# UDC-GAC/pRIblast

Hardware: AMD Instinct MI355X
Metric: query RNAs/sec in `ris` step (higher is better)
Workload: dtype f64

## Files before the change

### priblast_amd/csrc/capi_core.hip

```cpp
#include <dlfcn.h>

#include <algorithm>
#include <cstdio>
#include <cstdlib>
#include <cstring>
#include <numeric>

#include "../../include/priblast_hip.h"
#include "context.hpp"
#include "raccess_kernels.hpp"

namespace prb {

static thread_local std::string g_error;
void set_error(const std::string &msg) { g_error = msg; }
int hip_fail(hipError_t e, const char *what) {
  g_error = std::string("HIP error '") + hipGetErrorString(e) + "' in " + what;
  return PRB_ERR_HIP;
}

int DevBuf::ensure(size_t bytes) {
  if (bytes <= cap) return PRB_OK;
  if (p) {
    hipError_t e = hipFree(p);
    p = nullptr;
    cap = 0;
    if (e != hipSuccess) return hip_fail(e, "hipFree");
  }
  size_t want = bytes > ((size_t)8 << 30) ? bytes : bytes + bytes / 8;
  hipError_t e = hipMalloc(&p, want);
  if (e != hipSuccess) {
    (void)hipGetLastError();
    e = hipMalloc(&p, bytes);
    want = bytes;
  }
  if (e != hipSuccess) {
    (void)hipGetLastError();
    p = nullptr;
    size_t free_b = 0, total_b = 0;
    (void)hipMemGetInfo(&free_b, &total_b);
    set_error("out of device memory allocating " + std::to_string(bytes) + " bytes (" + std::to_string(free_b >> 20) + " MiB of " +
              std::to_string(total_b >> 20) + " free)");
    return PRB_ERR_NOMEM;
  }
  cap = want;
  return PRB_OK;
}
void DevBuf::release() {
  if (p) (void)hipFree(p);
  p = nullptr;
  cap = 0;
}

static std::string default_param_file() {
  Dl_info info;
  if (dladdr((void *)&default_param_file, &info) && info.dli_fname) {
    std::string so = info.dli_fname;
    size_t k = so.rfind('/');
    std::string dir = k == std::string::npos ? "." : so.substr(0, k);
    return dir + "/../params/rna_andronescu2007.par";
  }
  return "priblast_amd/params/rna_andronescu2007.par";
}

}

int prb_ctx::time_begin() {
  PRB_HIP(hipEventRecord(ev0, stream));
  return PRB_OK;
}
int prb_ctx::time_end(const char *stage, int64_t launches) { return time_end(timers[stage], launches); }
int prb_ctx::time_end(prb::StageTimer &t, int64_t launches) {
  PRB_HIP(hipEventRecord(ev1, stream));
  PRB_HIP(hipEventSynchronize(ev1));
  float ms = 0;
  PRB_HIP(hipEventElapsedTime(&ms, ev0, ev1));
  t.ms += ms;
  t.launches += launches;
  return PRB_OK;
}

using namespace prb;

extern "C" {

const char *prb_last_error(void) { return g_error.c_str(); }
const char *prb_version(void) { return "priblast-hip 0.1 (gfx950)"; }

void prb_ris_opts_default(prb_ris_opts *o) {
  o->max_seed_length = 20;
  o->hybrid_threshold = -6.0;
  o->interaction_threshold = -4.0;
  o->final_threshold = -8.0;
  o->drop_out_wo_gap = 5;
  o->drop_out_w_gap = 16;
  o->min_helix_length = 3;
  o->output_style = 0;
  o->distinct_sites = 0;
  o->chain_sites = 0;
  o->allowed_pairs = nullptr;
}

int prb_search_const_upload(prb_ctx *ctx);
void prb_search_const_free(prb_ctx *ctx);

}

static int ctx_init(prb_ctx *ctx, int device, const char *param_file) {
  PRB_HIP(hipSetDevice(device));
  ctx->device = device;
  std::string pf = param_file ? param_file : default_param_file();
  std::string err = load_energy_params(pf, ctx->params);
  if (!err.empty()) {
    set_error(err);
    return PRB_ERR_IO;
  }
  build_raccess_tables(ctx->params, ctx->ra_tables);
  build_fmath_tables(ctx->fm_tables);
  PRB_HIP(hipStreamCreateWithFlags(&ctx->stream, hipStreamNonBlocking));
  PRB_HIP(hipEventCreate(&ctx->ev0));
  PRB_HIP(hipEventCreate(&ctx->ev1));
  auto up = [&](DevBuf &b, const void *src, size_t bytes) -> int {
    int rc = b.ensure(bytes);
    if (rc) return rc;
    PRB_HIP(hipMemcpy(b.p, src, bytes, hipMemcpyHostToDevice));
    return PRB_OK;
  };
  int rc;
  if ((rc = up(ctx->d_expd, ctx->fm_tables.expd_tbl.data(), 2048 * sizeof(uint64_t)))) return rc;
  if ((rc = up(ctx->d_log, ctx->fm_tables.log_tbl.data(), 4096 * sizeof(float)))) return rc;
  if ((rc = up(ctx->d_small, ctx->ra_tables.small.data(), ctx->ra_tables.small.size() * sizeof(double)))) return rc;
  if ((rc = up(ctx->d_big, ctx->ra_tables.big.data(), ctx->ra_tables.big.size() * sizeof(double)))) return rc;
  RaConst &c = ctx->ra_const;
  c.expd_tbl = ctx->d_expd.as<uint64_t>();
  c.log_tbl = ctx->d_log.as<float>();
  c.small = ctx->d_small.as<double>();
  c.big = ctx->d_big.as<double>();
  c.expd_a = ctx->fm_tables.expd_a;
  c.expd_ra = ctx->fm_tables.expd_ra;
  c.c_log2 = ctx->fm_tables.c_log2;
  for (int a = 0; a < 5; a++)
    for (int b = 0; b < 5; b++) c.bp_pair[a * 5 + b] = (unsigned char)ctx->params.bp_pair[a][b];
  if ((rc = prb_search_const_upload(ctx))) return rc;
  size_t free_b = 0, total_b = 0;
  PRB_HIP(hipMemGetInfo(&free_b, &total_b));
  const char *env = getenv("PRB_RACCESS_WORKSPACE_GB");
  double gb = env ? atof(env) : 48.0;
  ctx->ra_budget_bytes = (size_t)std::min(gb * (double)(1ull << 30), 0.5 * (double)free_b);
  return PRB_OK;
}

extern "C" {

int prb_ctx_create(int device, const char *param_file, prb_ctx **out) {
  if (!out) return PRB_ERR_ARG;
  *out = nullptr;
  int ndev = 0;
  hipError_t e = hipGetDeviceCount(&ndev);
  if (e != hipSuccess || ndev == 0) {
    set_error("no HIP device available (this library has no CPU path)");
    return PRB_ERR_HIP;
  }
  if (device < 0 || device >= ndev) {
    set_error("device index out of range");
    return PRB_ERR_ARG;
  }
  prb_ctx *ctx = nullptr;
  int rc;
  try {
    ctx = new prb_ctx();
    rc = ctx_init(ctx, device, param_file);
  } catch (const std::exception &ex) {
    set_error(std::string("prb_ctx_create: ") + ex.what());
    rc = PRB_ERR_NOMEM;
  }
  if (rc != PRB_OK) {
    const std::string keep = prb_last_error();
    if (ctx) prb_ctx_destroy(ctx);
    set_error(keep);
    return rc;
  }
  *out = ctx;
  return PRB_OK;
}


void prb_ctx_destroy(prb_ctx *ctx) {
  if (!ctx) return;
  (void)hipSetDevice(ctx->device);
  if (ctx->stream) (void)hipStreamSynchronize(ctx->stream);
  prb_search_const_free(ctx);
  for (DevBuf *b : {&ctx->d_expd, &ctx->d_log, &ctx->d_small, &ctx->d_big, &ctx->ra_band, &ctx->ra_vec,
                    &ctx->ra_codes, &ctx->ra_desc, &ctx->ra_watchdog, &ctx->ra_acc, &ctx->ra_cond})
    b->release();
  if (ctx->ev0) (void)hipEventDestroy(ctx->ev0);
  if (ctx->ev1) (void)hipEventDestroy(ctx->ev1);
  if (ctx->stream) (void)hipStreamDestroy(ctx->stream);
  delete ctx;
}

int prb_ctx_synchronize(prb_ctx *ctx) {
  if (!ctx) return PRB_ERR_ARG;
  PRB_HIP(hipStreamSynchronize(ctx->stream));
  return PRB_OK;
}

int prb_ctx_stage_ms(prb_ctx *ctx, const char *stage, double *ms, int64_t *launches) {
  if (!ctx || !stage) return PRB_ERR_ARG;
  if (std::strcmp(stage, "slow_hits") == 0) {
    if (ms) *ms = 0;
    if (launches) *launches = ctx->slow_hits;
    return PRB_OK;
  }
  const prb::StageTimer *t = nullptr;
  for (int i = 0; i < (int)prb::ModeTimer::kCount && !t; i++)
    if (std::strcmp(stage, prb::kModeTimerName[i]) == 0) t = &ctx->mode_timers[i];
  if (!t) {
    auto it = ctx->timers.find(stage);
    if (it != ctx->timers.end()) t = &it->second;
  }
  if (ms) *ms = t ? t->ms : 0.0;
  if (launches) *launches = t ? t->launches : 0;
  return PRB_OK;
}
void prb_ctx_reset_timers(prb_ctx *ctx) {
  if (ctx) {
    ctx->timers.clear();
    for (prb::StageTimer &t : ctx->mode_timers) t = prb::StageTimer{};
    ctx->slow_hits = 0;
  }
}

}

namespace prb {

static inline unsigned char ra_code(char ch) {
  switch (ch) {
  case 'A': case 'a': return 1;
  case 'C': case 'c': return 2;
  case 'G': case 'g': return 3;
  case 'T': case 't': case 'U': case 'u': return 4;
  default: return 0;
  }
}

int run_accessibility(prb_ctx *ctx, int32_t nseq, const char *seqs, const int64_t *in_off, const int32_t *lens,
                      const int64_t *out_off, int W, int delta, float *d_acc, float *d_cond) {
  static_assert(kRaMaxSpan + 2 < RaSmallLayout::kHairpinN, "hairpin table covers every span");
  if (W < 1 || delta < 2 || W > kRaMaxSpan) {
    set_error("unsupported (maximal span -w, min accessible length -d): this build needs 1 <= w <= 255 and d >= 2");
    return PRB_ERR_ARG;
  }
  PRB_HIP(hipSetDevice(ctx->device));
  std::vector<int32_t> order(nseq);
  std::iota(order.begin(), order.end(), 0);
  auto len = [&](int i) { return (int64_t)lens[i]; };
  std::stable_sort(order.begin(), order.end(), [&](int a, int b) { return len(a) > len(b); });
  int32_t pos = 0;
  std::vector<RaSeqDesc> desc;
  std::vector<unsigned char> codes;
  while (pos < nseq) {
    desc.clear();
    codes.clear();
    int64_t band = 0, vec = 0;
    int32_t end = pos;
    while (end < nseq) {
      const int64_t L = len(order[end]);
      const size_t need = (size_t)(band + ra_band_elems((int)L, W) + vec + ra_vec_elems((int)L)) * sizeof(double);
      if (end > pos && (need > ctx->ra_budget_bytes || end - pos >= kRaMaxChunk)) break;
      RaSeqDesc d;
      d.band_off = band;
      d.vec_off = vec;
      d.code_off = (int64_t)codes.size();
      d.out_off = out_off[order[end]];
      d.L = (int32_t)L;
      d.pad = 0;
      desc.push_back(d);
      band += ra_band_elems((int)L, W);
      vec += ra_vec_elems((int)L);
      codes.push_back(0);
      const char *sp = seqs + in_off[order[end]];
      for (int64_t k = 0; k < L; k++) codes.push_back(ra_code(sp[k]));
      codes.push_back(0);
      end++;
    }
    const int32_t n = end - pos;
    int rc;
    if ((rc = ctx->ra_band.ensure((size_t)band * sizeof(double)))) return rc;
    if ((rc = ctx->ra_vec.ensure((size_t)vec * sizeof(double)))) return rc;
    if ((rc = ctx->ra_codes.ensure(codes.size()))) return rc;
    if ((rc = ctx->ra_desc.ensure(desc.size() * sizeof(RaSeqDesc)))) return rc;
    if ((rc = ctx->ra_watchdog.ensure(sizeof(int)))) return rc;
    PRB_HIP(hipMemcpyAsync(ctx->ra_codes.p, codes.data(), codes.size(), hipMemcpyHostToDevice, ctx->stream));
    PRB_HIP(hipMemcpyAsync(ctx->ra_desc.p, desc.data(), desc.size() * sizeof(RaSeqDesc), hipMemcpyHostToDevice,
                           ctx->stream));
    RaBatch b;
    b.desc = ctx->ra_desc.as<RaSeqDesc>();
    b.nseq = n;
    b.lmax = (int32_t)len(order[pos]);
    b.W = W;
    b.delta = delta;
    b.band = ctx->ra_band.as<double>();
    b.vec = ctx->ra_vec.as<double>();
    b.codes = ctx->ra_codes.as<unsigned char>();
    b.acc = d_acc;
    b.cond = d_cond;
    b.watchdog = ctx->ra_watchdog.as<int>();
    {
      const char *e = std::getenv("PRB_RACCESS_LOGSUM_WINDOWS");
      const int64_t lmax = len(order[pos]);
      b.logsum_windows = (e && std::atoi(e) == 0) ? 0 : (int32_t)((lmax + 63) / 64);
      const char *h = std::getenv("PRB_RACCESS_HELPERS");
      b.helpers = h ? std::max(0, std::min(3, std::atoi(h))) : (n <= 512 ? 3 : 0);
      const char *wa = std::getenv("PRB_RACCESS_WINDOWS_ALL");
      b.windows_all = wa ? (std::atoi(wa) != 0) : (n <= 512);
    }
    if (b.helpers == 3) PRB_HIP(hipMemsetAsync(b.watchdog, 0, sizeof(int), ctx->stream));
    if ((rc = ctx->time_begin())) return rc;
    PRB_HIP(ra_launch(b, ctx->ra_const, band, vec, ctx->stream));
    if ((rc = ctx->time_end("raccess", 1))) return rc;
    if (b.helpers == 3) {
      int tripped = 0;
      PRB_HIP(hipMemcpy(&tripped, b.watchdog, sizeof(int), hipMemcpyDeviceToHost));
      if (tripped) {
        set_error("Raccess: a wavefront gave up waiting for its workgroup (PRB_RACCESS_HELPERS=2 avoids that form of the passes)");
        return PRB_ERR_STATE;
      }
    }
    pos = end;
  }
  return PRB_OK;
}

}

extern "C" int prb_accessibility(prb_ctx *ctx, int32_t nseq, const char *seqs, const int64_t *offsets,
                                 int32_t maximal_span, int32_t min_accessible_length, float *acc, float *cond) {
  if (!ctx || nseq < 0 || (nseq > 0 && (!seqs || !offsets)) || !acc || !cond) {
    set_error("prb_accessibility: bad argument");
    return PRB_ERR_ARG;
  }
  if (nseq == 0) return PRB_OK;
  const int64_t total = offsets[nseq] - offsets[0];
  const size_t bytes = (size_t)std::max<int64_t>(total, 1) * sizeof(float);
  int rc;
  PRB_HIP(hipSetDevice(ctx->device));
  if ((rc = ctx->ra_acc.ensure(bytes))) return rc;
  if ((rc = ctx->ra_cond.ensure(bytes))) return rc;
  PRB_HIP(hipMemsetAsync(ctx->ra_acc.p, 0, bytes, ctx->stream));
  PRB_HIP(hipMemsetAsync(ctx->ra_cond.p, 0, bytes, ctx->stream));
  std::vector<int32_t> lens(nseq);
  std::vector<int64_t> out_off(nseq);
  for (int32_t i = 0; i < nseq; i++) {
    if (offsets[i + 1] < offsets[i] || offsets[i + 1] - offsets[i] > INT32_MAX - 4) {
      set_error("prb_accessibility: bad offsets");
      return PRB_ERR_ARG;
    }
    lens[i] = (int32_t)(offsets[i + 1] - offsets[i]);
    out_off[i] = offsets[i] - offsets[0];
  }
  if ((rc = run_accessibility(ctx, nseq, seqs, offsets, lens.data(), out_off.data(), maximal_span,
                              min_accessible_length, ctx->ra_acc.as<float>(), ctx->ra_cond.as<float>())))
    return rc;
  PRB_HIP(hipMemcpyAsync(acc, ctx->ra_acc.p, (size_t)total * sizeof(float), hipMemcpyDeviceToHost, ctx->stream));
  PRB_HIP(hipMemcpyAsync(cond, ctx->ra_cond.p, (size_t)total * sizeof(float), hipMemcpyDeviceToHost, ctx->stream));
  PRB_HIP(hipStreamSynchronize(ctx->stream));
  return PRB_OK;
}

extern "C" int prb_accessibility_tables(prb_ctx *ctx, const char *seq, int32_t len, int32_t maximal_span,
                                        int32_t min_accessible_length, float *acc, float *cond,
                                        double *alpha_outer, double *beta_outer, double *const tables[12]) {
  if (!ctx || !seq || len < 0 || !acc || !cond) return PRB_ERR_ARG;
  const int64_t offsets[2] = {0, len};
  int rc = prb_accessibility(ctx, 1, seq, offsets, maximal_span, min_accessible_length, acc, cond);
  if (rc) return rc;
  const int W = maximal_span, S = W + 2;
  const int64_t rows = (int64_t)len + 2;
  std::vector<double> band((size_t)kRaBands * rows * S), vec((size_t)kRaVecs * rows);
  PRB_HIP(hipMemcpy(band.data(), ctx->ra_band.p, band.size() * sizeof(double), hipMemcpyDeviceToHost));
  PRB_HIP(hipMemcpy(vec.data(), ctx->ra_vec.p, vec.size() * sizeof(double), hipMemcpyDeviceToHost));
  if (alpha_outer) std::memcpy(alpha_outer, vec.data(), (size_t)(len + 1) * sizeof(double));
  if (beta_outer) std::memcpy(beta_outer, vec.data() + rows, (size_t)(len + 1) * sizeof(double));
  static const int ids[12] = {0, 1, 2, 3, 4, 5, 7, 8, 9, 10, 11, 12};
  for (int t = 0; tables && t < 12; t++) {
    if (!tables[t]) continue;
    const double *src = band.data() + (size_t)ids[t] * rows * S;
    for (int64_t i = 0; i <= len; i++)
      for (int d = 0; d < S; d++) {
        const int64_t end = i + d;
        tables[t][i * S + d] = end <= len + 1 ? src[end * S + d] : kNegInf;
      }
  }
  return PRB_OK;
}
```

### priblast_amd/csrc/capi_gapped.hip

```cpp
#include <algorithm>
#include <cstdio>

#include "search_stages.hpp"

namespace prb {

static const char *const kTierTimer[5] = {"gapped", "gapped_t1", "gapped_t2", "gapped_t3", "gapped_slow"};

struct WorkList {
  const uint32_t *cur = nullptr;
  int64_t m = 0;
  uint32_t *bufs[2];
  int nb = 0;
  uint32_t *spare() const { return bufs[nb]; }
};
struct Cascade {
  WorkList l;
  GapResume rs[kLdsTiers - 1];
  int skip_mask = 0;
};

static GapArgs view_args(const SubSearch &s, int mode) {
  SearchWs &w = s.w;
  GapArgs a;
  a.in = s.U;
  a.out = s.G;
  a.qb = s.qb->view;
  a.pg = s.pd;
  a.sc = s.sc;
  a.o = s.eo;
  a.first_flag = s.first;
  a.bp_out = w.bpOut.as<int32_t>();
  a.next_work = w.count.as<unsigned long long>() + 1;
  if (mode == 0) {
    a.overflow = w.overflow.as<uint8_t>();
    a.tier_out = w.tierOf.as<uint8_t>();
    a.bp_count = w.ntrace.as<int32_t>();
    a.trace = w.trace.as<uint16_t>();
  }
  return a;
}

static int scratch_for(SubSearch &s, int64_t n, int cap_diag, int cap_rec, GapScratch &gs) {
  gs.cap_diag = cap_diag;
  gs.cap_rec = cap_rec;
  gs.bytes_per_wave = gapped_wave_scratch_bytes(cap_diag, cap_rec);
  if (gs.bytes_per_wave <= kGapWaveLdsBytes && !s.k.wave_hbm) {
    gs.base = nullptr;
    gs.nwaves = (int32_t)std::min<int64_t>(n, 4096);
    return PRB_OK;
  }
  int64_t nw = std::min<int64_t>(n, 4096);
  while (nw > 64 && (size_t)nw * gs.bytes_per_wave > ((size_t)4 << 30)) nw /= 2;
  gs.nwaves = (int32_t)nw;
  int r = s.w.gapScratch.ensure((size_t)nw * gs.bytes_per_wave);
  gs.base = s.w.gapScratch.as<uint8_t>();
  return r;
}

static int select_overflow(SubSearch &s, const uint32_t *cur, int64_t m, uint32_t *next, int64_t *mout) {
  return select_flagged(s.ctx, s.w, cur, s.w.overflow.as<uint8_t>(), next, (size_t)m, mout);
}
static int advance(SubSearch &s, WorkList &l, int64_t *rest) {
  if (int rc = select_overflow(s, l.cur, l.m, l.spare(), rest)) return rc;
  l.cur = l.spare();
  l.nb ^= 1;
  return PRB_OK;
}

static int run_wave(SubSearch &s, int mode, const uint32_t *cur, int64_t m, uint32_t *spare, const int64_t *off_dev, int handover = 0) {
  prb_ctx *ctx = s.ctx;
  SearchWs &w = s.w;
  int rc;
  const bool long_traces = mode == 0 && !s.chunked && m <= 65536 && !s.k.trace_no_long;
  if (long_traces && cur == nullptr) {
    if ((rc = w.slowList.ensure((size_t)m * 4))) return rc;
    PRB_HIP(launch_iota_u32(w.slowList.as<uint32_t>(), m, ctx->stream));
    cur = w.slowList.as<uint32_t>();
  }
  if (long_traces) {
    const int32_t cap = s.k.trace_long_cap;
    if (s.lt_used == 0) {
      if ((rc = w.slowSlot.ensure((size_t)s.nmax * 4))) return rc;
      PRB_HIP(hipMemsetAsync(w.slowSlot.p, 0xFF, (size_t)s.nmax * 4, ctx->stream));
    }
    const size_t have = (size_t)s.lt_used, need = have + (size_t)m;
    if ((rc = grow_keep(ctx, w.slowCnt, have * 8, need * 8)) || (rc = grow_keep(ctx, w.slowTrace, have * 8 * cap, need * 8 * cap))) return rc;
    PRB_HIP(hipMemsetAsync(w.slowCnt.as<int32_t>() + have * 2, 0xFF, (size_t)m * 8, ctx->stream));
    PRB_HIP(launch_assign_slots(cur, m, s.lt_used, w.slowSlot.as<int32_t>(), ctx->stream));
    s.lt_used += (int32_t)m;
    s.lt = LongTrace{w.slowTrace.as<uint32_t>(), w.slowCnt.as<int32_t>(), w.slowSlot.as<int32_t>(), cap};
  }
  int cap_diag = 512, cap_rec = 2048;
  if (mode != 0) {
    cap_diag = std::max(512, ctx->max_gap_caps);
    cap_rec = cap_diag * 4;
  }
  GapArgs a = view_args(s, mode);
  a.bp_off = off_dev;
  a.handover = handover;
  a.lt = s.lt;
  uint32_t *other = spare;
  while (m > 0) {
    GapScratch gs;
    if ((rc = scratch_for(s, m, cap_diag, cap_rec, gs))) return rc;
    a.n = m;
    a.subset = cur;
    PRB_HIP(launch_gapped_wave(a, gs, mode, ctx->stream));
    if (mode != 0) break;
    int64_t again = 0;
    if ((rc = select_overflow(s, cur, m, other, &again))) return rc;
    uint32_t *done_list = const_cast<uint32_t *>(cur);
    cur = other;
    other = done_list ? done_list : (other == w.listA.as<uint32_t>() ? w.listB.as<uint32_t>() : w.listA.as<uint32_t>());
    m = again;
    if (m == 0) break;
    cap_diag *= 4;
    cap_rec *= 4;
    if (cap_diag > 32768) {
      set_error("gapped extension exceeds the supported extension length (32768)");
      return PRB_ERR_STATE;
    }
    ctx->max_gap_caps = std::max(ctx->max_gap_caps, cap_diag);
  }
  return PRB_OK;
}
static int run_slow(SubSearch &s, WorkList &l, int handover) {
  int rc;
  if (!handover) call_front_free(s);
  if ((rc = s.ctx->time_begin())) return rc;
  s.hs->slow_hits += l.m;
  s.ctx->slow_hits += l.m;
  if ((rc = run_wave(s, 0, l.cur, l.m, l.spare(), nullptr, handover))) return rc;
  l.m = 0;
  return s.ctx->time_end(kTierTimer[kWaveTier], 1);
}

static int run_front(SubSearch &s, Cascade &c, bool second_only = false) {
  prb_ctx *ctx = s.ctx;
  SearchWs &w = s.w;
  WorkList &l = c.l;
  int rc;
  if ((rc = w.frontScratch.ensure(gapped_front_scratch_bytes()))) return rc;
  if ((rc = ctx->time_begin())) return rc;
  GapArgs a = view_args(s, 0);
  a.n = l.m;
  a.subset = l.cur;
  a.tier_id = 0;
  PRB_HIP(launch_gapped_front(a, w.frontScratch.p, second_only && !s.k.front_paired, ctx->stream));
  int64_t rest = 0;
  if ((rc = advance(s, l, &rest))) return rc;
  if (s.k.debug_rows) fprintf(stderr, "[front] hits %lld, go on %lld\n", (long long)l.m, (long long)rest);
  ctx->timers["gapped_front_hits"].launches += l.m - rest;
  l.m = rest;
  return ctx->time_end("gapped_front", 1);
}

static int run_cascade(SubSearch &s, Cascade &c, int handover, bool hold_wave) {
  prb_ctx *ctx = s.ctx;
  WorkList &l = c.l;
  int rc;
  for (int tier = s.k.first_tier; tier <= kWaveTier && l.m > 0; tier++) {
    if (tier < kLdsTiers - 1 && ((c.skip_mask >> tier) & 1)) continue;
    if (tier == kWaveTier) {
      if (hold_wave) break;
      if ((rc = run_slow(s, l, handover))) return rc;
      continue;
    }
    if ((rc = ctx->time_begin())) return rc;
    if (tier == 0) ctx->timers["gapped_tier0_hits"].launches += l.m;
    GapArgs a = view_args(s, 0);
    a.n = l.m;
    a.subset = l.cur;
    if (tier >= 1) a.rin = c.rs[tier - 1];
    if (tier < kLdsTiers - 1) a.rout = c.rs[tier];
    a.handover = handover;
    a.acc_scratch = s.w.accScratch.as<double>();
    PRB_HIP(launch_gapped_lds(a, 0, tier, s.k.tiers, ctx->stream));
    int64_t rest = 0;
    if ((rc = advance(s, l, &rest))) return rc;
    if (s.k.debug_rows)
      fprintf(stderr, "[tier %d%s] hits %lld, go on %lld\n", tier, handover ? ", first direction" : "", (long long)l.m, (long long)rest);
    l.m = rest;
    if ((rc = ctx->time_end(kTierTimer[tier], 1))) return rc;
  }
  return PRB_OK;
}

static const struct {
  int one_in;
  int32_t at_most;
} kResumeRoom[kLdsTiers - 1] = {{4, 4 << 20}, {8, 2 << 20}, {32, 1 << 20}};
static_assert(kLdsTiers == 4, "one capacity rule per LDS tier but the last");
static int prepare_resume(SubSearch &s, Cascade &c) {
  SearchWs &w = s.w;
  int rc;
  if ((rc = w.resumeSlot.ensure((size_t)s.nch * 4 * (kLdsTiers - 1))) || (rc = w.resumeCount.ensure(16))) return rc;
  for (int t = 0; t < kLdsTiers - 1; t++) {
    const auto &room = kResumeRoom[t];
    c.rs[t].cap = s.k.resume_cap > 0 ? s.k.resume_cap : (int32_t)std::min<int64_t>(s.nch / room.one_in + 1024, room.at_most);
    if ((rc = w.resumePool[t].ensure((size_t)c.rs[t].cap * gapped_resume_bytes(t)))) return rc;
    c.rs[t].slot = w.resumeSlot.as<int32_t>() + (size_t)t * s.nch;
    c.rs[t].pool = w.resumePool[t].as<uint8_t>();
    c.rs[t].count = w.resumeCount.as<uint32_t>() + t;
  }
  return PRB_OK;
}
static int clear_resume(SubSearch &s) {
  PRB_HIP(hipMemsetAsync(s.w.resumeCount.p, 0, 16, s.ctx->stream));
  PRB_HIP(hipMemsetAsync(s.w.resumeSlot.p, 0xFF, (size_t)s.nch * 4 * (kLdsTiers - 1), s.ctx->stream));
  return PRB_OK;
}

static int run_handover(SubSearch &s, Cascade &c) {
  prb_ctx *ctx = s.ctx;
  SearchWs &w = s.w;
  WorkList &l = c.l;
  int rc;
  const int64_t m_first = l.m;
  if ((rc = w.listC.ensure((size_t)m_first * 4))) return rc;
  PRB_HIP(hipMemcpyAsync(w.listC.p, l.cur, (size_t)m_first * 4, hipMemcpyDeviceToDevice, ctx->stream));
  if ((rc = run_cascade(s, c, 1, true))) return rc;
  const int64_t n_slow = l.m;
  if (n_slow > 0) {
    if ((rc = w.slowList.ensure((size_t)n_slow * 4))) return rc;
    PRB_HIP(hipMemcpyAsync(w.slowList.p, l.cur, (size_t)n_slow * 4, hipMemcpyDeviceToDevice, ctx->stream));
  }
  PRB_HIP(launch_flag_marked(w.tierOf.as<uint8_t>(), w.listC.as<uint32_t>(), m_first, kHandoverMark, w.overflow.as<uint8_t>(), ctx->stream));
  l.cur = w.listC.as<uint32_t>();
  l.m = m_first;
  int64_t mh = 0;
  if ((rc = advance(s, l, &mh))) return rc;
  l.m = mh;
  if (l.m > 0) {
    if (c.rs[0].slot && (rc = clear_resume(s))) return rc;
    if ((rc = run_front(s, c, true))) return rc;
    if ((rc = run_cascade(s, c, 0, true))) return rc;
  }
  if (n_slow + l.m == 0) return PRB_OK;
  if (l.m > 0) {
    if ((rc = grow_keep(ctx, w.slowList, (size_t)n_slow * 4, (size_t)(n_slow + l.m) * 4))) return rc;
    PRB_HIP(hipMemcpyAsync(w.slowList.as<uint32_t>() + n_slow, l.cur, (size_t)l.m * 4, hipMemcpyDeviceToDevice, ctx->stream));
  }
  l.cur = w.slowList.as<uint32_t>();
  l.m += n_slow;
  return run_slow(s, l, 0);
}

static int extend_chunk(SubSearch &s) {
  SearchWs &w = s.w;
  int rc;
  Cascade c;
  if ((rc = w.accScratch.ensure(std::max<size_t>(gapped_acc_scratch_bytes(), 8)))) return rc;
  PRB_HIP(hipMemsetAsync(w.tierOf.p, 0, (size_t)s.nch, s.ctx->stream));
  if (!s.k.no_resume) {
    if ((rc = prepare_resume(s, c)) || (rc = clear_resume(s))) return rc;
  }
  c.l.m = s.nch;
  c.l.bufs[0] = w.listA.as<uint32_t>();
  c.l.bufs[1] = w.listB.as<uint32_t>();
  const bool front_on = s.k.first_tier == 0 && s.k.front && gapped_front_supported(s.sc, s.eo);
  if (front_on) {
    if ((rc = run_front(s, c))) return rc;
    c.skip_mask = s.k.skip_tiers;
  }
  if (!(front_on && s.k.handover)) return run_cascade(s, c, 0, false);
  return c.l.m > 0 ? run_handover(s, c) : PRB_OK;
}

static int keep_chunk(SubSearch &s, int64_t c0) {
  prb_ctx *ctx = s.ctx;
  SearchWs &w = s.w;
  const size_t trace_row = 2 * kTraceCap * sizeof(uint16_t);
  int rc;
  int64_t mc = 0;
  if ((rc = ctx->time_begin())) return rc;
  if ((rc = compact_below(ctx, w, s.G, s.nch, s.opts.final_threshold, w.cidx, w.hitsB, &mc, s.ngap))) return rc;
  if (mc > 0) {
    const size_t have = (size_t)s.ngap, need = have + (size_t)mc;
    if ((rc = grow_keep(ctx, w.keptU, have * sizeof(HitRec), need * sizeof(HitRec))) || (rc = grow_keep(ctx, w.keptFirst, have, need)) ||
        (rc = grow_keep(ctx, w.keptTier, have, need)) || (rc = grow_keep(ctx, w.keptNtrace, have * 4, need * 4)) ||
        (rc = grow_keep(ctx, w.keptTrace, have * trace_row, need * trace_row)))
      return rc;
    const uint32_t *idx = w.cidx.as<uint32_t>();
    PRB_HIP(launch_gather_hits_to_recs(s.U, idx, w.keptU.as<HitRec>() + have, mc, ctx->stream));
    PRB_HIP(launch_gather_u8(s.first, idx, w.keptFirst.as<uint8_t>() + have, mc, ctx->stream));
    PRB_HIP(launch_gather_u8(w.tierOf.as<uint8_t>(), idx, w.keptTier.as<uint8_t>() + have, mc, ctx->stream));
    PRB_HIP(launch_gather_u32(w.ntrace.as<uint32_t>(), idx, w.keptNtrace.as<uint32_t>() + have, mc, ctx->stream));
    PRB_HIP(launch_gather_rows(w.trace.p, idx, static_cast<uint8_t *>(w.keptTrace.p) + have * trace_row, mc, (int)trace_row, ctx->stream));
  }
  if ((rc = ctx->time_end("filter", 2))) return rc;
  if (s.k.debug_rows)
    fprintf(stderr, "[gapped chunk] hits %lld at %lld of %lld, kept %lld\n", (long long)s.nch, (long long)c0, (long long)s.nung, (long long)mc);
  s.ngap += mc;
  if (s.ngap > (int64_t)UINT32_MAX - 16) {
    set_error("more than 4e9 hits under the -g threshold in one sub-batch: build the database in smaller pages (db -c)");
    return PRB_ERR_NOMEM;
  }
  return PRB_OK;
}

int gapped_stage(SubSearch &s) {
  prb_ctx *ctx = s.ctx;
  SearchWs &w = s.w;
  int rc;
  s.chunked = s.nung > s.k.gapped_chunk_hits;
  s.nmax = s.chunked ? s.k.gapped_chunk_hits : s.nung;
  const size_t NM = (size_t)s.nmax;
  if ((rc = w.hitsC.ensure(hits_bytes(s.nmax)))) return rc;
  if ((rc = w.overflow.ensure(NM)) || (rc = w.subset.ensure(NM * 4)) || (rc = w.ntrace.ensure(NM * 4)) || (rc = w.tierOf.ensure(NM)) ||
      (rc = w.listA.ensure(NM * 4)) || (rc = w.listB.ensure(NM * 4)) || (rc = w.count.ensure(16)) ||
      (rc = w.trace.ensure(NM * 2 * kTraceCap * sizeof(uint16_t))))
    return rc;
  s.G = carve_hits(w.hitsC, s.nmax);
  s.nch = s.nmax;
  if (!s.chunked) {
    if ((rc = extend_chunk(s))) return rc;
    s.tier_all = w.tierOf.as<uint8_t>();
    s.ntrace_all = w.ntrace.as<int32_t>();
    s.trace_all = w.trace.as<uint16_t>();
    return PRB_OK;
  }
  const HitSoA Uall = s.U;
  for (int64_t c0 = 0; c0 < s.nung; c0 += s.k.gapped_chunk_hits) {
    s.nch = std::min<int64_t>(s.k.gapped_chunk_hits, s.nung - c0);
    s.U = offset_hits(Uall, c0);
    s.G = carve_hits(w.hitsC, s.nch);
    s.first = w.first.as<uint8_t>() + c0;
    if ((rc = extend_chunk(s)) || (rc = keep_chunk(s, c0))) return rc;
  }
  if (s.ngap > 0) {
    if ((rc = w.hitsA.ensure(hits_bytes(s.ngap))) || (rc = w.cidx.ensure((size_t)s.ngap * 4))) return rc;
    s.U = carve_hits(w.hitsA, s.ngap);
    PRB_HIP(launch_iota_u32(w.cidx.as<uint32_t>(), s.ngap, ctx->stream));
    PRB_HIP(launch_gather_recs_to_hits(w.keptU.as<HitRec>(), w.cidx.as<uint32_t>(), s.U, s.ngap, ctx->stream));
  }
  s.first = w.keptFirst.as<uint8_t>();
  s.tier_all = w.keptTier.as<uint8_t>();
  s.ntrace_all = w.keptNtrace.as<int32_t>();
  s.trace_all = w.keptTrace.as<uint16_t>();
  return PRB_OK;
}

int retrace_tier(SubSearch &s, int tier, const uint32_t *subset2, const int64_t *bpOff2, int64_t m) {
  if (tier == kWaveTier) return run_wave(s, 2, subset2, m, nullptr, bpOff2);
  GapArgs a = view_args(s, 2);
  a.n = m;
  a.subset = subset2;
  a.bp_off = bpOff2;
  a.acc_scratch = s.w.accScratch.as<double>();
  PRB_HIP(launch_gapped_lds(a, 2, tier, s.k.tiers, s.ctx->stream));
  return PRB_OK;
}

}
```

### priblast_amd/csrc/capi_search.hip

```cpp
#include <omp.h>

#include <algorithm>
#include <cmath>
#include <cstdlib>
#include <cstring>

#include "search_stages.hpp"

using namespace prb;

namespace prb {

static bool env_off(const char *e) { return e && atoi(e) == 0; }
static SearchKnobs read_search_knobs() {
  SearchKnobs k;
  const char *e;
  e = getenv("PRB_SEARCH_PAIRS");
  k.budget = e ? atof(e) : 4.0e8;
  k.chunk_pairs = k.budget;
  if ((e = getenv("PRB_SEARCH_CHUNK_PAIRS"))) k.chunk_pairs = atof(e);
  e = getenv("PRB_SEED_ROW_SHIFT");
  k.row_shift = e ? std::min(atoi(e), 30) : 7;
  e = getenv("PRB_SEED_SORT_BITS");
  k.sort_bits = e ? std::max(atoi(e), 1) : 16;
  k.local_order = !env_off(getenv("PRB_SEED_LOCAL_ORDER"));
  e = getenv("PRB_SEED_PAIR_WIDE");
  k.pair_wide = e && atoi(e) != 0;
  k.fused = !env_off(getenv("PRB_SEED_FUSED"));
  k.front_ahead = !getenv("PRB_NO_FRONT_AHEAD");
  k.sort_four_keys = getenv("PRB_SORT_FOUR_KEYS") != nullptr;
  k.sort_two_lengths = getenv("PRB_SORT_TWO_LENGTHS") != nullptr;
  e = getenv("PRB_BIG_LIST_BYTES");
  k.big_list_bytes = e ? (size_t)atof(e) : (size_t)20 << 30;
  e = getenv("PRB_GAPPED_CHUNK_HITS");
  k.gapped_chunk_hits = e ? std::max<int64_t>(1, (int64_t)atof(e)) : 120000000;
  e = getenv("PRB_GAPPED_FIRST_TIER");
  k.first_tier = e ? std::min(std::max(atoi(e), 0), kWaveTier) : 0;
  k.wave_hbm = getenv("PRB_GAPPED_WAVE_HBM") != nullptr;
  k.no_resume = getenv("PRB_GAPPED_NO_RESUME") != nullptr;
  e = getenv("PRB_GAPPED_RESUME_CAP");
  k.resume_cap = e ? std::max(1, atoi(e)) : 0;
  k.front_paired = getenv("PRB_GAPPED_FRONT_PAIRED") != nullptr;
  e = getenv("PRB_GAPPED_SKIP_TIERS");
  k.skip_tiers = e ? atoi(e) : 0;
  k.front = !env_off(getenv("PRB_GAPPED_FRONT"));
  k.handover = !env_off(getenv("PRB_GAPPED_HANDOVER"));
  k.tiers.pair = !env_off(getenv("PRB_GAPPED_PAIR"));
  k.tiers.pool = !env_off(getenv("PRB_GAPPED_POOL"));
  GapTierKnobs &t = k.tiers;
  if ((e = getenv("PRB_GAPPED_LDS_PAD"))) sscanf(e, "%d,%d,%d", &t.pad[1], &t.pad[2], &t.pad[3]);
  t.pad_set = e != nullptr;
  if ((e = getenv("PRB_GAPPED_PERIOD"))) sscanf(e, "%d,%d,%d,%d", &t.period[0], &t.period[1], &t.period[2], &t.period[3]);
  t.period_set = e != nullptr;
  if ((e = getenv("PRB_GAPPED_EARLY"))) sscanf(e, "%d,%d,%d,%d", &t.early[0], &t.early[1], &t.early[2], &t.early[3]);
  t.early_set = e != nullptr;
  k.filter_tiles = !env_off(getenv("PRB_FILTER_TILES"));
  k.trace_no_long = getenv("PRB_TRACE_NO_LONG") != nullptr;
  e = getenv("PRB_TRACE_LONG_CAP");
  k.trace_long_cap = e ? std::max(1, atoi(e)) : 1024;
  k.trace_no_slots = getenv("PRB_TRACE_NO_SLOTS") != nullptr;
  e = getenv("PRB_TRACE_SLOT_CAP");
  k.trace_slot_cap = e ? std::min(kTraceCap, atoi(e)) : kTraceCap;
  e = getenv("PRB_DISTINCT_LDS_HITS");
  k.distinct_lds_hits = e ? atoi(e) : kSiteLdsHits;
  e = getenv("PRB_CHAIN_LDS_HITS");
  k.chain_lds_hits = e ? atoi(e) : kChainLdsHits;
  k.debug_rows = getenv("PRB_DEBUG_ROWS") != nullptr;
  k.debug_mem = getenv("PRB_DEBUG_MEM") != nullptr;
  return k;
}

HitSoA carve_hits(uint8_t *p, int64_t n) {
  HitSoA h;
  const size_t n8 = ((size_t)n + 1) & ~(size_t)1;
  h.e_acc = reinterpret_cast<double *>(p);
  h.e_hyb = h.e_acc + n8;
  h.e_tot = h.e_hyb + n8;
  int32_t *ip = reinterpret_cast<int32_t *>(h.e_tot + n8);
  h.q_sp = ip;
  h.db_sp = ip + n8;
  h.q_len = ip + 2 * n8;
  h.db_len = ip + 3 * n8;
  h.db_id = ip + 4 * n8;
  h.db_id_start = ip + 5 * n8;
  h.query = ip + 6 * n8;
  return h;
}

int sort_target_keys(hipStream_t s, DevBuf &tmp, const uint32_t *kin, uint32_t *kout, const uint32_t *vin, uint32_t *vout, size_t n, unsigned bits) {
  return sort_pairs(s, tmp, kin, kout, vin, vout, n, bits);
}
hipError_t sort_span_keys(void *tmp, size_t &bytes, uint64_t *kin, uint64_t *kout, uint32_t *vin, uint32_t *vout, size_t n, int bits, hipStream_t s) {
  return rocprim::radix_sort_pairs(tmp, bytes, kin, kout, vin, vout, n, 0, bits, s);
}

static int sort_hits(prb_ctx *ctx, SearchWs &w, const SearchKnobs &k, const HitRec *recs, HitSoA out, int64_t n, const SortBounds &sb,
                     uint32_t **perm_out, int32_t *form = nullptr) {
  int rc;
  int32_t why = PRB_SORT_GENERAL_FORCED;
  const size_t N = (size_t)n;
  {
    PackedKeyInfo f;
    f.qmin = sb.qmin;
    f.one_len = sb.eq_len_max > 0;
    f.lmax = f.one_len ? sb.eq_len_max : std::max(sb.max_qlen, sb.max_dblen);
    f.bl = bits_for(f.lmax);
    f.bq = bits_for(sb.max_qlen);
    f.bd = bits_for(sb.nchars);
    const int total = (f.one_len ? 1 : 2) * f.bl + f.bq + f.bd + bits_for(sb.qspan - 1);
    if (!k.sort_four_keys) why = PRB_SORT_GENERAL_WIDTH;
    if (total <= 64 && f.lmax <= 65535 && !k.sort_four_keys) {
      if ((rc = w.kP.ensure(N * 8)) || (rc = w.kTmp2.ensure(N * 8)) || (rc = w.kE.ensure(N * 8)) || (rc = w.kTmp.ensure(N * 8)) ||
          (rc = w.idxA.ensure(N * 4)) || (rc = w.idxB.ensure(N * 4)) || (rc = w.pending.ensure(16)))
        return rc;
      PRB_HIP(launch_make_packed_keys_recs(recs, n, f, w.kP.as<uint64_t>(), w.kE.as<uint64_t>(), w.idxA.as<uint32_t>(), ctx->stream));
      if ((rc = sort_pairs(ctx->stream, w.sortTmp, w.kP.as<uint64_t>(), w.kTmp2.as<uint64_t>(), w.idxA.as<uint32_t>(),
                           w.idxB.as<uint32_t>(), N, (unsigned)total)))
        return rc;
      PRB_HIP(launch_gather_u64(w.kE.as<uint64_t>(), w.idxB.as<uint32_t>(), w.kTmp.as<uint64_t>(), n, ctx->stream));
      PRB_HIP(hipMemsetAsync(w.pending.p, 0, 4, ctx->stream));
      PRB_HIP(launch_fix_ties(w.kTmp2.as<uint64_t>(), w.kTmp.as<uint64_t>(), w.idxB.as<uint32_t>(), n, recs, w.idxA.as<uint32_t>(),
                              w.pending.as<int32_t>(), ctx->stream));
      int32_t too_long = 0;
      PRB_HIP(hipMemcpyAsync(&too_long, w.pending.p, 4, hipMemcpyDeviceToHost, ctx->stream));
      PRB_HIP(hipStreamSynchronize(ctx->stream));
      if (!too_long) {
        PRB_HIP(launch_gather_recs_to_hits(recs, w.idxA.as<uint32_t>(), out, n, ctx->stream));
        *perm_out = w.idxA.as<uint32_t>();
        if (form) *form = f.one_len ? PRB_SORT_PACKED_ONE_LENGTH : PRB_SORT_PACKED_TWO_LENGTHS;
        return PRB_OK;
      }
      why = PRB_SORT_GENERAL_TIE_RUN;
    }
  }
  if (form) *form = why;
  if (k.debug_mem) fprintf(stderr, "[mem] sort: the general form (%lld hits)\n", (long long)n);
  if ((rc = w.hitsTmp.ensure(hits_bytes(n)))) return rc;
  const HitSoA in = carve_hits(w.hitsTmp, n);
  PRB_HIP(launch_gather_recs_to_hits(recs, nullptr, in, n, ctx->stream));
  if ((rc = w.kE.ensure(N * 8)) || (rc = w.kL.ensure(N * 4)) || (rc = w.kQ.ensure(N * 4)) || (rc = w.kP.ensure(N * 8)) ||
      (rc = w.kTmp.ensure(N * 8)) || (rc = w.kTmp2.ensure(N * 8)) || (rc = w.idxA.ensure(N * 4)) ||
      (rc = w.idxB.ensure(N * 4)))
    return rc;
  PRB_HIP(launch_make_keys(in, n, w.kE.as<uint64_t>(), w.kL.as<uint32_t>(), w.kQ.as<uint32_t>(), w.kP.as<uint64_t>(),
                           w.idxA.as<uint32_t>(), ctx->stream));
  uint32_t *ia = w.idxA.as<uint32_t>(), *ib = w.idxB.as<uint32_t>();
  auto sort_step = [&](auto *keys, unsigned bits) -> int {
    using K = std::remove_pointer_t<decltype(keys)>;
    if (int r = sort_pairs(ctx->stream, w.sortTmp, keys, w.kTmp2.as<K>(), ia, ib, N, bits)) return r;
    std::swap(ia, ib);
    return PRB_OK;
  };
  PRB_HIP(launch_order_keys(in.e_acc, n, w.kTmp.as<uint64_t>(), ctx->stream));
  if ((rc = sort_step(w.kTmp.as<uint64_t>(), 64))) return rc;
  PRB_HIP(launch_order_keys(in.e_hyb, n, w.kTmp2.as<uint64_t>(), ctx->stream));
  PRB_HIP(launch_gather_u64(w.kTmp2.as<uint64_t>(), ia, w.kTmp.as<uint64_t>(), n, ctx->stream));
  if ((rc = sort_step(w.kTmp.as<uint64_t>(), 64))) return rc;
  PRB_HIP(launch_gather_u64(w.kE.as<uint64_t>(), ia, w.kTmp.as<uint64_t>(), n, ctx->stream));
  if ((rc = sort_step(w.kTmp.as<uint64_t>(), 64))) return rc;
  PRB_HIP(launch_gather_u32(w.kL.as<uint32_t>(), ia, w.kTmp.as<uint32_t>(), n, ctx->stream));
  if ((rc = sort_step(w.kTmp.as<uint32_t>(), 32))) return rc;
  PRB_HIP(launch_gather_u32(w.kQ.as<uint32_t>(), ia, w.kTmp.as<uint32_t>(), n, ctx->stream));
  if ((rc = sort_step(w.kTmp.as<uint32_t>(), 32))) return rc;
  PRB_HIP(launch_gather_u64(w.kP.as<uint64_t>(), ia, w.kTmp.as<uint64_t>(), n, ctx->stream));
  unsigned qbits = 1;
  while ((int64_t(1) << qbits) < (int64_t)sb.qmin + sb.qspan && qbits < 31) qbits++;
  if ((rc = sort_step(w.kTmp.as<uint64_t>(), 32 + qbits))) return rc;
  PRB_HIP(launch_gather_hits(in, ia, out, n, ctx->stream));
  *perm_out = ia;
  return PRB_OK;
}

struct MaxOp {
  __host__ __device__ int64_t operator()(const int64_t &a, const int64_t &b) const { return a > b ? a : b; }
};

static int filter_hits(prb_ctx *ctx, SearchWs &w, const HitSoA &h, int64_t n, double thr, bool tiles, int64_t *nsurv) {
  int rc;
  const size_t N = (size_t)n;
  *nsurv = 0;
  if (n == 0) return PRB_OK;
  if ((rc = w.endKey.ensure(N * 8)) || (rc = w.pmax.ensure(N * 8)) || (rc = w.state.ensure(N)) || (rc = w.keep.ensure(N)) ||
      (rc = w.pending.ensure(16)) || (rc = w.surv.ensure(N * 4)) || (rc = w.count.ensure(16)))
    return rc;
  PRB_HIP(launch_filter_init(h, n, thr, w.endKey.as<int64_t>(), w.state.as<uint8_t>(), ctx->stream));
  if ((rc = with_temp(w.scanTmp, "rocprim::inclusive_scan", [&](void *t, size_t &b) {
         return rocprim::inclusive_scan(t, b, w.endKey.as<int64_t>(), w.pmax.as<int64_t>(), N, MaxOp(), ctx->stream);
       })))
    return rc;
  for (int round = 0;; round++) {
    PRB_HIP(hipMemsetAsync(w.pending.p, 0, 4, ctx->stream));
    PRB_HIP(launch_filter_round(h, n, w.pmax.as<int64_t>(), w.state.as<uint8_t>(), w.pending.as<int32_t>(), tiles, ctx->stream));
    int32_t pend = 0;
    PRB_HIP(hipMemcpyAsync(&pend, w.pending.p, 4, hipMemcpyDeviceToHost, ctx->stream));
    PRB_HIP(hipStreamSynchronize(ctx->stream));
    if (!pend) break;
    if (round > 100000) {
      set_error("redundancy filter did not converge");
      return PRB_ERR_STATE;
    }
  }
  PRB_HIP(launch_filter_final(h, n, w.pmax.as<int64_t>(), w.state.as<uint8_t>(), w.keep.as<uint8_t>(), tiles, ctx->stream));
  return select_flagged(ctx, w, nullptr, w.keep.as<uint8_t>(), w.surv.as<uint32_t>(), N, nsurv);
}

static void mem_note(const char *where, const SearchWs &w) {
  static const bool on = getenv("PRB_DEBUG_MEM") != nullptr;
  if (!on) return;
  size_t free_b = 0, total_b = 0;
  (void)hipMemGetInfo(&free_b, &total_b);
  fprintf(stderr, "[mem] %-18s free %7zu MiB | hitsA %6zu hitsB %6zu hitsC %6zu hitsTmp %6zu MiB\n", where, free_b >> 20, w.hitsA.cap >> 20,
          w.hitsB.cap >> 20, w.hitsC.cap >> 20, w.hitsTmp.cap >> 20);
}

int grow_keep(prb_ctx *ctx, DevBuf &buf, size_t have, size_t need, size_t spare_limit) {
  int rc;
  if (have > 0 && need > buf.cap) {
    DevBuf bigger;
    if ((rc = need > spare_limit ? PRB_ERR_NOMEM : bigger.ensure(need + need / 2)) && (rc = bigger.ensure(need + need / 6)) &&
        (rc = bigger.ensure(need)))
      return rc;
    PRB_HIP(hipMemcpyAsync(bigger.p, buf.p, have, hipMemcpyDeviceToDevice, ctx->stream));
    PRB_HIP(hipStreamSynchronize(ctx->stream));
    buf.release();
    buf = bigger;
    return PRB_OK;
  }
  return buf.ensure(need);
}
static int reserve_recs(prb_ctx *ctx, DevBuf &recbuf, int64_t have, int64_t more) {
  return grow_keep(ctx, recbuf, (size_t)have * sizeof(HitRec), ((size_t)have + (size_t)more) * sizeof(HitRec), (size_t)16 << 30);
}

int compact_below(prb_ctx *ctx, SearchWs &w, const HitSoA &in, int64_t n, double thr, DevBuf &idxbuf, DevBuf &recbuf, int64_t *m,
                  int64_t have) {
  int rc;
  *m = 0;
  if (n == 0) return PRB_OK;
  const size_t N = (size_t)n;
  if ((rc = w.keep.ensure(N)) || (rc = idxbuf.ensure(N * 4)) || (rc = w.count.ensure(16))) return rc;
  PRB_HIP(launch_flag_not_above(in.e_tot, n, thr, w.keep.as<uint8_t>(), ctx->stream));
  if ((rc = select_flagged(ctx, w, nullptr, w.keep.as<uint8_t>(), idxbuf.as<uint32_t>(), N, m))) return rc;
  if ((rc = reserve_recs(ctx, recbuf, have, std::max<int64_t>(*m, 1)))) return rc;
  PRB_HIP(launch_gather_hits_to_recs(in, idxbuf.as<uint32_t>(), recbuf.as<HitRec>() + have, *m, ctx->stream));
  return PRB_OK;
}

static int download_hits(prb_ctx *ctx, SearchWs &w, const HitSoA &h, int64_t n, std::vector<prb_hit> &out) {
  HostTimer ht(ctx, "host_download");
  const size_t base = out.size();
  if (n == 0) return PRB_OK;
  int rc;
  const size_t bytes = (size_t)n * sizeof(prb_hit);
  if ((rc = w.packed.ensure(bytes)) || (rc = w.pinned.ensure(bytes))) return rc;
  PRB_HIP(launch_pack_hits(h, n, nullptr, nullptr, -1, w.packed.p, ctx->stream));
  PRB_HIP(hipMemcpyAsync(w.pinned.p, w.packed.p, bytes, hipMemcpyDeviceToHost, ctx->stream));
  if (out.capacity() < base + (size_t)n) out.reserve(std::max(2 * out.capacity(), base + (size_t)n));
  PRB_HIP(hipStreamSynchronize(ctx->stream));
  const prb_hit *src = static_cast<const prb_hit *>(w.pinned.p);
  out.insert(out.end(), src, src + n);
  return PRB_OK;
}

static int32_t chunk_end(const CandDev *cd, int32_t ncand, int32_t c0, double chunk_pairs, double *pairs_out) {
  int32_t c1 = c0;
  double acc = 0;
  while (c1 < ncand) {
    const double pairs = (double)(cd[c1].ep_q - cd[c1].sp_q + 1) * (double)(cd[c1].ep_db - cd[c1].sp_db + 1);
    if (c1 > c0 && (acc + pairs > chunk_pairs || c1 - c0 >= kMaxFusedCands)) break;
    acc += pairs;
    c1++;
  }
  *pairs_out = acc;
  return c1;
}

struct RowKeyBits {
  int dbits, kbits;
  int begin = 0;
  bool wide() const { return kbits > 32; }
};
static RowKeyBits row_key_bits(const PageDev &pd, int row_shift, const CandDev *cd, int32_t nc) {
  const int dbits = bits_for(std::max<int64_t>(1, ((int64_t)pd.nchars - 1) >> row_shift));
  return RowKeyBits{dbits, dbits + bits_for(std::max<int64_t>(1, (int64_t)cd[nc - 1].query - cd[0].query))};
}
template <class V>
static int sort_by_row_key(hipStream_t s, DevBuf &tmp, const RowKeyBits &kb, DevBuf &kin, DevBuf &kout, const V *vin, V *vout, size_t n) {
  return kb.wide() ? sort_pairs(s, tmp, kin.as<uint64_t>(), kout.as<uint64_t>(), vin, vout, n, (unsigned)kb.begin, (unsigned)kb.kbits)
                   : sort_pairs(s, tmp, kin.as<uint32_t>(), kout.as<uint32_t>(), vin, vout, n, (unsigned)kb.begin, (unsigned)kb.kbits);
}
static int sort_chunk_pairs(hipStream_t s, DevBuf &tmp, const PairLayout &lay, DevBuf &kin, DevBuf &kout, DevBuf &vin, DevBuf &vout, size_t n) {
  const RowKeyBits kb{lay.pbits, lay.kbits, lay.begin};
  return lay.narrow ? sort_by_row_key(s, tmp, kb, kin, kout, vin.as<uint32_t>(), vout.as<uint32_t>(), n)
                    : sort_by_row_key(s, tmp, kb, kin, kout, vin.as<uint64_t>(), vout.as<uint64_t>(), n);
}

static int scan_row_counts(prb_ctx *ctx, SearchWs &w, int64_t n) {
  auto in = rocprim::make_transform_iterator(w.row_count.as<int32_t>(), ToI64());
  return with_temp(w.scanTmp, "rocprim::exclusive_scan", [&](void *t, size_t &b) {
    return rocprim::exclusive_scan(t, b, in, w.row_off.as<int64_t>(), (int64_t)0, (size_t)n + 1, rocprim::plus<int64_t>(), ctx->stream);
  });
}

static int issue_front(SearchWs &w, const prb_qbatch *qb, const PageDev &pd, int delta, const SearchKnobs &k, const CandDev *cd, int32_t nc,
                       int64_t cents, hipStream_t s, int64_t *np_out, const AllowDev *allow, prb_ctx *timed) {
  SearchWs::FrontStage &F = w.front;
  int rc;
  *np_out = -1;
  if ((rc = F.pair0_pin.ensure(((size_t)nc + 1) * 8))) return rc;
  int64_t *pair0 = static_cast<int64_t *>(F.pair0_pin.p);
  int64_t np = 0;
  for (int32_t c = 0; c < nc; c++) {
    const int64_t qw = cd[c].ep_q - cd[c].sp_q + 1;
    if (qw > kMaxFusedEntries) return PRB_OK;
    pair0[c] = np;
    np += qw * (int64_t)(cd[c].ep_db - cd[c].sp_db + 1);
  }
  pair0[nc] = np;
  const size_t NP = (size_t)np;
  const PairLayout lay = pair_layout(pd.nchars, (int64_t)cd[nc - 1].query - cd[0].query, k.row_shift, k.sort_bits, k.local_order, k.pair_wide);
  if ((rc = F.cands.ensure((size_t)nc * sizeof(CandDev))) || (rc = F.seed_qacc.ensure((size_t)std::max<int64_t>(cents, 1) * 8)) ||
      (rc = F.pair0.ensure(((size_t)nc + 1) * 8)) || (rc = F.keyA.ensure(NP * lay.key_bytes())) || (rc = F.keyB.ensure(NP * lay.key_bytes())) ||
      (rc = F.valA.ensure(NP * lay.val_bytes())) || (rc = F.valB.ensure(NP * lay.val_bytes())))
    return rc;
  PRB_HIP(hipMemcpyAsync(F.cands.p, cd, (size_t)nc * sizeof(CandDev), hipMemcpyHostToDevice, s));
  PRB_HIP(hipMemcpyAsync(F.pair0.p, pair0, ((size_t)nc + 1) * 8, hipMemcpyHostToDevice, s));
  PRB_HIP(launch_seed_qacc(F.cands.as<CandDev>(), nc, cents, qb->view, delta, F.seed_qacc.as<double>(), s));
  PRB_HIP(launch_pair_keys(F.cands.as<CandDev>(), F.pair0.as<int64_t>(), nc, np, pd, cd[0].query, lay, F.keyA.p, F.valA.p, s));
  F.unsorted = false;
  F.np_all = np;
  F.lay = lay;
  F.keys = F.keyB.p;
  F.vals = F.valB.p;
  if (allow) {
    const int64_t nw = allow_words(np);
    if ((rc = F.ballot.ensure((size_t)nw * 8)) || (rc = F.wcount.ensure((size_t)(nw + 1) * 4)) || (rc = F.woff.ensure((size_t)(nw + 1) * 8)) ||
        (rc = F.kept_pin.ensure(8)))
      return rc;
    if (timed && ((rc = timed->time_end("seed", 1)) || (rc = timed->time_begin()))) return rc;
    PRB_HIP(hipMemsetAsync(F.wcount.as<int32_t>() + nw, 0, 4, s));
    PRB_HIP(launch_allow_test(F.cands.as<CandDev>(), F.pair0.as<int64_t>(), F.valA.p, lay, np, pd, *allow, F.ballot.as<uint64_t>(),
                              F.wcount.as<int32_t>(), s));
    auto counts = rocprim::make_transform_iterator(F.wcount.as<int32_t>(), ToI64());
    if ((rc = with_temp(F.scanTmp, "rocprim::exclusive_scan", [&](void *t, size_t &b) {
           return rocprim::exclusive_scan(t, b, counts, F.woff.as<int64_t>(), (int64_t)0, (size_t)nw + 1, rocprim::plus<int64_t>(), s);
         })))
      return rc;
    PRB_HIP(launch_allow_scatter(F.keyA.p, F.valA.p, np, lay, F.ballot.as<uint64_t>(), F.woff.as<int64_t>(), F.keyB.p, F.valB.p, s));
    PRB_HIP(hipMemcpyAsync(F.kept_pin.p, F.woff.as<int64_t>() + nw, 8, hipMemcpyDeviceToHost, s));
    if (timed && ((rc = timed->time_end(ModeTimer::kAllow, 3)) || (rc = timed->time_begin()))) return rc;
    F.unsorted = true;
    *np_out = np;
    return PRB_OK;
  }
  if ((rc = sort_chunk_pairs(s, F.sortTmp, lay, F.keyA, F.keyB, F.valA, F.valB, NP))) return rc;
  *np_out = np;
  return PRB_OK;
}

static int finish_front(prb_ctx *ctx, SearchWs &w, const SearchKnobs &k, int32_t nc, int64_t *np) {
  SearchWs::FrontStage &F = w.front;
  int rc;
  PRB_HIP(hipStreamSynchronize(ctx->stream));
  F.unsorted = false;
  const int64_t kept = *static_cast<const int64_t *>(F.kept_pin.p);
  if (kept < 0 || kept > F.np_all) {
    set_error("pair mask: " + std::to_string(kept) + " of " + std::to_string(F.np_all) + " pairs kept");
    return PRB_ERR_STATE;
  }
  if (k.debug_rows) fprintf(stderr, "[allow] cands %d pairs %lld allowed %lld\n", nc, (long long)F.np_all, (long long)kept);
  *np = kept;
  if (kept == 0) return PRB_OK;
  if ((rc = sort_chunk_pairs(ctx->stream, F.sortTmp, F.lay, F.keyB, F.keyA, F.valB, F.valA, (size_t)kept))) return rc;
  F.keys = F.keyA.p;
  F.vals = F.valA.p;
  return PRB_OK;
}

struct SeedChunk {
  int32_t c0, c1, nc;
  int64_t crows, cents;
  double pairs;
};

static int count_hits_under_f(SubSearch &s, int64_t more) {
  s.nf += more;
  if (s.nf > (int64_t)UINT32_MAX - 16) {
    set_error("more than 4e9 hits under the -f threshold in one sub-batch: build the database in smaller pages (db -c)");
    return PRB_ERR_NOMEM;
  }
  return PRB_OK;
}

static int seed_chunk_one_pass(SubSearch &s, const SeedChunk &c, int64_t np) {
  prb_ctx *ctx = s.ctx;
  SearchWs &w = s.w;
  SearchWs::FrontStage &F = w.front;
  int rc;
  if ((rc = w.count.ensure(16))) return rc;
  if ((rc = ctx->time_end("seed", s.allow ? 1 : 2))) return rc;
  if ((rc = ctx->time_begin())) return rc;
  const int64_t nsl = fused_slices(np);
  if ((rc = w.hitsA.ensure((size_t)nsl * kFusePairs * kSliceRecBytes)) || (rc = w.row_count.ensure((size_t)(nsl + 1) * 4)) ||
      (rc = w.row_off.ensure((size_t)(nsl + 1) * 8)))
    return rc;
  PRB_HIP(hipMemsetAsync(w.count.p, 0, 16, ctx->stream));
  PRB_HIP(hipMemsetAsync(w.row_count.as<int32_t>() + nsl, 0, 4, ctx->stream));
  PRB_HIP(launch_seed_extend(F.cands.as<CandDev>(), F.keys, F.vals, F.lay, np, s.qb->view, s.pd, s.sc, s.eo, F.seed_qacc.as<double>(),
                             s.opts.interaction_threshold, s.max_qlen, w.hitsA.p, w.row_count.as<int32_t>(), w.count.as<uint64_t>(),
                             ctx->stream));
  if ((rc = scan_row_counts(ctx, w, nsl))) return rc;
  uint64_t kept = 0, seeds_maxlen[2] = {0, 0};
  PRB_HIP(hipMemcpyAsync(seeds_maxlen, w.count.p, 16, hipMemcpyDeviceToHost, ctx->stream));
  PRB_HIP(hipMemcpyAsync(&kept, w.row_off.as<int64_t>() + nsl, 8, hipMemcpyDeviceToHost, ctx->stream));
  PRB_HIP(hipStreamSynchronize(ctx->stream));
  s.one_pass_maxlen = std::max<int64_t>(s.one_pass_maxlen, (int64_t)seeds_maxlen[1]);
  if (kept > 0) {
    if ((rc = reserve_recs(ctx, w.hitsB, s.nf, (int64_t)kept))) return rc;
    PRB_HIP(launch_collect_slices(w.hitsA.p, w.row_count.as<int32_t>(), w.row_off.as<int64_t>(), nsl, w.hitsB.as<HitRec>() + s.nf,
                                  ctx->stream));
  }
  if ((rc = ctx->time_end("ungapped", 1))) return rc;
  s.hs->counts[0] += (int64_t)seeds_maxlen[0];
  if (s.k.debug_rows)
    fprintf(stderr, "[pairs] cands %d pairs %lld seeds %lld kept %lld\n", c.nc, (long long)np, (long long)seeds_maxlen[0], (long long)kept);
  return count_hits_under_f(s, (int64_t)kept);
}

static int seed_chunk_lists(SubSearch &s, const SeedChunk &c) {
  prb_ctx *ctx = s.ctx;
  SearchWs &w = s.w;
  const CandDev *cd = s.b.cd + c.c0;
  const int32_t nc = c.nc;
  const int64_t crows = c.crows, cents = c.cents;
  const int delta = s.eo.delta;
  int rc;
  s.all_one_pass = false;
  if ((rc = w.cands.ensure((size_t)nc * sizeof(CandDev))) || (rc = w.row_count.ensure((size_t)(crows + 1) * 4)) ||
      (rc = w.row_off.ensure((size_t)(crows + 1) * 8)) || (rc = w.row_cand.ensure((size_t)(crows + 1) * 4)) ||
      (rc = w.seed_qacc.ensure((size_t)std::max<int64_t>(cents, 1) * 8)))
    return rc;
  PRB_HIP(hipMemcpyAsync(w.cands.p, cd, (size_t)nc * sizeof(CandDev), hipMemcpyHostToDevice, ctx->stream));
  if ((rc = ctx->time_begin())) return rc;
  PRB_HIP(hipMemsetAsync(w.row_count.as<int32_t>() + crows, 0, 4, ctx->stream));
  PRB_HIP(launch_seed_qacc(w.cands.as<CandDev>(), nc, cents, s.qb->view, delta, w.seed_qacc.as<double>(), ctx->stream));
  const uint32_t *row_perm = nullptr;
  if (s.last_stage != 1 && crows > 1 && crows < (int64_t)UINT32_MAX && s.k.row_shift >= 0) {
    const size_t NR = (size_t)crows;
    const RowKeyBits kb = row_key_bits(s.pd, s.k.row_shift, cd, nc);
    if ((rc = w.kP.ensure(NR * 8)) || (rc = w.kTmp2.ensure(NR * 8)) || (rc = w.idxA.ensure(NR * 4)) || (rc = w.idxB.ensure(NR * 4)))
      return rc;
    PRB_HIP(launch_row_keys(w.cands.as<CandDev>(), nc, crows, s.pd, cd[0].query, s.k.row_shift, kb.dbits, kb.wide(), w.row_cand.as<int32_t>(),
                            w.kP.p, w.idxA.as<uint32_t>(), ctx->stream));
    if ((rc = sort_by_row_key(ctx->stream, w.sortTmp, kb, w.kP, w.kTmp2, w.idxA.as<uint32_t>(), w.idxB.as<uint32_t>(), NR))) return rc;
    row_perm = w.idxB.as<uint32_t>();
  }
  if (s.allow)
    PRB_HIP(launch_seed_count_allowed(w.cands.as<CandDev>(), nc, crows, s.qb->view, s.pd, delta, w.seed_qacc.as<double>(),
                                      w.row_count.as<int32_t>(), w.row_cand.as<int32_t>(), row_perm, *s.allow, ctx->stream));
  else
    PRB_HIP(launch_seed_count(w.cands.as<CandDev>(), nc, crows, s.qb->view, s.pd, delta, w.seed_qacc.as<double>(),
                              w.row_count.as<int32_t>(), w.row_cand.as<int32_t>(), row_perm, ctx->stream));
  if ((rc = scan_row_counts(ctx, w, crows))) return rc;
  int64_t nseed = 0;
  PRB_HIP(hipMemcpyAsync(&nseed, w.row_off.as<int64_t>() + crows, 8, hipMemcpyDeviceToHost, ctx->stream));
  PRB_HIP(hipStreamSynchronize(ctx->stream));
  s.hs->counts[0] += nseed;
  if (s.k.debug_rows)
    fprintf(stderr, "[rows] cands %d rows %lld qents %lld pairs %.0f seeds %lld\n", nc, (long long)crows, (long long)cents, c.pairs, (long long)nseed);
  if (nseed == 0) return ctx->time_end("seed", 2);
  if (nseed > (int64_t)UINT32_MAX - 16) {
    set_error("too many seed hits in one chunk of candidates (a single candidate with more than 4e9 seed hits?): lower "
              "PRB_SEARCH_CHUNK_PAIRS");
    return PRB_ERR_NOMEM;
  }
  if ((rc = w.hitsA.ensure(hits_bytes(nseed)))) return rc;
  HitSoA A = carve_hits(w.hitsA, nseed);
  if (s.allow)
    PRB_HIP(launch_seed_emit_allowed(w.cands.as<CandDev>(), nc, crows, s.qb->view, s.pd, delta, w.seed_qacc.as<double>(),
                                     w.row_cand.as<int32_t>(), w.row_off.as<int64_t>(), A, row_perm, *s.allow, ctx->stream));
  else
    PRB_HIP(launch_seed_emit(w.cands.as<CandDev>(), nc, crows, s.qb->view, s.pd, delta, w.seed_qacc.as<double>(),
                             w.row_cand.as<int32_t>(), w.row_off.as<int64_t>(), A, row_perm, ctx->stream));
  if ((rc = ctx->time_end("seed", 2))) return rc;
  if (s.last_stage == 1) return download_hits(ctx, w, A, nseed, s.hs->hits);
  if ((rc = ctx->time_begin())) return rc;
  PRB_HIP(launch_ungapped(A, nseed, s.qb->view, s.pd, s.sc, s.eo, s.max_qlen, ctx->stream));
  if ((rc = ctx->time_end("ungapped", 1))) return rc;
  int64_t mc = 0;
  if ((rc = ctx->time_begin())) return rc;
  if ((rc = compact_below(ctx, w, A, nseed, s.opts.interaction_threshold, w.cidx, w.hitsB, &mc, s.nf))) return rc;
  if ((rc = ctx->time_end("filter", 2))) return rc;
  return count_hits_under_f(s, mc);
// ... 854 lines not shown
```

### priblast_amd/csrc/context.hpp

```cpp
#pragma once
#include <hip/hip_runtime.h>

#include <cstdint>
#include <map>
#include <string>
#include <vector>

#include "energy.hpp"
#include "raccess_device.hpp"

namespace prb {

void set_error(const std::string &msg);
int hip_fail(hipError_t e, const char *what);

#define PRB_HIP(call)                                   \
  do {                                                  \
    hipError_t e_ = (call);                             \
    if (e_ != hipSuccess) return prb::hip_fail(e_, #call); \
  } while (0)

struct DevBuf {
  void *p = nullptr;
  size_t cap = 0;
  int ensure(size_t bytes);
  void release();
  template <class T> T *as() const { return static_cast<T *>(p); }
};

struct StageTimer {
  double ms = 0;
  int64_t launches = 0;
};

enum class ModeTimer { kSummary, kTop, kProfile, kTopHits, kTargets, kDistinct, kChain, kAllow, kCoverage, kNull, kGroup, kGnull, kEval, kGroupRank, kFeature, kFnull, kCount };
inline constexpr const char *kModeTimerName[(int)ModeTimer::kCount] = {"summary", "top",   "profile",  "tophits", "targets", "distinct",
                                                                       "chain",   "allow", "coverage", "null",    "group",   "gnull",
                                                                       "eval",    "grouprank", "feature", "fnull"};

}

struct prb_ctx {
  int device = 0;
  hipStream_t stream = nullptr;
  hipEvent_t ev0 = nullptr, ev1 = nullptr;
  prb::EnergyParams params;
  prb::RaccessTables ra_tables;
  prb::FmathTables fm_tables;
  prb::RaConst ra_const{};
  void *search_const = nullptr;
  void *search_ws = nullptr;
  int64_t slow_hits = 0;
  int max_gap_caps = 128;
  bool keep_device_records = false;
  size_t keep_hint_hits = 0, keep_hint_bp = 0;
  size_t host_hint_hits = 0, host_hint_bp = 0;
  prb::DevBuf d_expd, d_log, d_small, d_big;
  prb::DevBuf ra_band, ra_vec, ra_codes, ra_desc, ra_acc, ra_cond;
  prb::DevBuf ra_watchdog;
  size_t ra_budget_bytes = 0;
  std::map<std::string, prb::StageTimer> timers;
  prb::StageTimer mode_timers[(int)prb::ModeTimer::kCount];

  int time_begin();
  int time_end(const char *stage, int64_t launches);
  int time_end(prb::ModeTimer t, int64_t launches) { return time_end(mode_timers[(int)t], launches); }
  int time_end(prb::StageTimer &t, int64_t launches);
};
```

### priblast_amd/csrc/gapped_args.hpp

```cpp
#pragma once
#include <hip/hip_runtime.h>

#include <cstdint>

#include "search_device.hpp"
#include "search_kernels.hpp"

namespace prb {

struct Rec32 {
  using word = uint32_t;
  static constexpr bool kBases = true;
  static __device__ __forceinline__ word pack(int i, int j, int pred, int type, int qa, int da) {
    return (word)i | ((word)j << 7) | ((word)pred << 14) | ((word)type << 21) | ((word)qa << 24) | ((word)da << 27);
  }
  static __device__ __forceinline__ int i(word v) { return v & 0x7F; }
  static __device__ __forceinline__ int j(word v) { return (v >> 7) & 0x7F; }
  static __device__ __forceinline__ int pred(word v) { return (v >> 14) & 0x7F; }
  static __device__ __forceinline__ int type(word v) { return (v >> 21) & 7; }
  static __device__ __forceinline__ int qa(word v) { return (v >> 24) & 7; }
  static __device__ __forceinline__ int da(word v) { return (v >> 27) & 7; }
};



struct DirOrigin {
  int q_start, id_start, id_end;
  int64_t db_start;
};
__device__ __forceinline__ DirOrigin dir_origin(const HitState &h, int flag) {
  DirOrigin o;
  if (flag == 0) {
    o.q_start = h.q_sp;
    o.db_start = h.db_sp;
  } else {
    o.q_start = h.q_sp + h.q_len - 1;
    o.db_start = (int64_t)h.db_sp + h.db_len - 1;
  }
  o.id_start = h.id_start;
  o.id_end = h.id_start + h.db_len - 1;
  return o;
}

}
```

### priblast_amd/csrc/gapped_front.hip

```cpp
#include <algorithm>
#include <cstdlib>

#include "gapped_args.hpp"
#include "search_device.hpp"
#include "search_kernels.hpp"

namespace prb {

#ifdef PRB_GAP_PROFILE
__device__ unsigned long long g_front_prof[32];
#define FP_DECL unsigned long long fp_t0_ = __builtin_amdgcn_s_memtime(), fp_acc_[32] = {}
#define FP_MARK(k)                                              \
  do {                                                          \
    const unsigned long long t_ = __builtin_amdgcn_s_memtime(); \
    fp_acc_[k] += t_ - fp_t0_;                                  \
    fp_t0_ = t_;                                                \
  } while (0)
#define FP_COUNT(k, v) fp_acc_[k] += (unsigned long long)(v)
#define FP_FLUSH()                                                        \
  do {                                                                    \
    if (lane == 0)                                                        \
      for (int i_ = 0; i_ < 32; i_++) atomicAdd(&g_front_prof[i_], fp_acc_[i_]); \
  } while (0)
#else
#define FP_DECL
#define FP_MARK(k)
#define FP_COUNT(k, v)
#define FP_FLUSH()
#endif

namespace {

constexpr int kFD = kFrontMaxDrop;
#ifndef PRB_FRONT_RING
#define PRB_FRONT_RING 24
#endif
constexpr int kFR = PRB_FRONT_RING;
constexpr int kFWaves = 1;
constexpr int kFDirs = 64;
constexpr int kFCells = 192;
#ifndef PRB_FRONT_PAIRS
#define PRB_FRONT_PAIRS 256
#endif
constexpr int kFPairs = PRB_FRONT_PAIRS;
constexpr int kFScan = 8;

struct FrontTab {
  static constexpr int kBulge = SearchTab::kInt11;
  static constexpr int kTau = kBulge + 31;
  static constexpr int kZero = kTau + 8;
  static constexpr int kCount = kZero + 1;
};
static_assert(SearchTab::kStack == 0 && SearchTab::kInt11 == 255, "stack, internal and mismatch tables lead SearchTab");

struct FrontAcc {
  double eq[kFD][kFDirs], ed[kFD][kFDirs];
};

#ifndef PRB_FRONT_POOL
#define PRB_FRONT_POOL 832
#endif
constexpr int kFPool = PRB_FRONT_POOL;
static_assert(kFPool >= 2 * kFDirs && kFPool <= 1024, "FRec::pool");
static_assert(kFrontMaxDrop <= 16, "FrontLds::wfp: 16 cells per anti-diagonal");
struct FRec {
  static __device__ __forceinline__ uint32_t pack(int i, int j, int pool, int type, int qa, int da) {
    return (uint32_t)i | ((uint32_t)j << 5) | ((uint32_t)pool << 10) | ((uint32_t)type << 20) | ((uint32_t)qa << 23) | ((uint32_t)da << 26);
  }
  static __device__ __forceinline__ int i(uint32_t v) { return v & 31; }
  static __device__ __forceinline__ int j(uint32_t v) { return (v >> 5) & 31; }
  static __device__ __forceinline__ int pool(uint32_t v) { return (v >> 10) & 1023; }
  static __device__ __forceinline__ int type(uint32_t v) { return (v >> 20) & 7; }
  static __device__ __forceinline__ int qa(uint32_t v) { return (v >> 23) & 7; }
  static __device__ __forceinline__ int da(uint32_t v) { return (v >> 26) & 7; }
};

struct FrontLds {
  double hyb[kFPool];
  double te[kFPairs];
  int32_t tab[FrontTab::kCount];
  uint32_t info[kFR][kFDirs];
  uint32_t cells[kFCells];
  uint32_t wfp[2][kFDirs];
  uint8_t improved[kFDirs];
  uint32_t pairs[kFPairs];
};

struct Planes {
  uint32_t lo, hi, valid;
};
__device__ __forceinline__ int plane_base(uint32_t lo, uint32_t hi, uint32_t valid, int t) {
  const uint32_t l = (lo >> t) & 1, h = (hi >> t) & 1, v = (valid >> t) & 1;
  return v ? (int)(((h * 2 + l + 2) & 3) + 1) : 0;
}

__device__ __forceinline__ Planes load_planes(const uint8_t *s, int64_t n, int64_t start, int dir) {
  Planes p{0, 0, 0};
  const int64_t first = dir > 0 ? start : start - 31;
  const uintptr_t addr = reinterpret_cast<uintptr_t>(s) + (uintptr_t)first;
  const int sh = (int)(addr & 3);
  const uint32_t *sw = reinterpret_cast<const uint32_t *>(addr - (uintptr_t)sh);
  uint32_t w[9];
#pragma unroll
  for (int k = 0; k < 9; k++) {
    const int64_t pos_lo = first - sh + 4 * k;
    w[k] = (pos_lo + 3 >= 0 && pos_lo < n) ? sw[k] : 0u;
  }
  uint32_t x[8];
#pragma unroll
  for (int k = 0; k < 8; k++) x[k] = __builtin_amdgcn_alignbyte(w[k + 1], w[k], (uint32_t)sh);
#pragma unroll
  for (int k = 0; k < 8; k++) {
    const uint32_t c = x[k];
    const uint32_t any = (c | (c >> 1) | (c >> 2)) >> 1;
    const uint32_t lo4 = ((c & 0x01010101u) * 0x10204080u) >> 28;
    const uint32_t hi4 = (((c >> 1) & 0x01010101u) * 0x10204080u) >> 28;
    const uint32_t ok4 = ((any & 0x01010101u) * 0x10204080u) >> 28;
    p.lo |= lo4 << (4 * k);
    p.hi |= hi4 << (4 * k);
    p.valid |= ok4 << (4 * k);
  }
  {
    const int64_t lo_t = first < 0 ? -first : 0;
    const int64_t hi_t = first + 31 >= n ? n - 1 - first : 31;
    uint32_t inside = 0;
    if (hi_t >= lo_t) inside = (hi_t >= 31 ? ~0u : ((1u << (hi_t + 1)) - 1u)) & ~((1u << lo_t) - 1u);
    p.valid &= inside;
  }
  if (dir < 0) {
    p.lo = __builtin_bitreverse32(p.lo);
    p.hi = __builtin_bitreverse32(p.hi);
    p.valid = __builtin_bitreverse32(p.valid);
  }
  p.lo &= p.valid;
  p.hi &= p.valid;
  return p;
}

__device__ __forceinline__ void diag_masks(const Planes &q, const Planes &dr, int len, uint32_t &pairs, uint32_t &wob) {
  const int s = 31 - len;
  const uint32_t dl = dr.lo >> s, dh = dr.hi >> s, dv = dr.valid >> s;
  const uint32_t both = q.valid & dv, ldiff = q.lo ^ dl;
  const uint32_t gu = ~(q.hi | dh);
  wob = both & ldiff & gu;
  pairs = both & ldiff & ((q.hi ^ dh) | gu);
}

__device__ __forceinline__ int wave_excl_scan(int v, int lane, int &total) {
  int x = v;
  x += __builtin_amdgcn_update_dpp(0, x, 0x111, 0xF, 0xF, true);
  x += __builtin_amdgcn_update_dpp(0, x, 0x112, 0xF, 0xF, true);
  x += __builtin_amdgcn_update_dpp(0, x, 0x114, 0xF, 0xF, true);
  x += __builtin_amdgcn_update_dpp(0, x, 0x118, 0xF, 0xF, true);
  x += __builtin_amdgcn_update_dpp(0, x, 0x142, 0xA, 0xF, false);
  x += __builtin_amdgcn_update_dpp(0, x, 0x143, 0xC, 0xF, false);
  (void)lane;
  total = __builtin_amdgcn_readlane(x, 63);
  return x - v;
}

__device__ __forceinline__ void wave_lds_sync() {
  __builtin_amdgcn_fence(__ATOMIC_RELEASE, "wavefront");
  __builtin_amdgcn_wave_barrier();
  __builtin_amdgcn_fence(__ATOMIC_ACQUIRE, "wavefront");
}
__device__ __forceinline__ void wave_mem_sync() {
  __builtin_amdgcn_fence(__ATOMIC_RELEASE, "workgroup");
  __builtin_amdgcn_wave_barrier();
  __builtin_amdgcn_fence(__ATOMIC_ACQUIRE, "workgroup");
}

__device__ __forceinline__ double loop_energy_front(const SearchConst &sc, const int32_t *lt, int type, int type2, int u1, int u2, int a,
                                                    int b, int c, int d) {
  using T = SearchTab;
  using F = FrontTab;
  const int tt = type * 8 + type2;
  const int st = T::kStack + type * 7 + type2;
  const bool z1 = u1 == 0, z2 = u2 == 0;
  const int u = z1 ? u2 : u1;
  const bool c11 = u1 == 1 && u2 == 1, c12 = u1 == 1 && u2 == 2, c21 = u1 == 2 && u2 == 1, c22 = u1 == 2 && u2 == 2;
  const bool special = c11 || c12 || c21 || c22;
  int i1 = T::kInternal + u1 + u2;
  int i2 = special ? F::kZero : T::kMismatchI + (type * 5 + a) * 5 + b;
  int i3 = special ? F::kZero : T::kMismatchI + (type2 * 5 + d) * 5 + c;
  if (z1 || z2) {
    const bool stack = z1 && z2;
    i1 = stack ? st : F::kBulge + u;
    i2 = stack ? F::kZero : (u == 1 ? st : F::kTau + type);
    i3 = (stack || u == 1) ? F::kZero : F::kTau + type2;
  }
  int z1v = lt[special ? F::kZero : i1];
  if (special) {
    const int i11 = T::kInt11 + (tt * 5 + a) * 5 + b;
    const int i21a = T::kInt21 + ((tt * 5 + a) * 5 + d) * 5 + b;
    const int i21b = T::kInt21 + (((type2 * 8 + type) * 5 + d) * 5 + a) * 5 + c;
    const int i22 = T::kInt22 + (((tt * 5 + a) * 5 + c) * 5 + d) * 5 + b;
    z1v = sc.tab[c11 ? i11 : c12 ? i21a : c21 ? i21b : i22];
  }
  return div100(sc, z1v + lt[i2] + lt[i3]);
}

template <bool kOneDir>
__global__ __launch_bounds__(64 * kFWaves) void k_gapped_front(GapArgs a, FrontAcc *acc_blocks) {
  __shared__ FrontLds lds[kFWaves];
  const int lane = threadIdx.x & 63;
  FrontLds &S = lds[threadIdx.x >> 6];
  FrontAcc &A = acc_blocks[(int64_t)blockIdx.x * kFWaves + (threadIdx.x >> 6)];
  const SearchConst &sc = a.sc;
  for (int t = lane; t < FrontTab::kCount; t += 64)
    S.tab[t] = t < SearchTab::kInt11    ? sc.tab[t]
               : t < FrontTab::kTau     ? sc.tab[SearchTab::kBulge + (t - FrontTab::kBulge)]
               : t < FrontTab::kZero    ? sc.tab[SearchTab::kTau + (t - FrontTab::kTau)]
                                        : 0;
  const int flag = kOneDir ? 1 : lane & 1;
  const bool f0 = flag == 0;
  const int drop = a.o.drop_w_gap, min_helix = a.o.min_helix, delta = a.o.delta;
  const int64_t nwaves = (int64_t)gridDim.x * kFWaves;
  constexpr int kTileHits = kOneDir ? kFDirs : kFDirs / 2;
  const int64_t ntiles = (a.n + kTileHits - 1) / kTileHits;
  const bool isdir = lane < kFDirs;
  const int me = isdir ? lane : 0;
  int64_t tile = (int64_t)blockIdx.x * kFWaves + (threadIdx.x >> 6);
  FP_DECL;
  while (tile < ntiles) {
    FP_MARK(0);
    FP_COUNT(16, 1);
    unsigned long long nt = 0;
    const int64_t w = tile * kTileHits + (kOneDir ? lane : lane >> 1);
    const bool live = isdir && w < a.n;
    int64_t x = 0, qo = 0, dbase = 0;
    int query = 0, id = 0, qn = 1, q_sp = 0, db_sp = 0, q_len = 0, db_len = 0, id_start = 0;
    double e_tot = 0, e_acc = 0;
    bool resumed = false;
    int tier0 = 0, nleft0 = 0;
    if (live) {
      x = a.subset ? (int64_t)a.subset[w] : w;
      query = a.in.query[x];
      qo = a.qb.off[query];
      qn = a.qb.len[query] + 1;
      id = a.in.db_id[x];
      dbase = (int64_t)a.pg.start_pos[id] - id;
      q_sp = a.in.q_sp[x];
      db_sp = a.in.db_sp[x];
      q_len = a.in.q_len[x];
      db_len = a.in.db_len[x];
      id_start = a.in.db_id_start[x];
      e_tot = a.in.e_tot[x];
      e_acc = a.in.e_acc[x];
      const uint8_t mark = a.tier_out[x];
      if (is_resumed(mark)) {
        resumed = true;
        tier0 = mark & kMarkTier;
        nleft0 = a.bp_count[x] & 0xFFFF;
        q_sp = a.out.q_sp[x];
        db_sp = a.out.db_sp[x];
        q_len = a.out.q_len[x];
        db_len = a.out.db_len[x];
        id_start = a.out.db_id_start[x];
        e_tot = a.out.e_tot[x];
        e_acc = a.out.e_acc[x];
      }
    }
    const uint8_t *qs = a.qb.enc + qo;
    const int q_start = f0 ? q_sp : q_sp + US(q_len) - 1;
    const int64_t db_start = f0 ? (int64_t)db_sp : (int64_t)db_sp + US(db_len) - 1;
    const int id_end = id_start + US(db_len) - 1;
    bool dead = !live || (resumed && f0);
    if (kOneDir && !resumed) dead = true;
    FP_MARK(1);

    Planes q{0, 0, 0}, dr{0, 0, 0};
    int tq0 = 1, td0 = 1;
    int type0 = 0, q1 = 0, d1 = 0;
    if (live) {
      q = load_planes(qs, qn, q_start, f0 ? -1 : 1);
      const Planes dd = load_planes(a.pg.seqs, a.pg.nchars, db_start, f0 ? -1 : 1);
      tq0 = (q.valid >> 1) == 0x7FFFFFFFu ? 32 : __builtin_ctz(~(q.valid >> 1)) + 1;
      td0 = (dd.valid >> 1) == 0x7FFFFFFFu ? 32 : __builtin_ctz(~(dd.valid >> 1)) + 1;
      const int q0 = plane_base(q.lo, q.hi, q.valid, 0), d0 = plane_base(dd.lo, dd.hi, dd.valid, 0);
      q1 = plane_base(q.lo, q.hi, q.valid, 1);
      d1 = plane_base(dd.lo, dd.hi, dd.valid, 1);
      type0 = bp_type(sc, q0, d0);
      if (f0) type0 = rtype_of(type0);
      dr.lo = __builtin_bitreverse32(dd.lo);
      dr.hi = __builtin_bitreverse32(dd.hi);
      dr.valid = __builtin_bitreverse32(dd.valid);
    }
    FP_MARK(2);
    const int open_until = tq0 > td0 ? tq0 : td0;
    const int lend = drop < open_until ? drop : open_until;

    {
      const float *a3 = f0 ? a.qb.acc + qo : a.pg.acc + dbase, *c3 = f0 ? a.qb.cond + qo : a.pg.cond + dbase;
      const float *c1 = f0 ? a.pg.cond + dbase + id_end : a.qb.cond + qo + q_start;
      const int p0 = f0 ? q_start : id_start;
      const int t3 = f0 ? tq0 : td0, t1 = f0 ? td0 : tq0;
      double s3 = 0, s1 = 0;
      const float *const nowhere = a.qb.acc;
      float ta[kFD + 1], tz[kFD], tw[kFD];
      const bool v0 = live && 1 < t3 && 1 <= lend;
      ta[0] = *(v0 ? a3 + p0 : nowhere);
#pragma unroll
      for (int len = 1; len <= kFD; len++) {
        const bool v3 = live && len < t3 && len <= lend, v1 = live && len < t1 && len <= lend;
        ta[len] = *(v3 ? a3 + (p0 - len) : nowhere);
        tz[len - 1] = *(v3 ? c3 + (p0 - len + delta) : nowhere);
        tw[len - 1] = *(v1 ? c1 + len : nowhere);
      }
      if (lane == 0) nt = atomicAdd(a.next_work, 1ull);
      if (!v0) ta[0] = 0.0f;
#pragma unroll
      for (int len = 1; len <= kFD; len++) {
        const bool v3 = live && len < t3 && len <= lend, v1 = live && len < t1 && len <= lend;
        if (!v3) ta[len] = tz[len - 1] = 0.0f;
        if (!v1) tw[len - 1] = 0.0f;
      }
#pragma unroll
      for (int len = 1; len <= kFD; len++) {
        const float xx = ta[len], yy = ta[len - 1], zz = tz[len - 1], ww = tw[len - 1];
        s3 = len == 1 ? (double)(xx - yy + zz) : s3 + xx - yy + zz;
        s1 = len == 1 ? (double)ww : s1 + ww;
        if (isdir) {
          A.eq[len - 1][lane] = f0 ? s3 : s1;
          A.ed[len - 1][lane] = f0 ? s1 : s3;
        }
      }
    }
    if (isdir) {
      S.hyb[lane] = e_tot;
      S.info[0][lane] = FRec::pack(0, 0, lane, type0, q1, d1);
      S.improved[lane] = 0;
    }
    int nrec = 1;
    int pool_used = kFDirs;
    uint32_t F2 = type0 != 0 ? 1u : 0u, W2 = wobble(type0) ? 1u : 0u, F1 = 0, W1 = 0;
    wave_mem_sync();
    FP_MARK(3);

    for (int LA = 2; LA <= kFD; LA += 2) {
      if (__ballot(!dead && LA <= lend) == 0) break;
      FP_COUNT(17, 1);
      uint32_t fA = 0, fB = 0;
#pragma unroll
      for (int h = 0; h < 2; h++) {
        const int L = LA + h;
        uint32_t p0, wb0, ahead = ~0u;
        diag_masks(q, dr, L, p0, wb0);
        for (int xx = 1; xx <= min_helix - 1; xx++) {
          uint32_t px, wbx;
          Planes qx{q.lo >> xx, q.hi >> xx, q.valid >> xx};
          diag_masks(qx, dr, L + xx, px, wbx);
          ahead &= px;
          if (xx == 1) ahead &= ~(wb0 & wbx);
        }
        const uint32_t Fp = h == 0 ? F2 : F1, Wp = h == 0 ? W2 : W1;
        const uint32_t need = ~(Fp << 1) | (wb0 & (Wp << 1));
        const int i_first = L - td0 + 1 > 1 ? L - td0 + 1 : 1;
        const int i_hi = (L < tq0 ? L : tq0) - 1;
        const uint32_t range = i_hi >= i_first ? (((i_hi >= 31 ? ~0u : ((1u << (i_hi + 1)) - 1))) & ~((1u << i_first) - 1)) : 0u;
        const uint32_t f = (!dead && L <= lend) ? (p0 & (ahead | ~need) & range) : 0u;
        if (h == 0) fA = f;
        else fB = f;
      }
      int cnt = __popc(fA) + __popc(fB);
      FP_MARK(4);
      if (nrec + cnt > kFR) {
        FP_COUNT(21, __popcll(__ballot(nrec + cnt > kFR)));
        dead = true;
        fA = fB = 0;
        cnt = 0;
      }
      int total;
      int base = wave_excl_scan(cnt, lane, total);
      FP_COUNT(31, total > kFCells || pool_used + total > kFPool);
      if (total > kFCells || pool_used + total > kFPool) {
        if (base + cnt > kFCells || pool_used + base + cnt > kFPool) {
          dead = true;
          fA = fB = 0;
          cnt = 0;
        }
        base = wave_excl_scan(cnt, lane, total);
      }
      {
        int r = 0;
        for (uint32_t m = fA; m; m &= m - 1, r++) S.cells[base + r] = (uint32_t)lane | ((uint32_t)__builtin_ctz(m) << 8) | ((uint32_t)(nrec + r) << 16);
        for (uint32_t m = fB; m; m &= m - 1, r++)
          S.cells[base + r] = (uint32_t)lane | ((uint32_t)__builtin_ctz(m) << 8) | (1u << 13) | ((uint32_t)(nrec + r) << 16);
      }
      if (isdir) {
        S.wfp[0][lane] = 0;
        S.wfp[1][lane] = 0;
      }
      wave_lds_sync();
      FP_MARK(5);
      FP_COUNT(19, total);

      for (int c0 = 0; c0 < total;) {
        FP_COUNT(18, 1);
        const bool has = c0 + lane < total;
        const uint32_t cell = has ? S.cells[c0 + lane] : 0u;
        const int dl = cell & 63, ci = (cell >> 8) & 31, isB = (cell >> 13) & 1, rec = (int)(cell >> 16);
        const int cj = LA + isB - ci;
        const bool cf0 = !kOneDir && (dl & 1) == 0;
        const uint32_t cq_lo = __shfl(q.lo, dl), cq_hi = __shfl(q.hi, dl), cq_v = __shfl(q.valid, dl);
        const uint32_t cd_lo = __shfl(dr.lo, dl), cd_hi = __shfl(dr.hi, dl), cd_v = __shfl(dr.valid, dl);
        const int nrecb = __shfl(nrec, dl);
        const int qc = plane_base(cq_lo, cq_hi, cq_v, ci), nq = plane_base(cq_lo, cq_hi, cq_v, ci > 0 ? ci - 1 : 0),
                  fq = plane_base(cq_lo, cq_hi, cq_v, ci + 1);
        const int sh = 31 - cj - 1;
        const uint32_t dlo = cd_lo >> (sh & 31), dhi = cd_hi >> (sh & 31), dvv = cd_v >> (sh & 31);
        const int fd = plane_base(dlo, dhi, dvv, 0), dc = plane_base(dlo, dhi, dvv, 1), nd = plane_base(dlo, dhi, dvv, 2);
        int ctype = bp_type(sc, qc, dc);
        if (!cf0) ctype = rtype_of(ctype);
        uint32_t qmask = 0;
        double eqc = 0, edc = 0;
        if (has) {
          eqc = A.eq[ci - 1][dl];
          edc = A.ed[cj - 1][dl];
        }
        const int nscan = has ? nrecb : 0;
        FP_COUNT(27, __popcll(__ballot(nscan > kFScan)));
        FP_COUNT(28, __popcll(__ballot(nscan > 2 * kFScan)));
        FP_COUNT(29, __popcll(__ballot(nscan == kFR - 1)));
        for (int k = 0; __ballot(k < nscan) != 0; k += kFScan) {
          uint32_t v[kFScan];
#pragma unroll
          for (int u = 0; u < kFScan; u++) v[u] = S.info[k + u < kFR ? k + u : kFR - 1][dl];
#pragma unroll
          for (int u = 0; u < kFScan; u++)
            if (k + u < nscan && FRec::i(v[u]) < ci && FRec::j(v[u]) < cj) qmask |= 1u << (k + u);
        }
        const uint32_t cdw = (uint32_t)ci | ((uint32_t)cj << 5) | ((uint32_t)ctype << 10) | ((uint32_t)nq << 13) | ((uint32_t)nd << 16) |
                             ((uint32_t)dl << 19);
        const int pool = pool_used + c0 + lane;
        if (has) S.info[rec][dl] = FRec::pack(ci, cj, pool, rtype_of(ctype), fq, fd);
        FP_MARK(6);
        int npc = __popc(qmask), ptotal;
        int poff = wave_excl_scan(npc, lane, ptotal);
        const unsigned long long fits = __ballot(has && poff + npc <= kFPairs);
        const int ncr = fits == ~0ull ? 64 : __builtin_ctzll(~fits);
        const bool mine = lane < ncr;
        if (ncr < 64) ptotal = __shfl(poff, ncr);
        if (mine) {
          int r = 0;
          for (uint32_t m = qmask; m; m &= m - 1, r++) S.pairs[poff + r] = cdw | ((uint32_t)__builtin_ctz(m) << 25);
        }
        wave_lds_sync();
        FP_MARK(7);
        FP_COUNT(20, ptotal);
        for (int p0 = 0; p0 < ptotal; p0 += 64) {
          const int p = p0 + lane;
          if (p < ptotal) {
            const uint32_t cdv = S.pairs[p];
            const int k = cdv >> 25;
            const int pci = cdv & 31, pcj = (cdv >> 5) & 31, pct = (cdv >> 10) & 7, pnq = (cdv >> 13) & 7, pnd = (cdv >> 16) & 7,
                      pdl = (cdv >> 19) & 63;
            const bool pf0 = !kOneDir && (pdl & 1) == 0;
            const uint32_t v = S.info[k][pdl];
            const double hk = S.hyb[FRec::pool(v)];
            const int ri = FRec::i(v), rj = FRec::j(v), rq = FRec::qa(v), rd = FRec::da(v), rt = FRec::type(v);
            double te = loop_energy_front(sc, S.tab, pf0 ? pct : rt, pf0 ? rt : pct, pci - ri - 1, pcj - rj - 1, pf0 ? pnq : rq,
                                          pf0 ? pnd : rd, pf0 ? rq : pnq, pf0 ? rd : pnd);
            te += hk;
            S.te[p] = te;
          }
        }
        wave_lds_sync();
        FP_MARK(8);
        if (mine) {
          double bte = 1000000.0;
          int bk = 0;
          int r = 0;
          for (uint32_t m = qmask; m; m &= m - 1, r++) {
            const double te = S.te[poff + r];
            if (te < bte) {
              bte = te;
              bk = __builtin_ctz(m);
            }
          }
          const int ptype = FRec::type(S.info[bk][dl]);
          S.hyb[pool] = bte;
          FP_COUNT(30, __popcll(__ballot(wobble(ptype))));
          if (ptype != 0) atomicOr(&S.wfp[isB][dl], (wobble(ptype) ? 0x10001u : 1u) << (ci - 1));
          const double ie = eqc + edc + bte;
          const double min_e = S.hyb[dl];
          if (ie < min_e) S.improved[dl] = 1;
        }
        wave_lds_sync();
        FP_MARK(9);
        c0 += ncr;
      }
      nrec += cnt;
      pool_used += total;
      {
        const uint32_t m0 = S.wfp[0][me], m1 = S.wfp[1][me];
        F2 = (m0 & 0xFFFFu) << 1;
        W2 = (m0 >> 16) << 1;
        F1 = (m1 & 0xFFFFu) << 1;
        W1 = (m1 >> 16) << 1;
      }
      FP_COUNT(22, __popcll(__ballot(!dead && S.improved[me] != 0)));
      if (S.improved[me]) dead = true;
      FP_MARK(10);
    }

    FP_COUNT(23, pool_used > 640);
    FP_COUNT(24, pool_used > 704);
    FP_COUNT(25, pool_used > 768);
    FP_COUNT(26, pool_used);
    FP_MARK(11);
    bool ok = live && (!dead || (resumed && f0));
    bool ok_other;
    double dng = 0, dng_other = 0;
    if constexpr (kOneDir) {
      ok_other = ok;
      ok = live && resumed;
      if (live) {
        dng = dangle_energy_gapped(sc, q_sp, (int64_t)db_sp, 0, qs, qn, a.pg.seqs, a.pg.nchars);
        dng_other = dangle_energy_gapped(sc, q_sp + US(q_len) - 1, (int64_t)db_sp + US(db_len) - 1, 1, qs, qn, a.pg.seqs, a.pg.nchars);
      }
    } else {
      ok_other = __shfl_xor(ok ? 1 : 0, 1) != 0;
      if (live) {
        const int qp = f0 ? q_sp : q_sp + US(q_len) - 1;
        const int64_t dp = f0 ? (int64_t)db_sp : (int64_t)db_sp + US(db_len) - 1;
        dng = dangle_energy_gapped(sc, qp, dp, flag, qs, qn, a.pg.seqs, a.pg.nchars);
      }
      dng_other = __shfl_xor(dng, 1);
    }
    if (live && (kOneDir || f0)) {
      if (ok && ok_other) {
        const double d0 = dng, d1 = dng_other;
        double e = e_tot, hy = e_tot - e_acc;
        e += d0;
        e += d1;
        hy += d0;
        hy += d1;
        a.overflow[w] = 0;
        a.tier_out[x] = (uint8_t)(resumed ? tier0 : a.tier_id);
        a.bp_count[x] = nleft0;
        a.out.q_sp[x] = q_sp;
        a.out.db_sp[x] = db_sp;
        a.out.q_len[x] = q_len;
        a.out.db_len[x] = db_len;
        a.out.db_id[x] = id;
        a.out.db_id_start[x] = id_start;
        a.out.query[x] = query;
        a.out.e_acc[x] = e_acc;
        a.out.e_hyb[x] = hy;
        a.out.e_tot[x] = e;
      } else {
        a.overflow[w] = 1;
        if (resumed) {
          a.tier_out[x] = (uint8_t)(kResumeMark | tier0);
        } else if (ok) {
          a.out.q_sp[x] = q_sp;
          a.out.db_sp[x] = db_sp;
          a.out.q_len[x] = q_len;
          a.out.db_len[x] = db_len;
          a.out.db_id_start[x] = id_start;
          a.out.e_acc[x] = e_acc;
          a.out.e_hyb[x] = e_tot - e_acc;
          a.out.e_tot[x] = e_tot;
          a.bp_count[x] = 0;
          a.tier_out[x] = kResumeMark;
        }
      }
    }
    wave_mem_sync();
    tile = nwaves + (int64_t)__shfl(nt, 0);
    FP_MARK(12);
  }
  FP_FLUSH();
}

}

#ifdef PRB_GAP_PROFILE
extern "C" int prb_debug_front_profile(unsigned long long *out, int reset) {
  if (hipDeviceSynchronize() != hipSuccess) return -1;
  if (hipMemcpyFromSymbol(out, HIP_SYMBOL(g_front_prof), sizeof(unsigned long long) * 32) != hipSuccess) return -1;
  if (reset) {
    unsigned long long z[32] = {};
    if (hipMemcpyToSymbol(HIP_SYMBOL(g_front_prof), z, sizeof(z)) != hipSuccess) return -1;
  }
  return 0;
}
#endif

bool gapped_front_supported(const SearchConst &sc, const ExtOpts &o) {
  uint32_t pm = 0, wm = 0;
  auto set = [&](uint32_t &m, int q, int d) { m |= 1u << (q * 5 + d); };
  set(pm, 1, 4), set(pm, 4, 1), set(pm, 2, 3), set(pm, 3, 2), set(pm, 3, 4), set(pm, 4, 3);
  set(wm, 3, 4), set(wm, 4, 3);
  return sc.pair_mask == pm && sc.wobble_mask == wm && o.min_helix >= 1 && o.min_helix <= 7 && o.drop_w_gap >= 1 &&
         o.drop_w_gap <= kFD;
}

static int front_blocks_per_cu() {
  const size_t granule = 2048, lds = (sizeof(FrontLds) * kFWaves + granule - 1) / granule * granule;
  return std::max<int>(1, std::min<int>(12, (int)((160 * 1024) / lds)));
}
size_t gapped_front_scratch_bytes() { return (size_t)256 * front_blocks_per_cu() * kFWaves * sizeof(FrontAcc); }

hipError_t launch_gapped_front(const GapArgs &args, void *scratch, bool second_only, hipStream_t s) {
  const int64_t n = args.n;
  if (n <= 0) return hipSuccess;
  GapArgs a = args;
  a.first_flag = nullptr;
  a.trace = nullptr;
  a.bp_off = nullptr;
  a.bp_out = nullptr;
  a.rin = a.rout = GapResume{};
  if (hipError_t e = hipMemsetAsync(a.next_work, 0, sizeof(unsigned long long), s); e != hipSuccess) return e;
  const int per_tile = second_only ? kFDirs : kFDirs / 2;
  const int64_t tiles = (n + per_tile - 1) / per_tile, want_blocks = (tiles + kFWaves - 1) / kFWaves;
  const dim3 grid((unsigned)std::min<int64_t>(want_blocks, 256 * front_blocks_per_cu())), blk(64 * kFWaves);
  if (second_only) hipLaunchKernelGGL(k_gapped_front<true>, grid, blk, 0, s, a, static_cast<FrontAcc *>(scratch));
  else hipLaunchKernelGGL(k_gapped_front<false>, grid, blk, 0, s, a, static_cast<FrontAcc *>(scratch));
  return hipGetLastError();
}

}
```

### priblast_amd/csrc/gapped_lds.hip

```cpp
#include <algorithm>
#include <type_traits>

#include "gapped_args.hpp"
#include "search_device.hpp"
#include "search_kernels.hpp"

namespace prb {

#ifdef PRB_GAP_PROFILE
constexpr int kProfSlots = 31;
__device__ unsigned long long g_gap_prof[10 * kProfSlots];
struct GapProf {
  unsigned long long last, acc[kProfSlots];
  int cells_now = 0, cells_prev = 0;
  __device__ __forceinline__ void start() {
    for (int i = 0; i < kProfSlots; i++) acc[i] = 0;
    last = __builtin_amdgcn_s_memtime();
  }
  __device__ __forceinline__ void mark(int r) {
    const unsigned long long t = __builtin_amdgcn_s_memtime();
    if (t >= last) acc[r] += t - last;
    else acc[29] += 1;
    last = t;
  }
// ... 1006 lines not shown
    S.info(rec) = R::pack(ci, cj, bk, rtype_of(ctype), S.qb(ci + 1), S.db(cj + 1));
    S.ptab(cur, ci) = (uint8_t)ptype;
  }
  GP_MARK(6);
}

template <class Store>
__device__ __forceinline__ void pair_fill_group(const SearchConst &sc, const Store &S, int flag, const PairStep &p, int gl, GapProf &prof) {
  unsigned long long cells = (unsigned long long)p.cellsA | ((unsigned long long)p.cellsB << 32);
  int rec = p.nrec;
  while (cells) {
    const unsigned long long rest = cells & (cells - 1);
    const bool two = rest != 0, hi = two && gl >= 4;
    const int b = hi ? __builtin_ctzll(rest) : __builtin_ctzll(cells);
    pair_cell(sc, S, flag, p, b, rec + (hi ? 1 : 0), two ? (gl & 3) : gl, two ? 4 : 8, two, true, prof);
    cells = two ? rest & (rest - 1) : rest;
    rec += two ? 2 : 1;
  }
  GP_MARK(26);
  group_sync<true>();
}

template <class T, class Rec>
__device__ __forceinline__ void pair_fill_pool(const SearchConst &sc, LdsLive<T, Rec> *wave_lds, int flag, const PairStep &p, int lane,
                                               GapProf &prof) {
  static_assert(T::kG == 8 && !T::kAccGlobal && T::kCapD < 255 && T::kCapR < 256, "eight groups per wavefront, state in LDS, 8-bit fields");
  const int n = __popc(p.cellsA) + __popc(p.cellsB);
  int incl[8];
  int total = 0;
#pragma unroll
  for (int g = 0; g < 8; g++) {
    total += __builtin_amdgcn_readlane(n, 8 * g);
    incl[g] = total;
  }
  group_sync<true>();
  const uint32_t pk0 = (uint32_t)p.LA | ((uint32_t)p.loA << 8) | ((uint32_t)p.loB << 16) | ((uint32_t)p.dstartA << 24);
  const uint32_t pk1 = (uint32_t)p.i_loA | ((uint32_t)p.curA << 8) | ((uint32_t)p.typeA0 << 10) | ((uint32_t)flag << 13) | ((uint32_t)p.nrec << 16);
  const int slot = lane >> 2, sub = lane & 3;
  for (int t0 = 0; t0 < total; t0 += 16) {
    GP_COUNT(30);
    const int t = t0 + slot;
    int o = 0, ex = 0;
#pragma unroll
    for (int g = 0; g < 7; g++) {
      if (t >= incl[g]) {
        o = g + 1;
        ex = incl[g];
      }
    }
    const int ob = 8 * o;
    const uint32_t q0 = __shfl(pk0, ob), q1 = __shfl(pk1, ob), cA = __shfl(p.cellsA, ob), cB = __shfl(p.cellsB, ob);
    PairStep po;
    po.cellsA = cA;
    po.cellsB = cB;
    po.LA = q0 & 0xFF;
    po.loA = (q0 >> 8) & 0xFF;
    po.loB = (q0 >> 16) & 0xFF;
    po.dstartA = q0 >> 24;
    po.i_loA = q1 & 0xFF;
    po.curA = (q1 >> 8) & 3;
    po.typeA0 = (q1 >> 10) & 7;
    po.nrec = q1 >> 16;
    po.paired = false;
    const int oflag = (q1 >> 13) & 1;
    const int rank = t - ex, nA = __popc(cA);
    const int b = rank < nA ? nth_bit(cA, rank) : 32 + nth_bit(cB, rank - nA);
    GP_MARK(28);
    const LdsStore<T, Rec> So{wave_lds[o], nullptr};
    pair_cell(sc, So, oflag, po, b, po.nrec + rank, sub, 4, true, t < total, prof);
  }
  group_sync<true>();
}

template <class Store>
__device__ __forceinline__ bool pair_close(const ExtOpts &o, const Store &S, int gl, DirState &d, const PairStep &p, GapProf &prof) {
  using R = typename Store::R;
  const int drop = o.drop_w_gap;
  const int n = __popc(p.cellsA) + __popc(p.cellsB);
  if (n != 0) {
    double m = __builtin_inf();
    int key = 0x7fffffff;
    for (int r = gl; r < n; r += 8) {
      const auto v = S.info(p.nrec + r);
      const double ie = S.eq(R::i(v) - 1) + S.ed(R::j(v) - 1) + S.hyb(p.nrec + r);
      if (ie < m) {
        m = ie;
        key = r;
      }
    }
    group_min<8>(m, key);
    if (m < d.min_e) {
      const auto v = S.info(p.nrec + key);
      d.min_e = m;
      d.best = p.nrec + key;
      d.min_ci = R::i(v);
      d.min_cj = R::j(v);
    }
    d.nrec = p.nrec + n;
  }
  GP_MARK(6);
  if (d.overflow) return true;
  if (p.paired) {
    d.length = p.LA + 1;
    d.lo = p.loB;
    if (p.LA + 1 - (d.min_ci + d.min_cj) >= drop) return true;
    return !(p.LA + 1 < d.tq0 || p.LA + 1 < d.td0);
  }
  if (p.LA - (d.min_ci + d.min_cj) >= drop) return true;
  return !(p.LA < d.tq0 || p.LA < d.td0);
}

template <class Store> __device__ __forceinline__ DirResult dir_finish(const DirState &d, HitState &h, int flag, const Store &S) {
  DirResult r;
  r.overflow = d.overflow;
  r.best = d.min_ci != 0 ? d.best : 0;
  if (d.min_ci != 0) {
    h.e_acc = h.e_acc + S.eq(d.min_ci - 1) + S.ed(d.min_cj - 1);
    if (flag == 0) {
      h.q_sp -= d.min_ci;
      h.db_sp -= d.min_cj;
    } else {
      h.id_start -= d.min_cj;
    }
    h.q_len += d.min_ci;
    h.db_len += d.min_cj;
  }
  h.e_tot = d.min_e;
  return r;
}

struct ResumeHeader {
  DirState d;
  double acc_prev1;
  HitState h;
  int32_t flag, nleft;
};
template <class T, class Rec> constexpr size_t resume_bytes() {
  return (sizeof(ResumeHeader) + sizeof(LdsState<T, Rec>) + 63) & ~(size_t)63;
}

template <int G, class T, class Rec>
__device__ __forceinline__ void resume_dump(const GapResume &ro, const HitCtx &c, const DirState &d, int flag,
                                            const LdsStore<T, Rec> &S, int gl, int gbase) {
  int slot = -1;
  if (gl == 0) {
    slot = (int)atomicAdd(ro.count, 1u);
    if (slot >= ro.cap) slot = -1;
  }
  slot = __shfl(slot, gbase);
  if (slot < 0) return;
  uint8_t *dst = ro.pool + (size_t)slot * resume_bytes<T, Rec>();
  ResumeHeader *H = reinterpret_cast<ResumeHeader *>(dst);
  if (gl == 0) {
    H->d = d;
    H->h = c.h;
    H->flag = flag;
    H->nleft = c.nleft;
    ro.slot[c.x] = slot;
  } else if (gl == 1) {
    H->acc_prev1 = d.acc_prev;
  }
  if constexpr (!T::kAccGlobal) {
    uint32_t *w = reinterpret_cast<uint32_t *>(dst + sizeof(ResumeHeader));
    const uint32_t *src = reinterpret_cast<const uint32_t *>(&S.s);
#pragma unroll 2
    for (int t = gl; t < (int)(sizeof(LdsState<T, Rec>) / 4); t += G) w[t] = src[t];
  } else {
    LdsState<T, Rec> *o = reinterpret_cast<LdsState<T, Rec> *>(dst + sizeof(ResumeHeader));
    for (int t = gl; t < T::kCapD; t += G) {
      o->eq[t] = S.eq(t);
      o->ed[t] = S.ed(t);
    }
    for (int t = gl; t < d.nrec; t += G) {
      o->hyb[t] = S.hyb(t);
      o->info[t] = S.info(t);
    }
    uint32_t *pw = reinterpret_cast<uint32_t *>(&o->ptab[0][0]);
    const uint32_t *ps = reinterpret_cast<const uint32_t *>(&S.s.ptab[0][0]);
    for (int t = gl; t < 3 * LdsState<T, Rec>::kPtabLen / 4; t += G) pw[t] = ps[t];
  }
}

template <int G, class TS, class RecS, class Store>
__device__ __forceinline__ void resume_load(const GapResume &ri, int slot, const GapArgs &a, HitCtx &c, DirState &d, int &flag,
                                            const Store &S, int gl) {
  using R = typename Store::R;
  const uint8_t *src = ri.pool + (size_t)slot * resume_bytes<TS, RecS>();
  const ResumeHeader *H = reinterpret_cast<const ResumeHeader *>(src);
  d = H->d;
  if (G > 1 && gl == 1) d.acc_prev = H->acc_prev1;
  d.overflow = false;
  c.h = H->h;
  c.nleft = H->nleft;
  flag = H->flag;
  const LdsState<TS, RecS> *s0 = reinterpret_cast<const LdsState<TS, RecS> *>(src + sizeof(ResumeHeader));
  stage_windows<G, true>(SeqBases{a.qb.enc, a.qb.acc, a.qb.cond, a.pg.acc, a.pg.cond}, c, flag, a.pg.seqs, a.pg.nchars, S, gl,
                         d);
  for (int t = gl; t < TS::kCapD; t += G) {
    S.eq(t) = s0->eq[t];
    S.ed(t) = s0->ed[t];
  }
  for (int t = gl; t < d.nrec; t += G) {
    S.hyb(t) = s0->hyb[t];
    const auto v = s0->info[t];
    S.info(t) = R::pack(RecS::i(v), RecS::j(v), RecS::pred(v), RecS::type(v), RecS::qa(v), RecS::da(v));
  }
  constexpr int kLenS = LdsState<TS, RecS>::kPtabLen;
  for (int t = gl; t < 3 * kLenS; t += G) {
    const int row = t / kLenS, i = t - row * kLenS;
    S.ptab(row, i) = s0->ptab[row][i];
  }
  group_sync<true>();
  acc_sync<Store>();
}

template <int kMode> __device__ __forceinline__ void hit_load(const GapArgs &a, int64_t w, HitCtx &c) {
  const SearchConst &sc = a.sc;
  const int64_t x = a.subset ? (int64_t)a.subset[w] : w;
  c.x = x;
  c.query = a.in.query[x];
  c.qo = a.qb.off[c.query];
  c.qn = a.qb.len[c.query] + 1;
  c.id = a.in.db_id[x];
  c.dbase = (int64_t)a.pg.start_pos[c.id] - c.id;
  HitState &h = c.h;
  h.q_sp = a.in.q_sp[x];
  h.db_sp = a.in.db_sp[x];
  h.q_len = a.in.q_len[x];
  h.db_len = a.in.db_len[x];
  h.id_start = a.in.db_id_start[x];
  h.e_tot = a.in.e_tot[x];
  h.e_acc = a.in.e_acc[x];
  c.diag_q = h.q_sp;
  c.diag_d = h.db_sp;
  c.diag_len = US(h.q_len);
  c.ndiag = 0;
  if (kMode != 0)
    for (int t = 0; t < c.diag_len; t++)
      c.ndiag += diag_pairs(sc, a.qb.enc[c.qo + c.diag_q + t], a.pg.seqs[c.diag_d + t]);
  c.unsorted = kMode != 0 && a.first_flag && a.first_flag[x];
  c.out0 = kMode == 2 ? a.bp_off[w] : 0;
  c.ovf = false;
  c.nleft = 0;
  c.nright = 0;
  c.resumed = false;
  c.tier0 = 0;
  if (kMode == 0 && is_resumed(a.tier_out[x])) {
    c.tier0 = a.tier_out[x] & kMarkTier;
    h.q_sp = a.out.q_sp[x];
    h.db_sp = a.out.db_sp[x];
    h.q_len = a.out.q_len[x];
    h.db_len = a.out.db_len[x];
    h.id_start = a.out.db_id_start[x];
    h.e_tot = a.out.e_tot[x];
    h.e_acc = a.out.e_acc[x];
    c.nleft = a.bp_count[x] & 0xFFFF;
    c.resumed = true;
  }
}

template <int kMode, bool kLds, class Store>
__device__ __forceinline__ void hit_dir_done(const GapArgs &a, HitCtx &c, int flag, const DirOrigin &og ,
                                             const DirResult &r, const Store &S, int gl) {
  using R = typename Store::R;
  c.ovf = r.overflow;
  if (c.ovf) return;
  int cnt = 0;
  int lslot = -1;
  if constexpr (kMode == 0 && !kLds) lslot = a.lt.slot ? a.lt.slot[c.x] : -1;
  for (int k = r.best; k != 0; k = R::pred(S.info(k)), cnt++) {
    if (kMode == 0 && kLds && gl == 0 && cnt < kTraceCap) {
      const auto v = S.info(k);
      a.trace[(c.x * 2 + flag) * kTraceCap + cnt] = (uint16_t)(R::i(v) | (R::j(v) << 8));
    }
    if (kMode == 0 && !kLds && gl == 0 && lslot >= 0 && cnt < a.lt.cap) {
      const auto v = S.info(k);
      a.lt.trace[((int64_t)lslot * 2 + flag) * a.lt.cap + cnt] = (uint32_t)R::i(v) | ((uint32_t)R::j(v) << 16);
    }
  }
  if (kMode == 0 && !kLds && gl == 0 && lslot >= 0) a.lt.count[lslot * 2 + flag] = cnt <= a.lt.cap ? cnt : -2;
  if (flag == 0) c.nleft = cnt;
  else c.nright = cnt;
  if (kMode == 2 && gl == 0) {
    int t = 0;
    for (int k = r.best; k != 0; k = R::pred(S.info(k)), t++) {
      const auto v = S.info(k);
      int64_t pos;
      int qv, dv;
      if (flag == 0) {
        qv = og.q_start - R::i(v);
        dv = (int)(og.db_start - R::j(v));
        pos = c.unsorted ? c.out0 + c.ndiag + t : c.out0 + t;
      } else {
        qv = og.q_start + R::i(v);
        dv = (int)(og.db_start + R::j(v));
        pos = c.unsorted ? c.out0 + c.ndiag + c.nleft + t : c.out0 + c.nleft + c.ndiag + (cnt - 1 - t);
      }
      a.bp_out[2 * pos] = qv;
      a.bp_out[2 * pos + 1] = dv;
    }
  }
}

template <int kMode>
__device__ __forceinline__ void hit_store(const GapArgs &a, int64_t w, const HitCtx &c, int flag , int gl) {
  if (gl != 0) return;
  const SearchConst &sc = a.sc;
  const HitState &h = c.h;
  const uint8_t *ds = a.pg.seqs, *qs = a.qb.enc + c.qo;
  if (kMode == 0) {
    a.overflow[w] = c.ovf ? 1 : 0;
    if (c.ovf && flag == 1) {
      const int64_t x = c.x;
      a.out.q_sp[x] = h.q_sp;
      a.out.db_sp[x] = h.db_sp;
      a.out.q_len[x] = h.q_len;
      a.out.db_len[x] = h.db_len;
      a.out.db_id_start[x] = h.id_start;
      a.out.e_acc[x] = h.e_acc;
      a.out.e_hyb[x] = h.e_tot - h.e_acc;
      a.out.e_tot[x] = h.e_tot;
      a.bp_count[x] = c.nleft;
      a.tier_out[x] = (uint8_t)(kResumeMark | ((c.resumed ? c.tier0 : a.tier_id) & kMarkTier));
    }
    if (!c.ovf) {
      const int64_t x = c.x;
      int tcode = a.tier_id > c.tier0 ? a.tier_id : c.tier0;
      if (a.tier_id == kWaveTier && a.lt.slot) {
        const int ls = a.lt.slot[x];
        if (ls >= 0) {
          const int c0 = a.lt.count[ls * 2], c1 = a.lt.count[ls * 2 + 1];
          if ((c0 >= 0 || (c0 == -1 && c.nleft <= kTraceCap)) && c1 >= 0) tcode = kLongTraceTier;
        }
      }
      a.tier_out[x] = (uint8_t)tcode;
      a.bp_count[x] = c.nleft | (c.nright << 16);
      const double d0 = dangle_energy_gapped(sc, h.q_sp, h.db_sp, 0, qs, c.qn, ds, a.pg.nchars);
      const double d1 = dangle_energy_gapped(sc, h.q_sp + US(h.q_len) - 1, (int64_t)h.db_sp + US(h.db_len) - 1, 1, qs, c.qn,
                                             ds, a.pg.nchars);
      double e = h.e_tot, hy = h.e_tot - h.e_acc;
      e += d0;
      e += d1;
      hy += d0;
      hy += d1;
      a.out.q_sp[x] = h.q_sp;
      a.out.db_sp[x] = h.db_sp;
      a.out.q_len[x] = h.q_len;
      a.out.db_len[x] = h.db_len;
      a.out.db_id[x] = c.id;
      a.out.db_id_start[x] = h.id_start;
      a.out.query[x] = c.query;
      a.out.e_acc[x] = h.e_acc;
      a.out.e_hyb[x] = hy;
      a.out.e_tot[x] = e;
    }
  } else if (!c.ovf) {
    int t = 0;
    const int64_t d0 = c.unsorted ? c.out0 : c.out0 + c.nleft;
    for (int u = 0; u < c.diag_len; u++)
      if (diag_pairs(sc, qs[c.diag_q + u], ds[c.diag_d + u])) {
        a.bp_out[2 * (d0 + t)] = c.diag_q + u;
        a.bp_out[2 * (d0 + t) + 1] = c.diag_d + u;
        t++;
      }
  }
}

__device__ __forceinline__ void hit_handover(const GapArgs &a, int64_t w, const HitCtx &c, int gl) {
  if (gl != 0) return;
  const int64_t x = c.x;
  const HitState &h = c.h;
  a.overflow[w] = 0;
  a.out.q_sp[x] = h.q_sp;
  a.out.db_sp[x] = h.db_sp;
  a.out.q_len[x] = h.q_len;
  a.out.db_len[x] = h.db_len;
  a.out.db_id_start[x] = h.id_start;
  a.out.e_acc[x] = h.e_acc;
  a.out.e_hyb[x] = h.e_tot - h.e_acc;
  a.out.e_tot[x] = h.e_tot;
  a.bp_count[x] = c.nleft;
  a.tier_out[x] = (uint8_t)(kHandoverMark | (a.tier_id & kMarkTier));
}

template <int kMode, class T, class Rec, bool kPair>
#ifdef PRB_TIERS_VGPR128
__global__ __launch_bounds__(T::kG *T::kGroups) __attribute__((amdgpu_num_vgpr(128))) void k_gapped_lds(GapArgs a) {
#else
__global__ __launch_bounds__(T::kG *T::kGroups, T::kWavesPerSimd) void k_gapped_lds(GapArgs a) {
#endif
  static_assert(!kPair || (T::kPairSteps && T::kG == 8), "pair steps");
  __shared__ LdsLive<T, Rec> lds[T::kGroups];
  constexpr int G = T::kG;
  const int gl = threadIdx.x & (G - 1);
  const int gbase = (threadIdx.x & 63) & ~(G - 1);
  const int gid = threadIdx.x / G;
  const LdsStore<T, Rec> S{lds[gid], T::kAccGlobal ? a.acc_scratch + ((size_t)blockIdx.x * T::kGroups + gid) * 2 * T::kCapD : nullptr};
  const int64_t ngroups = (int64_t)gridDim.x * T::kGroups;
  GapProf prof;
  prof.start();
  int64_t w = (int64_t)blockIdx.x * T::kGroups + gid;
  enum { kLoad, kInit, kRun, kFinished, kDone };
  int phase = w < a.n ? kLoad : kDone, flag = 0;
  const int period = a.period > 0 ? a.period : kPair ? (a.o.drop_w_gap > 1 ? (a.o.drop_w_gap + 1) / 2 : 1) : (a.o.drop_w_gap > 1 ? a.o.drop_w_gap : 1);
  int tick = 0;
  HitCtx c;
  DirState d;
  const SeqBases sb{a.qb.enc, a.qb.acc, a.qb.cond, a.pg.acc, a.pg.cond};
  while (__ballot(phase != kDone) != 0) {
    GP_MARK(14);
    if (a.early > 0 && tick != 0 && __popcll(__ballot(phase == kFinished)) >= a.early * G) tick = 0;
    if (tick == 0) {
      if (phase == kFinished) {
        DirResult r{true, 0};
        const DirOrigin og = dir_origin(c.h, flag);
        if (!d.overflow) {
          r = dir_finish(d, c.h, flag, S);
        } else {
          if constexpr (kMode == 0 && T::kResumable)
            if (a.rout.slot) resume_dump<G, T, Rec>(a.rout, c, d, flag, S, gl, gbase);
        }
        hit_dir_done<kMode, true>(a, c, flag, og, r, S, gl);
        group_sync<true>();
        GP_MARK(7);
        const bool hand = kMode == 0 && a.handover && !c.ovf && flag == 0 && !c.resumed;
        if (c.ovf || flag == 1 || hand) {
          if (hand) hit_handover(a, w, c, gl);
          else hit_store<kMode>(a, w, c, flag, gl);
          unsigned long long nw = 0;
          if (gl == 0) nw = (unsigned long long)ngroups + atomicAdd(a.next_work, 1ull);
          w = (int64_t)__shfl(nw, gbase);
          phase = w < a.n ? kLoad : kDone;
          GP_MARK(9);
        } else {
          flag = 1;
          phase = kInit;
        }
      }
      if (phase == kLoad) {
        hit_load<kMode>(a, w, c);
        flag = c.resumed ? 1 : 0;
        phase = kInit;
        if constexpr (kMode == 0 && T::kResumes) {
          const int slot = a.rin.slot ? a.rin.slot[c.x] : -1;
          if (slot >= 0) {
            resume_load<G, typename T::From, typename T::FromRec>(a.rin, slot, a, c, d, flag, S, gl);
            phase = kRun;
          }
        }
        GP_MARK(8);
      }
      if (phase == kInit) {
        dir_init<G, true>(a.sc, sb, c, flag, a.pg.seqs, a.pg.nchars, S, gl, a.o.delta, d);
        phase = kRun;
        GP_MARK(0);
      }
    }
    GP_MARK(15);
#ifdef PRB_GAP_PROFILE
    prof.cells_now = 0;
#endif
    if constexpr (kPair) {
      const bool run = phase == kRun;
      PairStep ps{0u, 0u, 0, 0, 0, 0, 0, 0, 0, 0, false};
      bool fin = false;
      if (run) fin = pair_prep(a.sc, sb, a.o, c, flag, S, gl, gbase, d, ps, prof);
      GP_MARK(run ? 3 : 27);
      if (a.pool) pair_fill_pool<T, Rec>(a.sc, &lds[gid & ~7], flag, ps, threadIdx.x & 63, prof);
      else if (run) pair_fill_group(a.sc, S, flag, ps, gl, prof);
      GP_MARK(run ? 26 : 27);
      if (run && (fin || pair_close(a.o, S, gl, d, ps, prof))) phase = kFinished;
      GP_MARK(run ? 6 : 27);
    } else {
      if (phase == kRun && dir_step<G, true>(a.sc, sb, a.o, c, flag, S, gl, gbase, d, prof)) phase = kFinished;
    }
#ifdef PRB_GAP_PROFILE
    if constexpr (G == 8) {
      auto wave_max = [](int v) {
        for (int m = 32; m >= 8; m >>= 1) {
          const int o = __shfl_xor(v, m);
          v = o > v ? o : v;
        }
        return v;
      };
      const int cn = prof.cells_now;
      prof.acc[16] += (unsigned long long)wave_max((cn + 1) / 2);
      prof.acc[17] += (unsigned long long)wave_max(cn);
      auto wave_sum = [](int v) {
        for (int m = 32; m >= 8; m >>= 1) v += __shfl_xor(v, m);
        return v;
      };
      prof.acc[18] += (unsigned long long)wave_sum(cn);
      if (tick & 1) {
        prof.acc[19] += (unsigned long long)wave_max((cn + prof.cells_prev + 1) / 2);
        prof.acc[20] += 1;
      } else {
        prof.cells_prev = cn;
      }
      prof.acc[21] += 1;
    }
#endif
    tick = tick + 1 == period ? 0 : tick + 1;
  }
  prof.flush(a.tier_id * 2 + (kMode != 0));
}

template <int kMode, bool kInLds> __global__ __launch_bounds__(64) void k_gapped_wave(GapArgs a, GapScratch scratch) {
  extern __shared__ __align__(16) uint8_t wave_smem[];
  const int gl = threadIdx.x;
  uint8_t *mine = kInLds ? wave_smem : scratch.base + (size_t)blockIdx.x * scratch.bytes_per_wave;
  HbmStore S;
  S.capd = scratch.cap_diag;
  S.capr = scratch.cap_rec;
  S.eq_ = reinterpret_cast<double *>(mine);
  S.ed_ = S.eq_ + S.capd;
  S.hyb_ = S.ed_ + S.capd;
  S.info_ = reinterpret_cast<uint64_t *>(S.hyb_ + S.capr);
  S.ptab_ = reinterpret_cast<uint8_t *>(S.info_ + S.capr);
  S.qb_ = S.ptab_ + 3 * ((size_t)S.capd + 4);
  S.db_ = S.qb_ + S.capd + 16;
  GapProf prof;
  prof.start();
  HitCtx c;
  DirState d;
  const SeqBases sb{a.qb.enc, a.qb.acc, a.qb.cond, a.pg.acc, a.pg.cond};
  for (int64_t w = blockIdx.x; w < a.n; w += gridDim.x) {
    hit_load<kMode>(a, w, c);
    int last = 0;
    bool hand = false;
    for (int flag = c.resumed ? 1 : 0; flag < 2 && !c.ovf && !hand; flag++) {
      GP_MARK(8);
      dir_init<64, false>(a.sc, sb, c, flag, a.pg.seqs, a.pg.nchars, S, gl, a.o.delta, d);
      GP_MARK(0);
      while (!dir_step<64, false>(a.sc, sb, a.o, c, flag, S, gl, 0, d, prof)) {
      }
      DirResult r{true, 0};
      const DirOrigin og = dir_origin(c.h, flag);
      if (!d.overflow) r = dir_finish(d, c.h, flag, S);
      hit_dir_done<kMode, false>(a, c, flag, og, r, S, gl);
      group_sync<false>();
      last = flag;
      hand = kMode == 0 && a.handover && !c.ovf && flag == 0 && !c.resumed;
      GP_MARK(7);
    }
    if (hand) hit_handover(a, w, c, gl);
    else hit_store<kMode>(a, w, c, last, gl);
    GP_MARK(9);
  }
  prof.flush(kWaveTier * 2 + (kMode != 0));
}

}

#ifdef PRB_GAP_PROFILE
extern "C" int prb_debug_gap_profile(unsigned long long *out, int reset) {
  if (hipDeviceSynchronize() != hipSuccess) return -1;
  if (hipMemcpyFromSymbol(out, HIP_SYMBOL(g_gap_prof), sizeof(unsigned long long) * 10 * kProfSlots) != hipSuccess) return -1;
  if (reset) {
    unsigned long long z[10 * kProfSlots] = {};
    if (hipMemcpyToSymbol(HIP_SYMBOL(g_gap_prof), z, sizeof(z)) != hipSuccess) return -1;
  }
  return 0;
}
#endif

size_t gapped_resume_bytes(int tier) {
  return tier == 0 ? resume_bytes<Tier0, Rec32>() : tier == 1 ? resume_bytes<Tier1, Rec32>() : resume_bytes<Tier2, Rec32>();
}

size_t gapped_acc_scratch_bytes() {
  if (!Tier1::kAccGlobal && !Tier0::kAccGlobal) return 0;
  const size_t t0 = (size_t)256 * Tier0::kWgPerCu * Tier0::kGroups * 2 * Tier0::kCapD * sizeof(double);
  const size_t t1 = (size_t)256 * Tier1::kWgPerCu * Tier1::kGroups * 2 * Tier1::kCapD * sizeof(double);
  const size_t t2 = (size_t)256 * Tier2::kWgPerCu * Tier2::kGroups * 2 * Tier2::kCapD * sizeof(double);
  return std::max(t0, std::max(t1, t2));
}

size_t gapped_wave_scratch_bytes(int cap_diag, int cap_rec) {
  size_t b = (size_t)cap_diag * 16 + (size_t)cap_rec * 16 + 3 * ((size_t)cap_diag + 4) + 2 * ((size_t)cap_diag + 16);
  return (b + 255) & ~(size_t)255;
}

namespace {
template <class T, class Rec> hipError_t launch_tier(GapArgs a, int mode, const GapTierKnobs &k, hipStream_t s) {
  const int64_t want = (a.n + T::kGroups - 1) / T::kGroups;
  const dim3 grid((unsigned)std::min<int64_t>(want, 256 * T::kWgPerCu)), blk(T::kG * T::kGroups);
  if (hipError_t e = hipMemsetAsync(a.next_work, 0, sizeof(unsigned long long), s); e != hipSuccess) return e;
  if constexpr (T::kPairSteps) {
    if (k.pair) {
      a.pool = k.pool;
      if (mode == 0) hipLaunchKernelGGL((k_gapped_lds<0, T, Rec, true>), grid, blk, 0, s, a);
      else hipLaunchKernelGGL((k_gapped_lds<2, T, Rec, true>), grid, blk, 0, s, a);
      return hipGetLastError();
    }
  }
  const size_t pad = k.pad_set ? (size_t)k.pad[a.tier_id < kLdsTiers ? a.tier_id : 0] : 0;
  if (mode == 0) hipLaunchKernelGGL((k_gapped_lds<0, T, Rec, false>), grid, blk, pad, s, a);
  else hipLaunchKernelGGL((k_gapped_lds<2, T, Rec, false>), grid, blk, 0, s, a);
  return hipGetLastError();
}
}

hipError_t launch_gapped_lds(const GapArgs &args, int mode, int tier, const GapTierKnobs &knobs, hipStream_t s) {
  if (args.n <= 0) return hipSuccess;
  GapArgs a = args;
  a.tier_id = tier;
  a.lt = LongTrace{};
  if (mode != 0) a.handover = 0;
  if (((tier == 1 || tier == 2) && Tier1::kAccGlobal || tier == 0 && Tier0::kAccGlobal) && !a.acc_scratch) return hipErrorInvalidValue;
  const bool lds_tier = tier >= 0 && tier < kLdsTiers;
  a.period = knobs.period_set && mode == 0 && lds_tier ? knobs.period[tier] : 0;
  a.pool = 1;
  a.early = tier == 2 ? 2 : 0;
  if (knobs.early_set) a.early = lds_tier ? knobs.early[tier] : 0;
  if (tier == 0) return launch_tier<Tier0, Rec32>(a, mode, knobs, s);
  if (tier == 1) return launch_tier<Tier1, Rec32>(a, mode, knobs, s);
  if (tier == 2) return launch_tier<Tier2, Rec32>(a, mode, knobs, s);
  return launch_tier<Tier3, Rec32W>(a, mode, knobs, s);
}

hipError_t launch_gapped_wave(const GapArgs &args, GapScratch scratch, int mode, hipStream_t s) {
  if (args.n <= 0) return hipSuccess;
  GapArgs a = args;
  a.tier_id = kWaveTier;
  a.trace = nullptr;
  a.next_work = nullptr;
  a.rin = a.rout = GapResume{};
  if (mode != 0) {
    a.lt = LongTrace{};
    a.handover = 0;
  }
  const int blocks = scratch.nwaves;
  if (scratch.base == nullptr) {
    const size_t lds = scratch.bytes_per_wave;
    if (mode == 0) hipLaunchKernelGGL((k_gapped_wave<0, true>), dim3(blocks), dim3(64), lds, s, a, scratch);
    else hipLaunchKernelGGL((k_gapped_wave<2, true>), dim3(blocks), dim3(64), lds, s, a, scratch);
  } else {
    if (mode == 0) hipLaunchKernelGGL((k_gapped_wave<0, false>), dim3(blocks), dim3(64), 0, s, a, scratch);
    else hipLaunchKernelGGL((k_gapped_wave<2, false>), dim3(blocks), dim3(64), 0, s, a, scratch);
  }
  return hipGetLastError();
}

}
```

### priblast_amd/csrc/search_host.hpp

```cpp
#pragma once
#include <atomic>
#include <chrono>
#include <condition_variable>
#include <cstring>
#include <deque>
#include <memory>
#include <mutex>
#include <thread>

#include <rocprim/rocprim.hpp>

#include "../../include/priblast_hip.h"
#include "context.hpp"
#include "db_format.hpp"
#include "hitset.hpp"
#include "output.hpp"
#include "search_kernels.hpp"
#include "seed_dfs.hpp"

namespace prb {

struct SearchConstMem {
  DevBuf ints, bulge;
  SearchConst view{};
};

struct PageMem {
  DevBuf seqs, sa, sa_seq, blk_seq, start_pos, seq_length, acc, cond;
  PageDev view{};
};

#define PRB_SEARCH_BUFFERS(X)                                                                                                   \
  X(cands, 1) X(row_count, 1) X(row_off, 1) X(row_cand, 1) X(seed_qacc, 1)                                           \
  X(hitsA, 1) X(hitsB, 1) X(hitsC, 1) X(hitsTmp, 1)                                                              \
  X(kE, 1) X(kL, 1) X(kQ, 1) X(kP, 1) X(kTmp, 1) X(kTmp2, 1) X(idxA, 1) X(idxB, 1) X(sortTmp, 1)                      \
  X(endKey, 1) X(pmax, 1) X(state, 1) X(keep, 1) X(pending, 0) X(surv, 1) X(count, 0) X(scanTmp, 1)         \
  X(first, 1) X(cidx, 1)                                                                                                        \
  X(gapScratch, 1) X(overflow, 1) X(tierOf, 1) X(listA, 1) X(listB, 1) X(listC, 1) X(ntrace, 1) X(trace, 1)         \
  X(frontScratch, 1) X(accScratch, 0)                                                                                           \
  X(resumeSlot, 0) X(resumeCount, 0)                                                                                            \
  X(slowList, 1) X(slowSlot, 1) X(slowCnt, 1) X(slowTrace, 1)                                                                   \
  X(keptU, 1) X(keptFirst, 1) X(keptTier, 1) X(keptNtrace, 1) X(keptTrace, 1)                               \
  X(subset, 1) X(subset2, 1) X(tierFin, 1) X(ntraceFin, 1)                                                       \
  X(bpCount, 1) X(bpOff, 1) X(bpOff2, 1) X(bpOut, 1) X(bpEnds, 1)                                                               \
  X(packed, 0) X(pairHead, 1) X(pairStart, 1)

struct SearchWs {
#define X(name, trimmable) DevBuf name;
  PRB_SEARCH_BUFFERS(X)
#undef X
  DevBuf resumePool[kLdsTiers - 1];
  struct FrontStage {
    DevBuf cands, seed_qacc, pair0, keyA, keyB, valA, valB, sortTmp;
    PinnedBuf pair0_pin;
    hipStream_t stream = nullptr;
    hipEvent_t done = nullptr;
    bool ahead = false;
    const CandDev *cd = nullptr;
    int32_t nc = 0;
    int64_t np = 0;
    PairLayout lay;
    const void *keys = nullptr, *vals = nullptr;
    DevBuf ballot, wcount, woff, scanTmp;
    PinnedBuf kept_pin;
    bool unsorted = false;
    int64_t np_all = 0;
    int init() {
      if (stream) return PRB_OK;
      int lo = 0, hi = 0;
      (void)hipDeviceGetStreamPriorityRange(&lo, &hi);
      if (hipStreamCreateWithPriority(&stream, hipStreamNonBlocking, lo) != hipSuccess ||
          hipEventCreateWithFlags(&done, hipEventDisableTiming) != hipSuccess) {
        set_error("hipStreamCreateWithPriority / hipEventCreate failed (seed front stage)");
        return PRB_ERR_HIP;
      }
      return PRB_OK;
    }
    void release() {
      if (stream) {
        (void)hipStreamSynchronize(stream);
        (void)hipStreamDestroy(stream);
        (void)hipEventDestroy(done);
        stream = nullptr;
      }
      for (DevBuf *b : {&cands, &seed_qacc, &pair0, &keyA, &keyB, &valA, &valB, &sortTmp, &ballot, &wcount, &woff, &scanTmp}) b->release();
      pair0_pin.release();
      kept_pin.release();
      ahead = false;
    }
  } front;
  hipStream_t copy_stream = nullptr;
  hipEvent_t packed_ready = nullptr, copy_done = nullptr;
  bool copy_pending = false;
  int copy_init() {
    if (copy_stream) return PRB_OK;
    if (hipStreamCreateWithFlags(&copy_stream, hipStreamNonBlocking) != hipSuccess ||
        hipEventCreateWithFlags(&packed_ready, hipEventDisableTiming) != hipSuccess ||
        hipEventCreateWithFlags(&copy_done, hipEventDisableTiming) != hipSuccess) {
      set_error("hipStreamCreate / hipEventCreate failed (result copies)");
      return PRB_ERR_HIP;
    }
    return PRB_OK;
  }
  PinnedBuf pinned, cand_pinned[2], tb_pinned, pin_hits[2], pin_bp[2];
  bool trim_next = false;
  void trim() {
#define X(name, trimmable) \
  if (trimmable && name.cap > ((size_t)256 << 20)) name.release();
    PRB_SEARCH_BUFFERS(X)
#undef X
    for (DevBuf &b : resumePool)
      if (b.cap > ((size_t)256 << 20)) b.release();
    trim_next = false;
  }
  void release() {
#define X(name, trimmable) name.release();
    PRB_SEARCH_BUFFERS(X)
#undef X
    for (DevBuf &b : resumePool) b.release();
    front.release();
    if (copy_stream) {
      (void)hipStreamSynchronize(copy_stream);
      (void)hipStreamDestroy(copy_stream);
      (void)hipEventDestroy(packed_ready);
      (void)hipEventDestroy(copy_done);
      copy_stream = nullptr;
    }
    for (PinnedBuf *b : {&pinned, &cand_pinned[0], &cand_pinned[1], &tb_pinned, &pin_hits[0], &pin_hits[1], &pin_bp[0], &pin_bp[1]})
      b->release();
  }
};

inline SearchWs &ws_of(prb_ctx *ctx) {
  if (!ctx->search_ws) ctx->search_ws = new SearchWs();
  return *static_cast<SearchWs *>(ctx->search_ws);
}

struct Drainer {
  struct Job {
    int slot;
    int64_t nhits, nbp_ints;
  };
  std::vector<prb_hit> *hits;
  std::vector<int32_t> *bp;
  std::vector<prb_pair_summary> *pairs = nullptr;
  PinnedBuf *pin_hits, *pin_bp;
  hipEvent_t ev[2] = {nullptr, nullptr};
  std::thread th;
  std::mutex m;
  std::condition_variable cv;
  std::deque<Job> jobs;
  bool busy[2] = {false, false}, stop = false, failed = false;
  std::atomic<size_t> hint_hits{0}, hint_bp{0};

  Drainer(std::vector<prb_hit> *h, std::vector<int32_t> *b, PinnedBuf *ph, PinnedBuf *pb)
      : hits(h), bp(b), pin_hits(ph), pin_bp(pb) {}
  int start() {
    for (int i = 0; i < 2; i++)
      if (hipEventCreateWithFlags(&ev[i], hipEventDisableTiming) != hipSuccess) return PRB_ERR_HIP;
    th = std::thread([this] { run(); });
    return PRB_OK;
  }
  void run() {
    for (;;) {
      Job j;
      {
        std::unique_lock<std::mutex> lk(m);
        cv.wait(lk, [this] { return stop || !jobs.empty(); });
        if (jobs.empty()) return;
        j = jobs.front();
        jobs.pop_front();
      }
      if (hipEventSynchronize(ev[j.slot]) != hipSuccess) failed = true;
      if (pairs) {
        const prb_pair_summary *ps = static_cast<const prb_pair_summary *>(pin_hits[j.slot].p);
        pairs->insert(pairs->end(), ps, ps + j.nhits);
      } else {
        const prb_hit *src = static_cast<const prb_hit *>(pin_hits[j.slot].p);
        if (hits->capacity() < hits->size() + (size_t)j.nhits)
          hits->reserve(std::max({2 * hits->capacity(), hits->size() + (size_t)j.nhits, hint_hits.load()}));
        hits->insert(hits->end(), src, src + j.nhits);
        const int32_t *bsrc = static_cast<const int32_t *>(pin_bp[j.slot].p);
        if (bp->capacity() < bp->size() + (size_t)j.nbp_ints)
          bp->reserve(std::max({2 * bp->capacity(), bp->size() + (size_t)j.nbp_ints, hint_bp.load()}));
        bp->insert(bp->end(), bsrc, bsrc + j.nbp_ints);
      }
      {
        std::lock_guard<std::mutex> lk(m);
        busy[j.slot] = false;
      }
      cv.notify_all();
    }
  }
  void acquire(int slot) {
    std::unique_lock<std::mutex> lk(m);
    cv.wait(lk, [&] { return !busy[slot]; });
    busy[slot] = true;
  }
  void submit(const Job &j) {
    {
      std::lock_guard<std::mutex> lk(m);
      jobs.push_back(j);
    }
    cv.notify_all();
  }
  int finish() {
    {
      std::lock_guard<std::mutex> lk(m);
      stop = true;
    }
    cv.notify_all();
    if (th.joinable()) th.join();
    for (int i = 0; i < 2; i++)
      if (ev[i]) (void)hipEventDestroy(ev[i]);
    return failed ? PRB_ERR_HIP : PRB_OK;
  }
};

struct HostTimer {
  prb_ctx *ctx;
  const char *name;
  std::chrono::steady_clock::time_point t0 = std::chrono::steady_clock::now();
  HostTimer(prb_ctx *c, const char *n) : ctx(c), name(n) {}
  ~HostTimer() {
    auto &t = ctx->timers[name];
    t.ms += std::chrono::duration<double, std::milli>(std::chrono::steady_clock::now() - t0).count();
    t.launches++;
  }
};

struct ToI64 {
  __host__ __device__ int64_t operator()(const int32_t &v) const { return (int64_t)v; }
};
inline int bits_for(int64_t max_value) {
  int b = 1;
  while (b < 40 && (int64_t(1) << b) <= max_value) b++;
  return b;
}

template <class Call> int with_temp(DevBuf &tmp, const char *what, Call &&call) {
  size_t bytes = 0;
  if (hipError_t e = call(nullptr, bytes); e != hipSuccess) return hip_fail(e, what);
  if (int rc = tmp.ensure(bytes)) return rc;
  if (hipError_t e = call(tmp.p, bytes); e != hipSuccess) return hip_fail(e, what);
  return PRB_OK;
}

template <class K, class V>
int sort_pairs(hipStream_t s, DevBuf &tmp, const K *kin, K *kout, const V *vin, V *vout, size_t n, unsigned begin, unsigned end) {
  return with_temp(tmp, "rocprim::radix_sort_pairs",
                   [&](void *t, size_t &b) { return rocprim::radix_sort_pairs(t, b, kin, kout, vin, vout, n, begin, end, s); });
}
template <class K, class V>
int sort_pairs(hipStream_t s, DevBuf &tmp, const K *kin, K *kout, const V *vin, V *vout, size_t n, unsigned bits) {
  return sort_pairs(s, tmp, kin, kout, vin, vout, n, 0u, bits);
}

inline PairLayout pair_layout(int64_t nchars, int64_t qspan, int row_shift, int sort_bits, bool local_order, bool force_wide) {
  PairLayout L;
  if (row_shift < 0) return L;
  const int qbits = bits_for(std::max<int64_t>(1, qspan)), pbits = bits_for(std::max<int64_t>(1, nchars - 1));
  if (!force_wide && pbits + qbits <= 32) {
    L.narrow = true;
    L.pbits = pbits;
    L.kbits = pbits + qbits;
    const int shift = std::min(row_shift, pbits);
    L.begin = shift;
    if (local_order) L.begin = std::min(std::max(shift, L.kbits - std::max(sort_bits, 1)), shift + kPairLocalBits);
    L.local_bits = L.begin - shift;
    return L;
  }
  L.shift = row_shift;
  L.pbits = bits_for(std::max<int64_t>(1, (nchars - 1) >> row_shift));
  L.kbits = L.pbits + qbits;
  return L;
}

inline int select_flagged(prb_ctx *ctx, SearchWs &w, const uint32_t *in, const uint8_t *flags, uint32_t *out, size_t n, int64_t *nsel) {
  int rc;
  if (in)
    rc = with_temp(w.scanTmp, "rocprim::select",
                   [&](void *t, size_t &b) { return rocprim::select(t, b, in, flags, out, w.count.as<size_t>(), n, ctx->stream); });
  else
    rc = with_temp(w.scanTmp, "rocprim::select", [&](void *t, size_t &b) {
      return rocprim::select(t, b, rocprim::counting_iterator<uint32_t>(0), flags, out, w.count.as<size_t>(), n, ctx->stream);
    });
  if (rc) return rc;
  size_t cnt = 0;
  PRB_HIP(hipMemcpyAsync(&cnt, w.count.p, sizeof(size_t), hipMemcpyDeviceToHost, ctx->stream));
  PRB_HIP(hipStreamSynchronize(ctx->stream));
  *nsel = (int64_t)cnt;
  return PRB_OK;
}

}

struct prb_db {
  prb_ctx *ctx = nullptr;
  prb::DbHeader hdr;
  std::vector<prb::DbPage> pages;
  std::vector<prb::PageMem> mem;
  std::vector<int> slot_of_page, page_in_slot;
  std::vector<uint64_t> slot_used;
  std::vector<hipEvent_t> slot_ready;
  uint64_t clock = 0;
  hipStream_t copy_stream = nullptr;
  bool pinned = false;
  int64_t uploads = 0;
  std::vector<prb::SeqTable> tabs;
};

namespace prb {
struct SeedPlan {
  const prb_db *db = nullptr;
  int32_t page = 0, nq = 0, max_seed_length = 0;
  double hybrid_threshold = 0;
  std::vector<std::vector<SeedCandidate>> per_q;
  std::vector<double> qpairs;
  std::vector<int64_t> qrows, qents;
  std::unique_ptr<std::atomic<int>[]> done;
  std::atomic<int32_t> next_query{0};
  std::thread producer;
  double dfs_ms = 0;
  ~SeedPlan() {
    if (producer.joinable()) producer.join();
  }
  void wait_for(int32_t q) const {
    while (!done[q].load(std::memory_order_acquire)) std::this_thread::sleep_for(std::chrono::microseconds(50));
  }
};
}

struct prb_qbatch {
  prb_ctx *ctx = nullptr;
  int32_t nq = 0, repeat_flag = 0;
  std::vector<int64_t> off;
  std::vector<int32_t> len, len_unmasked;
  std::vector<char> seqs;
  std::vector<uint8_t> enc;
  std::vector<int32_t> sa;
  prb::DevBuf d_enc, d_sa, d_acc, d_cond, d_off, d_len;
  bool have_acc = false;
  int32_t W = 0, delta = 0;
  prb::QBatchDev view{};
  std::unique_ptr<prb::SeedPlan> plan;
};

struct prb_pairmask {
  prb_ctx *ctx = nullptr;
  const prb_qbatch *qb = nullptr;
  const prb_db *db = nullptr;
  int32_t nq = 0;
  std::vector<int64_t> tbase;
  int64_t row_words = 0;
  std::vector<uint32_t> bits;
  int64_t count = 0;
  bool used = false;
  std::mutex first_use;
  prb::DevBuf dev;
  ~prb_pairmask() {
    if (dev.p) (void)hipSetDevice(ctx->device);
    dev.release();
  }
};

namespace prb {
int use_pairmask(const char *fn, prb_ctx *ctx, const prb_qbatch *qb, const prb_db *db, int32_t page, const prb_pairmask *pm, AllowDev *view);

enum class TableFeed {
  kHits,
  kPairRuns,
  kPairRecords,
  kHitRecords,
};
struct SubBatch {
  int32_t page, q0, q1, nq, nseq;
  HitSoA F;
  int64_t nfin;
  const int32_t *ends = nullptr;
  const uint32_t *pair_start = nullptr;
  int64_t npairs = 0;
  void *records = nullptr;
  const int32_t *fresh_bp = nullptr;
};

struct TableState {
  virtual ~TableState() = default;
  virtual TableFeed feed() const = 0;
  virtual int64_t bp_base() const { return 0; }
  virtual int take(const SubBatch &b) = 0;
  prb_ctx *ctx = nullptr;
  const prb_db *db = nullptr;
  bool broken = false;
  bool finished = false;
  int32_t distinct = -1;
  int32_t chain = -1;
  int64_t counts[3] = {0, 0, 0};
  DevBuf table;
  bool bad = false;
  DevBuf badflag;
  bool quiesce() const {
    if (!ctx) return false;
    (void)hipSetDevice(ctx->device);
    (void)hipStreamSynchronize(ctx->stream);
    return true;
  }
};

struct MergeTable : TableState {
  const prb_qbatch *qb = nullptr;
  int32_t nq = 0;
  std::vector<int32_t> qlen;
  std::vector<uint8_t> merged;
};

struct RunTable : TableState {
  std::vector<int64_t> tbase;
  std::vector<std::vector<uint64_t>> merged;
  DevBuf ids;
  int64_t targets() const { return tbase.empty() ? 0 : tbase.back(); }
  bool has(size_t page, int32_t id) const {
    const std::vector<uint64_t> &m = merged[page];
    return ((size_t)id >> 6) < m.size() && (m[(size_t)id >> 6] >> (id & 63) & 1);
  }
  void set(size_t page, int32_t id) {
    std::vector<uint64_t> &m = merged[page];
    if (((size_t)id >> 6) >= m.size()) m.resize(((size_t)id >> 6) + 1, 0);
    m[(size_t)id >> 6] |= 1ull << (id & 63);
  }
};

// ... 415 lines not shown
```

### priblast_amd/csrc/search_kernels.hpp

```cpp
#pragma once
#include <hip/hip_runtime.h>

#include <cstdint>

namespace prb {

struct SearchTab {
  static constexpr int kStack = 0;
  static constexpr int kInternal = kStack + 49;
  static constexpr int kMismatchI = kInternal + 31;
  static constexpr int kInt11 = kMismatchI + 175;
  static constexpr int kInt21 = kInt11 + 1600;
  static constexpr int kInt22 = kInt21 + 8000;
  static constexpr int kDangle5 = kInt22 + 40000;
  static constexpr int kDangle3 = kDangle5 + 40;
  static constexpr int kBulge = kDangle3 + 40;
  static constexpr int kTau = kBulge + 31;
  static constexpr int kZero = kTau + 8;
  static constexpr int kCount = kZero + 1;
};

struct SearchConst {
  const int32_t *tab;
  const int32_t *stack37;
  const int32_t *internal37;
  const int32_t *mismatchI37;
  const int32_t *int11;
  const int32_t *int21;
  const int32_t *int22;
  const int32_t *dangle5;
  const int32_t *dangle3;
  const double *bulge;
  int32_t terminal_au;
  uint64_t bp_rows;
  uint32_t pair_mask, wobble_mask;
  unsigned char bp_pair[25];
};

struct PageDev {
  const uint8_t *seqs;
  const int32_t *sa;
  const int32_t *sa_seq;
  const int32_t *blk_seq;
  const int32_t *start_pos;
  const int32_t *seq_length;
  const float *acc;
  const float *cond;
  int32_t nchars, nseq;
};

struct QBatchDev {
  const uint8_t *enc;
  const int32_t *sa;
  const float *acc;
  const float *cond;
  const int64_t *off;
  const int32_t *len;
  int32_t nq;
};

struct CandDev {
  int32_t sp_q, ep_q, sp_db, ep_db, length, query;
  double score;
  int64_t row0;
  int64_t qoff;
};

struct AllowDev {
  const uint32_t *bits;
  int64_t row_words, tbase;
};
__host__ __device__ inline bool pair_allowed(const AllowDev &a, int query, int db_id) {
  const int64_t t = a.tbase + db_id;
  return (a.bits[(int64_t)query * a.row_words + (t >> 5)] >> (t & 31)) & 1u;
}

struct HitSoA {
  int32_t *q_sp, *db_sp, *q_len, *db_len, *db_id, *db_id_start, *query;
  double *e_acc, *e_hyb, *e_tot;
};
constexpr int kHitInts = 7, kHitDoubles = 3;
constexpr size_t kHitBytes = kHitInts * 4 + kHitDoubles * 8;

struct ExtOpts {
  int32_t delta;
  int32_t drop_wo_gap;
  int32_t drop_w_gap;
  int32_t min_helix;
};

struct alignas(16) HitRec {
  int32_t q_sp, db_sp, q_len, db_len, db_id, db_id_start, query, pad0;
  double e_acc, e_hyb, e_tot;
  int64_t pad1;
};
static_assert(sizeof(HitRec) == 64, "one cache line half, two per 128-byte line");

hipError_t launch_sa_seq(const PageDev &pg, int32_t *sa_seq, hipStream_t s);
hipError_t launch_seed_qacc(const CandDev *cands, int32_t ncand, int64_t nq_entries, const QBatchDev &qb, int delta, double *qacc,
                            hipStream_t s);
hipError_t launch_row_keys(const CandDev *cands, int32_t ncand, int64_t nrows, const PageDev &pg, int qmin, int shift, int dbits,
                           bool wide, int32_t *row_cand, void *key, uint32_t *val, hipStream_t s);
hipError_t launch_seed_count(const CandDev *cands, int32_t ncand, int64_t nrows, const QBatchDev &qb, const PageDev &pg,
                             int delta, const double *qacc, int32_t *row_count, int32_t *row_cand, const uint32_t *row_perm,
                             hipStream_t s);
hipError_t launch_seed_emit(const CandDev *cands, int32_t ncand, int64_t nrows, const QBatchDev &qb, const PageDev &pg,
                            int delta, const double *qacc, const int32_t *row_cand, const int64_t *row_off, HitSoA hits,
                            const uint32_t *row_perm, hipStream_t s);
hipError_t launch_seed_count_allowed(const CandDev *cands, int32_t ncand, int64_t nrows, const QBatchDev &qb, const PageDev &pg,
                                     int delta, const double *qacc, int32_t *row_count, int32_t *row_cand, const uint32_t *row_perm,
                                     const AllowDev &allow, hipStream_t s);
hipError_t launch_seed_emit_allowed(const CandDev *cands, int32_t ncand, int64_t nrows, const QBatchDev &qb, const PageDev &pg,
                                    int delta, const double *qacc, const int32_t *row_cand, const int64_t *row_off, HitSoA hits,
                                    const uint32_t *row_perm, const AllowDev &allow, hipStream_t s);

hipError_t launch_ungapped(HitSoA hits, int64_t n, const QBatchDev &qb, const PageDev &pg, const SearchConst &sc,
                           ExtOpts o, int max_query_len, hipStream_t s);
inline int64_t blk_seq_entries(int64_t nchars) { return (nchars >> 5) + 1; }
hipError_t launch_blk_seq(const PageDev &pg, int32_t *blk_seq, hipStream_t s);
constexpr int64_t kMaxFusedCands = 1 << 20, kMaxFusedEntries = 1 << 12;
struct PairLayout {
  bool narrow = false;
  int shift = 0;
  int pbits = 0;
  int kbits = 0;
  int begin = 0;
  int local_bits = 0;
  bool wide_key() const { return !narrow && kbits > 32; }
  size_t key_bytes() const { return wide_key() ? 8 : 4; }
  size_t val_bytes() const { return narrow ? 4 : 8; }
};
constexpr int kPairLocalBits = 5;
hipError_t launch_pair_keys(const CandDev *cands, const int64_t *pair0, int32_t ncand, int64_t npairs, const PageDev &pg, int qmin,
                            const PairLayout &lay, void *key, void *val, hipStream_t s);
inline int64_t allow_words(int64_t npairs) { return (npairs + 63) / 64; }
hipError_t launch_allow_test(const CandDev *cands, const int64_t *pair0, const void *val, const PairLayout &lay, int64_t npairs,
                             const PageDev &pg, const AllowDev &allow, uint64_t *ballot, int32_t *count, hipStream_t s);
hipError_t launch_allow_scatter(const void *key_in, const void *val_in, int64_t npairs, const PairLayout &lay, const uint64_t *ballot,
                                const int64_t *off, void *key_out, void *val_out, hipStream_t s);
constexpr int kFusePairs = 2048, kSliceRecBytes = 48;
inline int64_t fused_slices(int64_t npairs) { return (npairs + kFusePairs - 1) / kFusePairs; }
hipError_t launch_seed_extend(const CandDev *cands, const void *keys, const void *vals, const PairLayout &lay, int64_t npairs,
                              const QBatchDev &qb, const PageDev &pg, const SearchConst &sc, ExtOpts o, const double *qacc, double thr,
                              int max_query_len, void *slices, int32_t *slice_count, uint64_t *nseed, hipStream_t s);
hipError_t launch_collect_slices(const void *slices, const int32_t *slice_count, const int64_t *slice_off, int64_t nslices, HitRec *out,
                                 hipStream_t s);

struct PackedKeyInfo {
  int32_t qmin, lmax;
  int32_t bl, bq, bd;
  int32_t one_len = 0;
};
hipError_t launch_make_packed_keys(const HitSoA &hits, int64_t n, const PackedKeyInfo &f, uint64_t *key, uint64_t *k_energy,
                                   uint32_t *idx, hipStream_t s);
hipError_t launch_make_packed_keys_recs(const HitRec *hits, int64_t n, const PackedKeyInfo &f, uint64_t *key, uint64_t *k_energy,
                                        uint32_t *idx, hipStream_t s);
hipError_t launch_fix_ties(const uint64_t *key_sorted, const uint64_t *e_sorted, const uint32_t *perm, int64_t n, const HitRec *recs,
                           uint32_t *perm_out, int32_t *too_long, hipStream_t s);
hipError_t launch_make_keys(const HitSoA &hits, int64_t n, uint64_t *k_energy, uint32_t *k_len, uint32_t *k_qsp,
                            uint64_t *k_pos, uint32_t *idx, hipStream_t s);
hipError_t launch_order_keys(const double *v, int64_t n, uint64_t *key, hipStream_t s);
hipError_t launch_gather_u64(const uint64_t *src, const uint32_t *idx, uint64_t *dst, int64_t n, hipStream_t s);
hipError_t launch_gather_u32(const uint32_t *src, const uint32_t *idx, uint32_t *dst, int64_t n, hipStream_t s);
hipError_t launch_gather_u8(const uint8_t *src, const uint32_t *idx, uint8_t *dst, int64_t n, hipStream_t s);
hipError_t launch_iota_u32(uint32_t *dst, int64_t n, hipStream_t s);
hipError_t launch_gather_rows(const void *src, const uint32_t *idx, void *dst, int64_t n, int row_bytes, hipStream_t s);
hipError_t launch_gather_hits(const HitSoA &src, const uint32_t *idx, HitSoA dst, int64_t n, hipStream_t s);
hipError_t launch_gather_hits_to_recs(const HitSoA &src, const uint32_t *idx, HitRec *dst, int64_t n, hipStream_t s);
hipError_t launch_gather_recs_to_hits(const HitRec *src, const uint32_t *idx, HitSoA dst, int64_t n, hipStream_t s);
hipError_t launch_flag_marked(const uint8_t *marks, const uint32_t *list, int64_t n, uint8_t mask, uint8_t *flags, hipStream_t s);
hipError_t launch_flag_not_above(const double *e_tot, int64_t n, double thr, uint8_t *keep, hipStream_t s);
hipError_t launch_mark_first(const int32_t *query, int64_t n, uint8_t *first, hipStream_t s);
hipError_t launch_pack_hits(const HitSoA &src, int64_t n, const int32_t *bp_count, const int64_t *bp_off, int64_t bp_base,
                            void *out, hipStream_t s);

hipError_t launch_filter_init(const HitSoA &h, int64_t n, double thr, int64_t *db_end_key, uint8_t *state, hipStream_t s);
hipError_t launch_filter_round(const HitSoA &h, int64_t n, const int64_t *pmax, uint8_t *state, int32_t *pending, bool tiles,
                               hipStream_t s);
hipError_t launch_filter_final(const HitSoA &h, int64_t n, const int64_t *pmax, const uint8_t *state, uint8_t *keep, bool tiles,
                               hipStream_t s);

constexpr size_t kGapWaveLdsBytes = 64 * 1024;
struct GapScratch {
  uint8_t *base;
  size_t bytes_per_wave;
  int32_t cap_rec, cap_diag;
  int32_t nwaves;
};
size_t gapped_wave_scratch_bytes(int cap_diag, int cap_rec);
struct GapResume {
  int32_t *slot = nullptr;
  uint8_t *pool = nullptr;
  uint32_t *count = nullptr;
  int32_t cap = 0;
};
size_t gapped_resume_bytes(int tier);
constexpr int kLdsTiers = 4, kWaveTier = 4;
struct GapTierKnobs {
  bool pair = true;
  bool pool = true;
  bool pad_set = false, period_set = false, early_set = false;
  int pad[kLdsTiers] = {};
  int period[kLdsTiers] = {};
  int early[kLdsTiers] = {};
};
constexpr int kTraceCap = 32;
constexpr int kLongTraceTier = 5;
struct LongTrace {
  uint32_t *trace = nullptr;
  int32_t *count = nullptr;
  const int32_t *slot = nullptr;
  int32_t cap = 0;
};
constexpr uint8_t kResumeMark = 0x40, kHandoverMark = 0x80, kMarkTier = 0x07;
__host__ __device__ inline bool is_resumed(uint8_t t) { return (t & (kResumeMark | kHandoverMark)) != 0; }
struct GapArgs {
  HitSoA in{}, out{};
  int64_t n = 0;
  const uint32_t *subset = nullptr;
  QBatchDev qb{};
  PageDev pg{};
  SearchConst sc{};
  ExtOpts o{};
  uint8_t *overflow = nullptr;
  uint8_t *tier_out = nullptr;
  int tier_id = 0;
  const uint8_t *first_flag = nullptr;
  int32_t *bp_count = nullptr;
  uint16_t *trace = nullptr;
  const int64_t *bp_off = nullptr;
  int32_t *bp_out = nullptr;
  unsigned long long *next_work = nullptr;
  GapResume rin{}, rout{};
  LongTrace lt{};
  double *acc_scratch = nullptr;
  int period = 0;
  int early = 0;
  int pool = 1;
  int handover = 0;
};
hipError_t launch_gapped_lds(const GapArgs &a, int mode, int tier, const GapTierKnobs &knobs, hipStream_t s);
size_t gapped_acc_scratch_bytes();
hipError_t launch_gapped_wave(const GapArgs &a, GapScratch scratch, int mode, hipStream_t s);

constexpr int kFrontMaxDrop = 16;
bool gapped_front_supported(const SearchConst &sc, const ExtOpts &o);
size_t gapped_front_scratch_bytes();
hipError_t launch_gapped_front(const GapArgs &a, void *scratch, bool second_only, hipStream_t s);

hipError_t launch_assign_slots(const uint32_t *list, int64_t n, int32_t base, int32_t *slot, hipStream_t s);
hipError_t launch_bp_count(const HitSoA &in, int64_t n, const uint32_t *subset, const QBatchDev &qb, const PageDev &pg,
                           const SearchConst &sc, const int32_t *ntrace, int32_t *bp_count, hipStream_t s);
hipError_t launch_bp_expand(const HitSoA &in, int64_t n, const uint32_t *subset, const QBatchDev &qb, const PageDev &pg,
                            const SearchConst &sc, const uint8_t *first_flag, const int32_t *ntrace, const uint8_t *tier_of,
                            const uint16_t *trace, const LongTrace &lt, const int64_t *bp_off, int32_t *bp_out, hipStream_t s);
hipError_t launch_bp_ends(const int64_t *bp_off, int64_t n, const int32_t *bp, int32_t *ends, hipStream_t s);

hipError_t launch_pair_heads(const int32_t *query, const int32_t *db_id, int64_t n, uint8_t *head, hipStream_t s);
hipError_t launch_pair_fold(const HitSoA &h, int64_t n, const uint32_t *start, int64_t npairs, const int32_t *ends, void *out,
                            hipStream_t s);
constexpr int kSiteLdsHits = 2048;
constexpr int kSiteLongGrid = 1024;
inline int64_t site_long_runs_max(int64_t n) { return n / 2 + 1; }
struct SiteScratch {
  uint32_t *long_list;
  uint32_t *nlong;
  int32_t *lo, *hi;
  uint8_t *state;
};
hipError_t launch_site_select(const HitSoA &h, int64_t n, const uint8_t *head, int lds_hits, const SiteScratch &w, uint8_t *keep,
                              hipStream_t s);
constexpr int kChainLdsHits = 1536;
struct ChainScratch {
  uint32_t *long_list;
  uint32_t *nlong;
  double *score;
  int32_t *prev;
};
hipError_t launch_chain_select(const HitSoA &h, int64_t n, const uint8_t *head, int lds_hits, const ChainScratch &w, uint8_t *keep,
                               hipStream_t s);

constexpr int kTopMaxN = 1024;
hipError_t launch_top_merge(const void *rec, int64_t nrec, int32_t q0, int32_t q1, int32_t page, int32_t n, void *tab, int32_t *fill,
                            hipStream_t s);
hipError_t launch_tophits_merge(const void *rec, int64_t nrec, int32_t q0, int32_t q1, int32_t page, int32_t n, void *tab, int32_t *fill,
                                hipStream_t s);
hipError_t launch_tophits_counts(const void *tab, const int32_t *fill, int32_t n, int64_t nslots, int32_t *cnt, hipStream_t s);
hipError_t launch_tophits_gather(void *tab, const int32_t *fill, int32_t n, int64_t nslots, const int64_t *off, int64_t split,
                                 const int32_t *old_pool, const int32_t *fresh, int32_t *pool, hipStream_t s);
hipError_t launch_top_join(void *tab, int32_t *fill, const void *src, const int32_t *src_fill, int32_t nq, int32_t n, hipStream_t s);
hipError_t launch_tophits_join(void *tab, int32_t *fill, const void *src, const int32_t *src_fill, int32_t nq, int32_t n, int64_t shift,
                               hipStream_t s);

struct alignas(16) TargetKey {
  uint64_t e;
  uint32_t id, at;
};
hipError_t launch_target_ids(void *rec, int64_t nrec, const int32_t *ids, int32_t nq, uint32_t *key, uint32_t *val, hipStream_t s);
hipError_t launch_target_runs(const void *rec, int64_t nrec, const uint32_t *key, const uint32_t *val, TargetKey *rkey, uint8_t *head,
                              hipStream_t s);
hipError_t launch_target_merge(const void *rec, const TargetKey *rkey, const uint32_t *db_of, const uint32_t *start, int64_t nruns,
                               int64_t nrec, int32_t page, int64_t tbase, int32_t nseq, int32_t n, TargetKey *keys, void *slots, int32_t *fill,
                               hipStream_t s);
hipError_t launch_target_join(TargetKey *keys, void *slots, int32_t *fill, const TargetKey *skeys, const void *sslots, const int32_t *sfill,
                              int64_t ntargets, int32_t n, hipStream_t s);
hipError_t launch_target_gather(const TargetKey *keys, const void *slots, const int64_t *off, int64_t ntargets, int32_t n, int64_t total,
                                void *out, hipStream_t s);

struct ProfTab {
  const int64_t *off;
  unsigned long long *hdiff;
  unsigned long long *key, *tie;
  unsigned long long *skey;
  double *e_min;
  int32_t *tdiff;
  uint32_t *stie;
  int32_t *db_id;
  int32_t *bp;
  uint32_t *bad;
  int32_t nq;
};
hipError_t launch_prof_keys(int64_t n, const uint32_t *start, int64_t npairs, const int32_t *ends, uint64_t *key, uint32_t *val,
                            hipStream_t s);
hipError_t launch_prof_span(int64_t n, const uint64_t *key, const uint32_t *val, const int32_t *ends, uint64_t *v, hipStream_t s);
hipError_t launch_prof_add(const HitSoA &h, int64_t n, const uint64_t *key, const uint32_t *val, const uint64_t *m, const int32_t *ends,
                           const ProfTab &t, hipStream_t s);
hipError_t launch_prof_min(const HitSoA &h, int64_t n, const uint32_t *val, const int32_t *ends, const ProfTab &t, hipStream_t s);
hipError_t launch_prof_merge(const HitSoA &h, const int32_t *ends, const ProfTab &t, int64_t p0, int64_t p1, int32_t page,
                             hipStream_t s);
hipError_t launch_prof_join(const ProfTab &t, const ProfTab &src, int64_t P, hipStream_t s);
hipError_t launch_prof_rows(const ProfTab &t, const uint32_t *idx, int64_t n, const int64_t *hits, const int32_t *targets, void *rows,
                            hipStream_t s);

struct CovTab {
  const int64_t *seq_lo;
  unsigned long long *hdiff;
  unsigned long long *key, *tie;
  unsigned long long *skey, *stie;
  double *e_min;
  int32_t *qdiff;
  uint32_t *starts;
  int32_t *bp;
  uint32_t *bad;
};
struct CovPage {
  int64_t slot0, target0;
  int32_t nseq;
};
struct CovHits {
  int64_t n;
  const int32_t *query, *db_id;
  const double *e_tot;
  const int32_t *ends;
};
hipError_t launch_cov_keys(const CovHits &h, const CovTab &t, const CovPage &pg, uint64_t *key, uint32_t *val, uint32_t *place, hipStream_t s);
hipError_t launch_cov_span(const CovHits &h, const uint64_t *key, const uint32_t *val, const CovTab &t, const CovPage &pg, uint64_t *v,
                           hipStream_t s);
hipError_t launch_cov_add(const CovHits &h, const uint64_t *key, const uint32_t *val, const uint64_t *m, const CovTab &t, const CovPage &pg,
                          hipStream_t s);
hipError_t launch_cov_min(const CovHits &h, const uint32_t *val, const uint32_t *place, const int32_t *ids, const CovTab &t, const CovPage &pg,
                          hipStream_t s);
hipError_t launch_cov_join(const CovTab &t, const CovTab &src, int64_t P, hipStream_t s);
hipError_t launch_cov_regions(const CovTab &t, const int64_t *tbase, int32_t npages, int64_t ntargets, const uint32_t *first, int64_t nregions,
                              const int64_t *hits, const int32_t *queries, int32_t D, void *out, hipStream_t s);

struct NullSlot {
  uint64_t s[8];
  unsigned long long null_hits, null_le, null_min;
  uint32_t observed, reserved;
};
static_assert(sizeof(NullSlot) == 96, "NullSlot: 64 B of record, three counters, the flag");
struct NullTab {
  NullSlot *slot;
  uint8_t *obs;
  uint32_t *bad;
  int64_t nslots, ntargets;
  int32_t nq, ndecoys;
};
struct NullPage {
  int64_t target0;
  int32_t nseq;
};
hipError_t launch_null_clear(const NullTab &t, hipStream_t s);
hipError_t launch_null_observe(const void *rec, int64_t nrec, const NullTab &t, const NullPage &pg, hipStream_t s);
hipError_t launch_null_count(const void *rec, int64_t nrec, const int32_t *owner, const int32_t *decoy, int32_t ndq, const NullTab &t,
                             const NullPage &pg, hipStream_t s);
hipError_t launch_null_gather(const NullTab &t, const uint32_t *idx, int64_t n, const int64_t *tbase, int32_t npages, void *out, hipStream_t s);

struct GroupSlot {
  uint64_t s[8];
  unsigned long long ekey, tie;
  unsigned long long hits;
  uint32_t members, reserved;
};
static_assert(sizeof(GroupSlot) == 96, "GroupSlot: 64 B of record, two keys, two counters");
struct GroupTab {
  GroupSlot *slot;
  uint32_t *bad;
  int64_t nslots;
  int32_t nq, ngroups, npages;
};
struct GroupPage {
  const int32_t *group_of;
  int32_t page, nseq;
};
inline constexpr int kGroupSelect = 2048;
hipError_t launch_group_clear(const GroupTab &t, hipStream_t s);
hipError_t launch_group_fold(const void *rec, int64_t nrec, const GroupTab &t, const GroupPage &pg, hipStream_t s);
hipError_t launch_group_join(const GroupTab &t, const GroupSlot *src, hipStream_t s);
hipError_t launch_group_flags(const GroupTab &t, uint8_t *occ, hipStream_t s);
hipError_t launch_group_select(const GroupTab &t, const uint32_t *occ, int64_t nocc, int32_t n, uint32_t *top, uint8_t *keep, hipStream_t s);
hipError_t launch_group_gather(const GroupTab &t, const uint32_t *idx, int64_t nrec, const uint32_t *top, int32_t n, void *out, hipStream_t s);

hipError_t launch_grouprank_slot_groups(const GroupTab &t, const uint32_t *cand, int64_t ncand, uint32_t *key, uint32_t *val, uint32_t *bad,
                                        hipStream_t s);
hipError_t launch_grouprank_record_groups(const void *rec, int64_t nrec, int32_t ngroups, uint32_t *key, uint32_t *val, uint32_t *bad,
                                          hipStream_t s);
hipError_t launch_grouprank_slot_runs(const GroupTab &t, const int32_t *ids, int64_t ncand, const uint32_t *key, const uint32_t *val,
                                      TargetKey *rkey, uint8_t *head, uint32_t *bad, hipStream_t s);
hipError_t launch_grouprank_record_runs(const void *rec, int64_t nrec, int32_t ngroups, const uint32_t *key, const uint32_t *val, TargetKey *rkey,
                                        uint8_t *head, uint32_t *bad, hipStream_t s);
struct GroupRankRuns {
  const TargetKey *rkey;
  const uint32_t *group_of, *start;
  int64_t nruns, ncand;
};
hipError_t launch_grouprank_slot_merge(const GroupTab &t, const int32_t *ids, const GroupRankRuns &r, int32_t n, TargetKey *keys, void *slots,
                                       int32_t *fill, hipStream_t s);
hipError_t launch_grouprank_record_merge(const void *rec, int64_t nrec, const GroupRankRuns &r, int32_t ngroups, int32_t n, TargetKey *keys,
                                         void *slots, int32_t *fill, hipStream_t s);
hipError_t launch_grouprank_join(TargetKey *keys, void *slots, int32_t *fill, const TargetKey *skeys, const void *sslots, const int32_t *sfill,
                                 int64_t ngroups, int32_t n, hipStream_t s);
hipError_t launch_grouprank_gather(const TargetKey *keys, const void *slots, const int64_t *off, int64_t ngroups, int32_t n, int64_t total,
                                   void *out, hipStream_t s);

struct GNullCount {
  unsigned long long ekey, null_hits, null_le, null_min;
};
struct GNullTab {
  uint32_t *lookup;
  GNullCount *cnt;
  unsigned long long *cell;
  const int32_t *owner, *decoy;
  uint32_t *bad;
  int64_t nkept;
  int32_t nq, ngroups, ndecoys, npages, ndq;
};
hipError_t launch_gnull_keep(const void *rec, const GNullTab &t, void *kept, hipStream_t s);
hipError_t launch_gnull_fold(const void *rec, int64_t nrec, const GNullTab &t, const GroupPage &pg, hipStream_t s);
hipError_t launch_gnull_close(const GNullTab &t, hipStream_t s);
hipError_t launch_gnull_gather(const GNullTab &t, const void *kept, void *out, hipStream_t s);

struct EvalTab {
  const unsigned long long *rkey, *dkey;
  const int64_t *roff, *doff;
  uint32_t *null_le, *rank, *qnum, *qden;
  uint32_t *bad;
  int64_t nreal, ndecoy;
  int32_t nq, ndecoys;
};
inline constexpr int kEvalChunk = 256;
hipError_t launch_eval_append(const int32_t *ids, const double *energy, int64_t n, const int32_t *owner, const int32_t *decoy, int32_t ndq,
                              int32_t nq, int32_t ndecoys, unsigned long long *key, uint32_t *own, uint32_t *bad, hipStream_t s);
hipError_t launch_eval_iota(uint32_t *v, int64_t n, hipStream_t s);
hipError_t launch_eval_gather32(const uint32_t *src, const uint32_t *idx, uint32_t *dst, int64_t n, uint32_t *bad, hipStream_t s);
hipError_t launch_eval_gather64(const unsigned long long *src, const uint32_t *idx, unsigned long long *dst, int64_t n, uint32_t *bad, hipStream_t s);
hipError_t launch_eval_count(const uint32_t *own, int64_t n, int32_t nq, uint32_t *cnt, uint32_t *bad, hipStream_t s);
hipError_t launch_eval_rank(const EvalTab &t, hipStream_t s);
hipError_t launch_eval_qmin(const EvalTab &t, hipStream_t s);
hipError_t launch_eval_lookup(const EvalTab &t, const int32_t *query, const double *energy, int64_t n, void *out, hipStream_t s);

struct FeatPage {
  const int32_t *off;
  const int32_t *slo, *slen;
  const int32_t *tlo, *thi, *idx;
  int32_t page, nseq;
};
struct FeatHits {
  int64_t n;
  const int32_t *query, *db_id;
  const double *e_tot, *e_acc, *e_hyb;
  const int32_t *ends;
};
struct FeatWork {
  int32_t *cnt;
  int64_t *ioff;
  void *tmp;
  uint8_t *flag;
  uint32_t *long_list, *nlong;
  uint32_t *bad;
};
inline constexpr int kFeatLongRun = 128;
hipError_t launch_feat_count(const FeatHits &h, const uint32_t *start, int64_t npairs, const FeatPage &pg, int32_t nq, const FeatWork &w,
                             hipStream_t s);
hipError_t launch_feat_items(const FeatHits &h, const uint32_t *start, int64_t npairs, int64_t nitems, const FeatPage &pg, const FeatWork &w,
                             hipStream_t s);
hipError_t launch_feat_items_long(const FeatHits &h, const uint32_t *start, int64_t npairs, int64_t nitems, const FeatPage &pg,
                                  const FeatWork &w, hipStream_t s);
hipError_t launch_feat_unassigned(const FeatHits &h, const FeatPage &pg, int32_t nq, const FeatWork &w, hipStream_t s);
hipError_t launch_feat_append(const void *tmp, const uint32_t *sel, int64_t nsel, void *rec, int64_t base, int64_t *first, int64_t *end,
                              int32_t page, int32_t nq, hipStream_t s);
hipError_t launch_feat_join(void *rec, int64_t base, int64_t *first, int64_t *end, const void *src_rec, int64_t nsrc, const int64_t *src_first,
                            const int64_t *src_end, int64_t ncells, hipStream_t s);
hipError_t launch_feat_cell_counts(const int64_t *first, const int64_t *end, int32_t npages, int32_t nq, int64_t *cnt, hipStream_t s);
hipError_t launch_feat_gather(const void *rec, int64_t nrec, const int64_t *first, const int64_t *off, int32_t npages, int32_t nq, int64_t total,
                              void *out, uint32_t *bad, hipStream_t s);

struct FNullTab {
  const unsigned long long *key;
  const uint32_t *rec;
  const int64_t *qoff;
  GNullCount *cnt;
  unsigned long long *cell;
  const int32_t *owner, *decoy;
  const int64_t *doff;
  uint32_t *bad;
  int64_t nkept, ncells, nfeat;
  int32_t nq, ndecoys, npages, ndq;
};
hipError_t launch_fnull_keep(const void *rec, const FNullTab &t, void *kept, unsigned long long *key, uint32_t *idx, hipStream_t s);
hipError_t launch_fnull_order(const FNullTab &t, hipStream_t s);
hipError_t launch_fnull_items(const FeatHits &h, const uint32_t *start, int64_t npairs, int64_t nitems, const FeatPage &pg, const FeatWork &w,
                              const FNullTab &t, hipStream_t s);
hipError_t launch_fnull_items_long(const FeatHits &h, const uint32_t *start, int64_t npairs, int64_t nitems, const FeatPage &pg,
                                   const FeatWork &w, const FNullTab &t, hipStream_t s);
hipError_t launch_fnull_close(const FNullTab &t, hipStream_t s);
hipError_t launch_fnull_gather(const FNullTab &t, const void *kept, void *out, hipStream_t s);
// ... 3 lines not shown
```

Before: 7.874.

## Build gapped-cascade work lists on device and defer stage timer syncs

Gapped extension kernels now append overflowing hits straight into the next tier's work list with wave-aggregated atomics and read the list length from device memory. This replaces the per-tier host select and the synchronizing readback between tiers. Stage timers record events and resolve them in one flush, and the counts are read back once per chunk. In exchange, each launch is sized by an upper bound and may start idle waves, the handover path now uses a rocPRIM select over all hits, and an extra filter-round launch was added at round zero.

```diff
diff --git a/priblast_amd/csrc/capi_core.hip b/priblast_amd/csrc/capi_core.hip
--- a/priblast_amd/csrc/capi_core.hip
+++ b/priblast_amd/csrc/capi_core.hip
@@ -78,6 +78,39 @@
   t.ms += ms;
   t.launches += launches;
   return PRB_OK;
+}
+static int later_event(prb_ctx *ctx, hipEvent_t *ev) {
+  if (ctx->later_used == ctx->later_events.size()) {
+    hipEvent_t e = nullptr;
+    PRB_HIP(hipEventCreate(&e));
+    ctx->later_events.push_back(e);
+  }
+  *ev = ctx->later_events[ctx->later_used++];
+  PRB_HIP(hipEventRecord(*ev, ctx->stream));
+  return PRB_OK;
+}
+int prb_ctx::time_begin_later() { return later_event(this, &later_open); }
+int prb_ctx::time_end_later(prb::StageTimer &t, int64_t launches) {
+  hipEvent_t e1 = nullptr;
+  if (int rc = later_event(this, &e1)) return rc;
+  later.push_back(LaterBracket{later_open, e1, &t, launches});
+  return PRB_OK;
+}
+int prb_ctx::time_flush() {
+  int rc = PRB_OK;
+  if (!later.empty()) {
+    hipError_t e = hipEventSynchronize(later.back().e1);
+    for (const LaterBracket &b : later) {
+      float ms = 0;
+      if (e == hipSuccess) e = hipEventElapsedTime(&ms, b.e0, b.e1);
+      b.t->ms += ms;
+      b.t->launches += b.launches;
+    }
+    if (e != hipSuccess) rc = prb::hip_fail(e, "hipEventSynchronize / hipEventElapsedTime (stage timers)");
+  }
+  later.clear();
+  later_used = 0;
+  return rc;
 }
 
 using namespace prb;
@@ -195,6 +228,7 @@
     b->release();
   if (ctx->ev0) (void)hipEventDestroy(ctx->ev0);
   if (ctx->ev1) (void)hipEventDestroy(ctx->ev1);
+  for (hipEvent_t e : ctx->later_events) (void)hipEventDestroy(e);
   if (ctx->stream) (void)hipStreamDestroy(ctx->stream);
   delete ctx;
 }
diff --git a/priblast_amd/csrc/capi_gapped.hip b/priblast_amd/csrc/capi_gapped.hip
--- a/priblast_amd/csrc/capi_gapped.hip
+++ b/priblast_amd/csrc/capi_gapped.hip
@@ -1,5 +1,6 @@
 #include <algorithm>
 #include <cstdio>
+#include <vector>
 
 #include "search_stages.hpp"
 
@@ -7,18 +8,69 @@
 
 static const char *const kTierTimer[5] = {"gapped", "gapped_t1", "gapped_t2", "gapped_t3", "gapped_slow"};
 
+constexpr int kGapCounts = 32;
+constexpr int kSlowCount = 0, kHandCount = 2;
 struct WorkList {
   const uint32_t *cur = nullptr;
-  int64_t m = 0;
+  int slot = -1;
+  int64_t bound = 0;
   uint32_t *bufs[2];
   int nb = 0;
-  uint32_t *spare() const { return bufs[nb]; }
 };
 struct Cascade {
   WorkList l;
   GapResume rs[kLdsTiers - 1];
   int skip_mask = 0;
+  unsigned *counts = nullptr;
+  int used = 4;
+  struct Launch {
+    int tier;
+    int in, out;
+    bool first_dir;
+  };
+  std::vector<Launch> launches;
+  unsigned slow_seen = 0;
 };
+
+struct HandedOver {
+  __host__ __device__ bool operator()(const uint8_t &mark) const { return (mark & kHandoverMark) != 0; }
+};
+
+static void list_in(const Cascade &c, GapArgs &a) {
+  a.n = c.l.bound;
+  a.subset = c.l.cur;
+  a.n_dev = c.l.slot >= 0 ? c.counts + c.l.slot : nullptr;
+}
+static void list_out(Cascade &c, GapArgs &a, int tier, bool first_dir, uint32_t *slow_list) {
+  const bool last = tier == kLdsTiers - 1;
+  const int out = last ? kSlowCount : c.used++;
+  a.next_list = last ? slow_list : c.l.bufs[c.l.nb];
+  a.next_count = c.counts + out;
+  c.launches.push_back({tier, c.l.slot, out, first_dir});
+  if (!last) {
+    c.l.cur = c.l.bufs[c.l.nb];
+    c.l.nb ^= 1;
+  }
+  c.l.slot = out;
+}
+static int read_counts(SubSearch &s, const unsigned **host) {
+  int rc;
+  if ((rc = s.w.gap_pinned.ensure(kGapCounts * sizeof(unsigned)))) return rc;
+  PRB_HIP(hipMemcpyAsync(s.w.gap_pinned.p, s.w.gapCounts.p, kGapCounts * sizeof(unsigned), hipMemcpyDeviceToHost, s.ctx->stream));
+  PRB_HIP(hipStreamSynchronize(s.ctx->stream));
+  *host = static_cast<const unsigned *>(s.w.gap_pinned.p);
+  return PRB_OK;
+}
+static int debug_row(SubSearch &s, Cascade &c) {
+  const unsigned *h = nullptr;
+  if (int rc = read_counts(s, &h)) return rc;
+  const Cascade::Launch &k = c.launches.back();
+  const long long in = k.in < 0 ? (long long)s.nch : h[k.in], out = k.out == kSlowCount ? h[k.out] - c.slow_seen : h[k.out];
+  if (k.out == kSlowCount) c.slow_seen = h[k.out];
+  if (k.tier < 0) fprintf(stderr, "[front] hits %lld, go on %lld\n", in, out);
+  else fprintf(stderr, "[tier %d%s] hits %lld, go on %lld\n", k.tier, k.first_dir ? ", first direction" : "", in, out);
+  return PRB_OK;
+}
 
 static GapArgs view_args(const SubSearch &s, int mode) {
   SearchWs &w = s.w;
@@ -61,13 +113,6 @@
 static int select_overflow(SubSearch &s, const uint32_t *cur, int64_t m, uint32_t *next, int64_t *mout) {
   return select_flagged(s.ctx, s.w, cur, s.w.overflow.as<uint8_t>(), next, (size_t)m, mout);
 }
-static int advance(SubSearch &s, WorkList &l, int64_t *rest) {
-  if (int rc = select_overflow(s, l.cur, l.m, l.spare(), rest)) return rc;
-  l.cur = l.spare();
-  l.nb ^= 1;
-  return PRB_OK;
-}
-
 static int run_wave(SubSearch &s, int mode, const uint32_t *cur, int64_t m, uint32_t *spare, const int64_t *off_dev, int handover = 0) {
   prb_ctx *ctx = s.ctx;
   SearchWs &w = s.w;
@@ -125,64 +170,47 @@
   }
   return PRB_OK;
 }
-static int run_slow(SubSearch &s, WorkList &l, int handover) {
-  int rc;
-  if (!handover) call_front_free(s);
+static int run_slow(SubSearch &s, const uint32_t *cur, int64_t m, uint32_t *spare) {
+  int rc;
+  call_front_free(s);
   if ((rc = s.ctx->time_begin())) return rc;
-  s.hs->slow_hits += l.m;
-  s.ctx->slow_hits += l.m;
-  if ((rc = run_wave(s, 0, l.cur, l.m, l.spare(), nullptr, handover))) return rc;
-  l.m = 0;
+  s.hs->slow_hits += m;
+  s.ctx->slow_hits += m;
+  if ((rc = run_wave(s, 0, cur, m, spare, nullptr, 0))) return rc;
   return s.ctx->time_end(kTierTimer[kWaveTier], 1);
 }
 
 static int run_front(SubSearch &s, Cascade &c, bool second_only = false) {
   prb_ctx *ctx = s.ctx;
   SearchWs &w = s.w;
-  WorkList &l = c.l;
   int rc;
   if ((rc = w.frontScratch.ensure(gapped_front_scratch_bytes()))) return rc;
-  if ((rc = ctx->time_begin())) return rc;
+  if ((rc = ctx->time_begin_later())) return rc;
   GapArgs a = view_args(s, 0);
-  a.n = l.m;
-  a.subset = l.cur;
+  list_in(c, a);
+  list_out(c, a, -1, false, nullptr);
   a.tier_id = 0;
   PRB_HIP(launch_gapped_front(a, w.frontScratch.p, second_only && !s.k.front_paired, ctx->stream));
-  int64_t rest = 0;
-  if ((rc = advance(s, l, &rest))) return rc;
-  if (s.k.debug_rows) fprintf(stderr, "[front] hits %lld, go on %lld\n", (long long)l.m, (long long)rest);
-  ctx->timers["gapped_front_hits"].launches += l.m - rest;
-  l.m = rest;
-  return ctx->time_end("gapped_front", 1);
-}
-
-static int run_cascade(SubSearch &s, Cascade &c, int handover, bool hold_wave) {
-  prb_ctx *ctx = s.ctx;
-  WorkList &l = c.l;
-  int rc;
-  for (int tier = s.k.first_tier; tier <= kWaveTier && l.m > 0; tier++) {
+  if ((rc = ctx->time_end_later(ctx->timers["gapped_front"], 0))) return rc;
+  return s.k.debug_rows ? debug_row(s, c) : PRB_OK;
+}
+
+static int run_cascade(SubSearch &s, Cascade &c, int handover) {
+  prb_ctx *ctx = s.ctx;
+  int rc;
+  for (int tier = s.k.first_tier; tier < kLdsTiers; tier++) {
     if (tier < kLdsTiers - 1 && ((c.skip_mask >> tier) & 1)) continue;
-    if (tier == kWaveTier) {
-      if (hold_wave) break;
-      if ((rc = run_slow(s, l, handover))) return rc;
-      continue;
-    }
-    if ((rc = ctx->time_begin())) return rc;
-    if (tier == 0) ctx->timers["gapped_tier0_hits"].launches += l.m;
+    if ((rc = ctx->time_begin_later())) return rc;
     GapArgs a = view_args(s, 0);
-    a.n = l.m;
-    a.subset = l.cur;
+    list_in(c, a);
+    list_out(c, a, tier, handover != 0, s.w.slowList.as<uint32_t>());
     if (tier >= 1) a.rin = c.rs[tier - 1];
     if (tier < kLdsTiers - 1) a.rout = c.rs[tier];
     a.handover = handover;
     a.acc_scratch = s.w.accScratch.as<double>();
     PRB_HIP(launch_gapped_lds(a, 0, tier, s.k.tiers, ctx->stream));
-    int64_t rest = 0;
-    if ((rc = advance(s, l, &rest))) return rc;
-    if (s.k.debug_rows)
-      fprintf(stderr, "[tier %d%s] hits %lld, go on %lld\n", tier, handover ? ", first direction" : "", (long long)l.m, (long long)rest);
-    l.m = rest;
-    if ((rc = ctx->time_end(kTierTimer[tier], 1))) return rc;
+    if ((rc = ctx->time_end_later(ctx->timers[kTierTimer[tier]], 0))) return rc;
+    if (s.k.debug_rows && (rc = debug_row(s, c))) return rc;
   }
   return PRB_OK;
 }
@@ -213,59 +241,65 @@
 }
 
 static int run_handover(SubSearch &s, Cascade &c) {
-  prb_ctx *ctx = s.ctx;
-  SearchWs &w = s.w;
-  WorkList &l = c.l;
-  int rc;
-  const int64_t m_first = l.m;
-  if ((rc = w.listC.ensure((size_t)m_first * 4))) return rc;
-  PRB_HIP(hipMemcpyAsync(w.listC.p, l.cur, (size_t)m_first * 4, hipMemcpyDeviceToDevice, ctx->stream));
-  if ((rc = run_cascade(s, c, 1, true))) return rc;
-  const int64_t n_slow = l.m;
-  if (n_slow > 0) {
-    if ((rc = w.slowList.ensure((size_t)n_slow * 4))) return rc;
-    PRB_HIP(hipMemcpyAsync(w.slowList.p, l.cur, (size_t)n_slow * 4, hipMemcpyDeviceToDevice, ctx->stream));
-  }
-  PRB_HIP(launch_flag_marked(w.tierOf.as<uint8_t>(), w.listC.as<uint32_t>(), m_first, kHandoverMark, w.overflow.as<uint8_t>(), ctx->stream));
-  l.cur = w.listC.as<uint32_t>();
-  l.m = m_first;
-  int64_t mh = 0;
-  if ((rc = advance(s, l, &mh))) return rc;
-  l.m = mh;
-  if (l.m > 0) {
-    if (c.rs[0].slot && (rc = clear_resume(s))) return rc;
-    if ((rc = run_front(s, c, true))) return rc;
-    if ((rc = run_cascade(s, c, 0, true))) return rc;
-  }
-  if (n_slow + l.m == 0) return PRB_OK;
-  if (l.m > 0) {
-    if ((rc = grow_keep(ctx, w.slowList, (size_t)n_slow * 4, (size_t)(n_slow + l.m) * 4))) return rc;
-    PRB_HIP(hipMemcpyAsync(w.slowList.as<uint32_t>() + n_slow, l.cur, (size_t)l.m * 4, hipMemcpyDeviceToDevice, ctx->stream));
-  }
-  l.cur = w.slowList.as<uint32_t>();
-  l.m += n_slow;
-  return run_slow(s, l, 0);
+  int rc;
+  if ((rc = run_cascade(s, c, 1))) return rc;
+  static_assert(kHandCount % 2 == 0, "rocPRIM writes a size_t: the kernels read its low half");
+  if ((rc = with_temp(s.w.scanTmp, "rocprim::select", [&](void *t, size_t &b) {
+         return rocprim::select(t, b, rocprim::counting_iterator<uint32_t>(0),
+                                rocprim::make_transform_iterator(s.w.tierOf.as<uint8_t>(), HandedOver()), s.w.listC.as<uint32_t>(),
+                                reinterpret_cast<size_t *>(c.counts + kHandCount), (size_t)s.nch, s.ctx->stream);
+       })))
+    return rc;
+  c.l.cur = s.w.listC.as<uint32_t>();
+  c.l.slot = kHandCount;
+  if (c.rs[0].slot && (rc = clear_resume(s))) return rc;
+  if ((rc = run_front(s, c, true))) return rc;
+  return run_cascade(s, c, 0);
+}
+
+static int book_counts(SubSearch &s, const Cascade &c, int64_t *n_slow) {
+  prb_ctx *ctx = s.ctx;
+  const unsigned *h = nullptr;
+  int rc;
+  if ((rc = read_counts(s, &h)) || (rc = ctx->time_flush())) return rc;
+  for (const Cascade::Launch &k : c.launches) {
+    const int64_t in = k.in < 0 ? s.nch : (int64_t)h[k.in];
+    if (in > 0) (k.tier < 0 ? ctx->timers["gapped_front"] : ctx->timers[kTierTimer[k.tier]]).launches += 1;
+    if (k.tier < 0) ctx->timers["gapped_front_hits"].launches += in - (int64_t)h[k.out];
+    if (k.tier == 0) ctx->timers["gapped_tier0_hits"].launches += in;
+  }
+  *n_slow = h[kSlowCount];
+  return PRB_OK;
 }
 
 static int extend_chunk(SubSearch &s) {
+  prb_ctx *ctx = s.ctx;
   SearchWs &w = s.w;
   int rc;
   Cascade c;
+  ctx->later.clear();
+  ctx->later_used = 0;
   if ((rc = w.accScratch.ensure(std::max<size_t>(gapped_acc_scratch_bytes(), 8)))) return rc;
-  PRB_HIP(hipMemsetAsync(w.tierOf.p, 0, (size_t)s.nch, s.ctx->stream));
+  PRB_HIP(hipMemsetAsync(w.tierOf.p, 0, (size_t)s.nch, ctx->stream));
+  if (s.nch == 0) return PRB_OK;
+  PRB_HIP(hipMemsetAsync(w.gapCounts.p, 0, kGapCounts * sizeof(unsigned), ctx->stream));
   if (!s.k.no_resume) {
     if ((rc = prepare_resume(s, c)) || (rc = clear_resume(s))) return rc;
   }
-  c.l.m = s.nch;
+  c.counts = w.gapCounts.as<unsigned>();
+  c.l.bound = s.nch;
   c.l.bufs[0] = w.listA.as<uint32_t>();
   c.l.bufs[1] = w.listB.as<uint32_t>();
+  if (s.k.first_tier >= kWaveTier) return run_slow(s, nullptr, s.nch, c.l.bufs[0]);
   const bool front_on = s.k.first_tier == 0 && s.k.front && gapped_front_supported(s.sc, s.eo);
   if (front_on) {
     if ((rc = run_front(s, c))) return rc;
     c.skip_mask = s.k.skip_tiers;
   }
-  if (!(front_on && s.k.handover)) return run_cascade(s, c, 0, false);
-  return c.l.m > 0 ? run_handover(s, c) : PRB_OK;
+  if ((rc = front_on && s.k.handover ? run_handover(s, c) : run_cascade(s, c, 0))) return rc;
+  int64_t n_slow = 0;
+  if ((rc = book_counts(s, c, &n_slow))) return rc;
+  return n_slow > 0 ? run_slow(s, w.slowList.as<uint32_t>(), n_slow, c.l.bufs[0]) : PRB_OK;
 }
 
 static int keep_chunk(SubSearch &s, int64_t c0) {
@@ -309,7 +343,8 @@
   const size_t NM = (size_t)s.nmax;
   if ((rc = w.hitsC.ensure(hits_bytes(s.nmax)))) return rc;
   if ((rc = w.overflow.ensure(NM)) || (rc = w.subset.ensure(NM * 4)) || (rc = w.ntrace.ensure(NM * 4)) || (rc = w.tierOf.ensure(NM)) ||
-      (rc = w.listA.ensure(NM * 4)) || (rc = w.listB.ensure(NM * 4)) || (rc = w.count.ensure(16)) ||
+      (rc = w.listA.ensure(NM * 4)) || (rc = w.listB.ensure(NM * 4)) || (rc = w.listC.ensure(NM * 4)) || (rc = w.slowList.ensure(NM * 4)) ||
+      (rc = w.count.ensure(16)) || (rc = w.gapCounts.ensure(kGapCounts * sizeof(unsigned))) ||
       (rc = w.trace.ensure(NM * 2 * kTraceCap * sizeof(uint16_t))))
     return rc;
   s.G = carve_hits(w.hitsC, s.nmax);
diff --git a/priblast_amd/csrc/capi_search.hip b/priblast_amd/csrc/capi_search.hip
--- a/priblast_amd/csrc/capi_search.hip
+++ b/priblast_amd/csrc/capi_search.hip
@@ -189,6 +189,7 @@
        })))
     return rc;
   for (int round = 0;; round++) {
+    if (round == 0) PRB_HIP(launch_filter_round(h, n, w.pmax.as<int64_t>(), w.state.as<uint8_t>(), w.pending.as<int32_t>(), tiles, ctx->stream));
     PRB_HIP(hipMemsetAsync(w.pending.p, 0, 4, ctx->stream));
     PRB_HIP(launch_filter_round(h, n, w.pmax.as<int64_t>(), w.state.as<uint8_t>(), w.pending.as<int32_t>(), tiles, ctx->stream));
     int32_t pend = 0;
diff --git a/priblast_amd/csrc/context.hpp b/priblast_amd/csrc/context.hpp
--- a/priblast_amd/csrc/context.hpp
+++ b/priblast_amd/csrc/context.hpp
@@ -66,4 +66,16 @@
   int time_end(const char *stage, int64_t launches);
   int time_end(prb::ModeTimer t, int64_t launches) { return time_end(mode_timers[(int)t], launches); }
   int time_end(prb::StageTimer &t, int64_t launches);
+  struct LaterBracket {
+    hipEvent_t e0, e1;
+    prb::StageTimer *t;
+    int64_t launches;
+  };
+  std::vector<hipEvent_t> later_events;
+  size_t later_used = 0;
+  std::vector<LaterBracket> later;
+  hipEvent_t later_open = nullptr;
+  int time_begin_later();
+  int time_end_later(prb::StageTimer &t, int64_t launches);
+  int time_flush();
 };
diff --git a/priblast_amd/csrc/gapped_args.hpp b/priblast_amd/csrc/gapped_args.hpp
--- a/priblast_amd/csrc/gapped_args.hpp
+++ b/priblast_amd/csrc/gapped_args.hpp
@@ -22,7 +22,16 @@
   static __device__ __forceinline__ int da(word v) { return (v >> 27) & 7; }
 };
 
-
+__device__ __forceinline__ void wave_append(uint32_t *list, unsigned *count, bool take, uint32_t x) {
+  const unsigned long long m = __ballot(take);
+  if (m == 0) return;
+  const int lane = (int)__lane_id(), leader = __ffsll((long long)m) - 1;
+  int base = 0;
+  if (lane == leader) base = (int)atomicAdd(count, (unsigned)__popcll(m));
+  base = __builtin_amdgcn_readlane(base, leader);
+  if (take) list[(unsigned)base + (unsigned)__popcll(m & ((1ull << lane) - 1))] = x;
+}
+__device__ __forceinline__ int64_t list_length(const GapArgs &a) { return a.n_dev ? (int64_t)*a.n_dev : a.n; }
 
 struct DirOrigin {
   int q_start, id_start, id_end;
diff --git a/priblast_amd/csrc/gapped_front.hip b/priblast_amd/csrc/gapped_front.hip
--- a/priblast_amd/csrc/gapped_front.hip
+++ b/priblast_amd/csrc/gapped_front.hip
@@ -217,7 +217,8 @@
   const int drop = a.o.drop_w_gap, min_helix = a.o.min_helix, delta = a.o.delta;
   const int64_t nwaves = (int64_t)gridDim.x * kFWaves;
   constexpr int kTileHits = kOneDir ? kFDirs : kFDirs / 2;
-  const int64_t ntiles = (a.n + kTileHits - 1) / kTileHits;
+  const int64_t n = list_length(a);
+  const int64_t ntiles = (n + kTileHits - 1) / kTileHits;
   const bool isdir = lane < kFDirs;
   const int me = isdir ? lane : 0;
   int64_t tile = (int64_t)blockIdx.x * kFWaves + (threadIdx.x >> 6);
@@ -227,7 +228,7 @@
     FP_COUNT(16, 1);
     unsigned long long nt = 0;
     const int64_t w = tile * kTileHits + (kOneDir ? lane : lane >> 1);
-    const bool live = isdir && w < a.n;
+    const bool live = isdir && w < n;
     int64_t x = 0, qo = 0, dbase = 0;
     int query = 0, id = 0, qn = 1, q_sp = 0, db_sp = 0, q_len = 0, db_len = 0, id_start = 0;
     double e_tot = 0, e_acc = 0;
@@ -536,7 +537,6 @@
         e += d1;
         hy += d0;
         hy += d1;
-        a.overflow[w] = 0;
         a.tier_out[x] = (uint8_t)(resumed ? tier0 : a.tier_id);
         a.bp_count[x] = nleft0;
         a.out.q_sp[x] = q_sp;
@@ -550,7 +550,6 @@
         a.out.e_hyb[x] = hy;
         a.out.e_tot[x] = e;
       } else {
-        a.overflow[w] = 1;
         if (resumed) {
           a.tier_out[x] = (uint8_t)(kResumeMark | tier0);
         } else if (ok) {
@@ -567,6 +566,7 @@
         }
       }
     }
+    wave_append(a.next_list, a.next_count, live && (kOneDir || f0) && !(ok && ok_other), (uint32_t)x);
     wave_mem_sync();
     tile = nwaves + (int64_t)__shfl(nt, 0);
     FP_MARK(12);
diff --git a/priblast_amd/csrc/gapped_lds.hip b/priblast_amd/csrc/gapped_lds.hip
--- a/priblast_amd/csrc/gapped_lds.hip
+++ b/priblast_amd/csrc/gapped_lds.hip
@@ -1332,14 +1332,14 @@
   }
 }
 
-template <int kMode>
+template <int kMode, bool kLds>
 __device__ __forceinline__ void hit_store(const GapArgs &a, int64_t w, const HitCtx &c, int flag , int gl) {
   if (gl != 0) return;
   const SearchConst &sc = a.sc;
   const HitState &h = c.h;
   const uint8_t *ds = a.pg.seqs, *qs = a.qb.enc + c.qo;
   if (kMode == 0) {
-    a.overflow[w] = c.ovf ? 1 : 0;
+    if constexpr (!kLds) a.overflow[w] = c.ovf ? 1 : 0;
     if (c.ovf && flag == 1) {
       const int64_t x = c.x;
       a.out.q_sp[x] = h.q_sp;
@@ -1396,11 +1396,12 @@
   }
 }
 
+template <bool kLds>
 __device__ __forceinline__ void hit_handover(const GapArgs &a, int64_t w, const HitCtx &c, int gl) {
   if (gl != 0) return;
   const int64_t x = c.x;
   const HitState &h = c.h;
-  a.overflow[w] = 0;
+  if constexpr (!kLds) a.overflow[w] = 0;
   a.out.q_sp[x] = h.q_sp;
   a.out.db_sp[x] = h.db_sp;
   a.out.q_len[x] = h.q_len;
@@ -1429,9 +1430,10 @@
   const int64_t ngroups = (int64_t)gridDim.x * T::kGroups;
   GapProf prof;
   prof.start();
+  const int64_t n = list_length(a);
   int64_t w = (int64_t)blockIdx.x * T::kGroups + gid;
   enum { kLoad, kInit, kRun, kFinished, kDone };
-  int phase = w < a.n ? kLoad : kDone, flag = 0;
+  int phase = w < n ? kLoad : kDone, flag = 0;
   const int period = a.period > 0 ? a.period : kPair ? (a.o.drop_w_gap > 1 ? (a.o.drop_w_gap + 1) / 2 : 1) : (a.o.drop_w_gap > 1 ? a.o.drop_w_gap : 1);
   int tick = 0;
   HitCtx c;
@@ -1455,12 +1457,17 @@
         GP_MARK(7);
         const bool hand = kMode == 0 && a.handover && !c.ovf && flag == 0 && !c.resumed;
         if (c.ovf || flag == 1 || hand) {
-          if (hand) hit_handover(a, w, c, gl);
-          else hit_store<kMode>(a, w, c, flag, gl);
+          if (hand) hit_handover<true>(a, w, c, gl);
+          else hit_store<kMode, true>(a, w, c, flag, gl);
+          if constexpr (kMode == 0 && G == 64) {
+            if (gl == 0 && c.ovf) a.next_list[atomicAdd(a.next_count, 1u)] = (uint32_t)c.x;
+          } else if constexpr (kMode == 0) {
+            wave_append(a.next_list, a.next_count, gl == 0 && c.ovf, (uint32_t)c.x);
+          }
           unsigned long long nw = 0;
           if (gl == 0) nw = (unsigned long long)ngroups + atomicAdd(a.next_work, 1ull);
           w = (int64_t)__shfl(nw, gbase);
-          phase = w < a.n ? kLoad : kDone;
+          phase = w < n ? kLoad : kDone;
           GP_MARK(9);
         } else {
           flag = 1;
@@ -1573,8 +1580,8 @@
       hand = kMode == 0 && a.handover && !c.ovf && flag == 0 && !c.resumed;
       GP_MARK(7);
     }
-    if (hand) hit_handover(a, w, c, gl);
-    else hit_store<kMode>(a, w, c, last, gl);
+    if (hand) hit_handover<false>(a, w, c, gl);
+    else hit_store<kMode, false>(a, w, c, last, gl);
     GP_MARK(9);
   }
   prof.flush(kWaveTier * 2 + (kMode != 0));
@@ -1649,6 +1656,16 @@
   return launch_tier<Tier3, Rec32W>(a, mode, knobs, s);
 }
 
+extern "C" int prb_debug_gapped_resident_hits(int tier) {
+  switch (tier) {
+  case 0: return 256 * Tier0::kWgPerCu * Tier0::kGroups;
+  case 1: return 256 * Tier1::kWgPerCu * Tier1::kGroups;
+  case 2: return 256 * Tier2::kWgPerCu * Tier2::kGroups;
+  case 3: return 256 * Tier3::kWgPerCu * Tier3::kGroups;
+  }
+  return -1;
+}
+
 hipError_t launch_gapped_wave(const GapArgs &args, GapScratch scratch, int mode, hipStream_t s) {
   if (args.n <= 0) return hipSuccess;
   GapArgs a = args;
diff --git a/priblast_amd/csrc/search_host.hpp b/priblast_amd/csrc/search_host.hpp
--- a/priblast_amd/csrc/search_host.hpp
+++ b/priblast_amd/csrc/search_host.hpp
@@ -38,7 +38,7 @@
   X(first, 1) X(cidx, 1)                                                                                                        \
   X(gapScratch, 1) X(overflow, 1) X(tierOf, 1) X(listA, 1) X(listB, 1) X(listC, 1) X(ntrace, 1) X(trace, 1)         \
   X(frontScratch, 1) X(accScratch, 0)                                                                                           \
-  X(resumeSlot, 0) X(resumeCount, 0)                                                                                            \
+  X(resumeSlot, 0) X(resumeCount, 0) X(gapCounts, 0)                                                                                          \
   X(slowList, 1) X(slowSlot, 1) X(slowCnt, 1) X(slowTrace, 1)                                                                   \
   X(keptU, 1) X(keptFirst, 1) X(keptTier, 1) X(keptNtrace, 1) X(keptTrace, 1)                               \
   X(subset, 1) X(subset2, 1) X(tierFin, 1) X(ntraceFin, 1)                                                       \
@@ -102,7 +102,7 @@
     }
     return PRB_OK;
   }
-  PinnedBuf pinned, cand_pinned[2], tb_pinned, pin_hits[2], pin_bp[2];
+  PinnedBuf pinned, cand_pinned[2], tb_pinned, pin_hits[2], pin_bp[2], gap_pinned;
   bool trim_next = false;
   void trim() {
 #define X(name, trimmable) \
@@ -126,7 +126,7 @@
       (void)hipEventDestroy(copy_done);
       copy_stream = nullptr;
     }
-    for (PinnedBuf *b : {&pinned, &cand_pinned[0], &cand_pinned[1], &tb_pinned, &pin_hits[0], &pin_hits[1], &pin_bp[0], &pin_bp[1]})
+    for (PinnedBuf *b : {&pinned, &cand_pinned[0], &cand_pinned[1], &tb_pinned, &pin_hits[0], &pin_hits[1], &pin_bp[0], &pin_bp[1], &gap_pinned})
       b->release();
   }
 };
diff --git a/priblast_amd/csrc/search_kernels.hpp b/priblast_amd/csrc/search_kernels.hpp
--- a/priblast_amd/csrc/search_kernels.hpp
+++ b/priblast_amd/csrc/search_kernels.hpp
@@ -222,7 +222,10 @@
   PageDev pg{};
   SearchConst sc{};
   ExtOpts o{};
+  const unsigned *n_dev = nullptr;
   uint8_t *overflow = nullptr;
+  uint32_t *next_list = nullptr;
+  unsigned *next_count = nullptr;
   uint8_t *tier_out = nullptr;
   int tier_id = 0;
   const uint8_t *first_flag = nullptr;
```

After: 7.831. About the same (-0.5%).
